# matthewyjiang/safe_bayesian_optimization

Measured on AMD Instinct MI355X. Metric: GP posterior+acq grid-points/sec at N train pts; 1/2/4/8 GPU, higher is better.
Workload: dtype f32 (bf16x3-split MFMA, f32 accumulation)

## Files before the change

### include/sbo.h

```cpp
#ifndef SBO_H_
#define SBO_H_

#include <stdint.h>

#ifdef __cplusplus
extern "C" {
#endif

#define SBO_API __attribute__((visibility("default")))

typedef enum sbo_status {
    SBO_OK = 0,
    SBO_E_INVAL = 1,
    SBO_E_NOT_SPD = 2,
    SBO_E_DEVICE = 3,
    SBO_E_OOM = 4,
    SBO_E_EMPTY = 5,
    SBO_E_STATE = 6
} sbo_status;

#define SBO_DEVICE_PTRS 0x1u
#define SBO_ASYNC 0x2u

typedef struct sbo_hyper {
// ... 89 lines not shown
SBO_API sbo_status sbo_import_state(sbo_ctx *ctx, const void *dev_buf, int64_t bytes);

SBO_API int64_t sbo_find_contours_external(const uint8_t *img, int width, int height,
                                           int32_t *pts, int64_t pts_cap,
                                           int64_t *start, int64_t contours_cap);

SBO_API sbo_status sbo_rbf_fill(sbo_ctx *ctx, const float *x, const float *y, int64_t n,
                                sbo_hyper hyper, float *K, uint32_t flags);
SBO_API sbo_status sbo_get_factor(sbo_ctx *ctx, float *L, float *alpha, uint32_t flags);

SBO_API sbo_status sbo_kd_order(const float *x, const float *y, int64_t n, int64_t first_offset, int64_t *perm);

#define SBO_OPT_INVERSE_BITS 1
#define SBO_OPT_SPATIAL_ORDER 2
#define SBO_OPT_TILE_SKIP 3
#define SBO_OPT_QUERY_ORDER 4
#define SBO_OPT_KERNEL_VARIANT 5
#define SBO_OPT_SWEEP_GROUPS 6
#define SBO_OPT_SKIP_BUDGET 7
#define SBO_OPT_CHOLESKY 8
#define SBO_OPT_INVERSE 9
#define SBO_OPT_JITTER_RETRIES 10
#define SBO_OPT_PRECISION 11
#define SBO_OPT_RESORT 12
#define SBO_OPT_CHOL_RESERVE 13
#define SBO_OPT_INV_OVERLAP 14
#define SBO_OPT_CHOL_OUTER 15
#define SBO_OPT_CHOL_DIAG 16
#define SBO_OPT_CHOL_GEMM 17
#define SBO_OPT_INV_BASE 18
#define SBO_OPT_INV_PANELS 19
#define SBO_OPT_INV_LEAVES 20
#define SBO_OPT_REPROBE 21
#define SBO_OPT_PRECISE_KERNEL 22
#define SBO_OPT_TABLE_MB 23
#define SBO_OPT_INV_OZ 24
#define SBO_OPT_INV_CHECK 25
#define SBO_OPT_PLAN_BLOCK 26
#define SBO_OPT_PROBE_SIZE 27
#define SBO_OPT_INV_OZ_MIN 28
#define SBO_OPT_INV_OZ_ADAPT 29
SBO_API sbo_status sbo_set_option(sbo_ctx *ctx, int option, int64_t value);

typedef struct sbo_inv_check {
    int32_t ran, fired, digits, m;
    double err, err_grid, err_train, err_fallback, tol, var_max, ms;
    double err_mean, mean_max, err_mean_fallback;
    int32_t kept_digits, reserved;
} sbo_inv_check;
SBO_API sbo_status sbo_get_inverse_check(const sbo_ctx *ctx, sbo_inv_check *out);

SBO_API sbo_status sbo_trim(sbo_ctx *ctx);

SBO_API sbo_status sbo_warmup(sbo_ctx *ctx, int64_t n_cap, int64_t m_cap, sbo_hyper hyper);

SBO_API sbo_status sbo_get_precision(const sbo_ctx *ctx, int *precise, double *probe_err, double *probe_var_min,
                                     double *probe_var_max);

typedef struct sbo_probe {
    int32_t precise, m_grid, m_train, precise_kernel;
    int64_t n_at_probe;
    double err, err_grid, err_train;
    double var_min, var_max, var_max_grid, var_max_train;
} sbo_probe;
SBO_API sbo_status sbo_get_probe(const sbo_ctx *ctx, sbo_probe *out);

SBO_API sbo_status sbo_get_skip(const sbo_ctx *ctx, int *cutoff_log2, double *max_row_l1, double *alpha_l1);

SBO_API sbo_status sbo_get_order(const sbo_ctx *ctx, int64_t *order);

SBO_API sbo_status sbo_get_inverse(sbo_ctx *ctx, float *Linv);

SBO_API sbo_status sbo_get_tile_bounds(sbo_ctx *ctx, float *bounds, int64_t cap);

SBO_API sbo_status sbo_profile(sbo_ctx *ctx, int enable);
SBO_API sbo_status sbo_profile_read(sbo_ctx *ctx, double *predict_ms, int64_t *predict_launches,
                                    double *fill_ms, int64_t *fill_launches);
SBO_API sbo_status sbo_profile_work(sbo_ctx *ctx, double *predict_flops);
SBO_API sbo_status sbo_profile_mfma(sbo_ctx *ctx, double *mfma_flops, int64_t *tiles_by_level );
SBO_API sbo_status sbo_debug_x3_stamps(sbo_ctx *ctx, double *cycles, int n);

SBO_API sbo_status sbo_debug_x3_operand(sbo_ctx *ctx, void *host_buf, int64_t cap, int64_t *bytes);

#define SBO_GZ_TRI_A 1u
#define SBO_GZ_TRANS_A 2u
#define SBO_GZ_TRI_B_LOWER 4u
#define SBO_GZ_TRI_B_UPPER 8u
#define SBO_GZ_TRANS_B 16u
#define SBO_GZ_TRANS_C 32u
#define SBO_GZ_BETA1 64u
#define SBO_GZ_LOWER_C 128u
SBO_API sbo_status sbo_debug_gz_gemm(sbo_ctx *ctx, int nd, int is_f32, const void *A, int64_t lda, int64_t a_cols,
                                     const void *B, int64_t ldb, int64_t b_cols, int64_t m, int64_t n, int64_t K,
                                     double alpha, void *C, int64_t ldc, int64_t c_cols, uint32_t flags);
SBO_API sbo_status sbo_debug_gz_gemm_packed(sbo_ctx *ctx, int nd, const float *P, int64_t ld, int64_t mpack,
                                            int64_t K, int64_t a0, int64_t m, int64_t b0, int64_t n, double alpha,
                                            float *C, int64_t ldc, int64_t c_cols, uint32_t flags);

#ifdef __cplusplus
}
#endif

#endif
```

### safe_bayesian_optimization_amd/_native.py

```python
from __future__ import annotations

import ctypes
import os
import subprocess

_PKG = os.path.dirname(os.path.abspath(__file__))
LIB_PATH = os.environ.get("SBO_LIB") or os.path.join(_PKG, "lib", "libsbo.so")

SBO_DEVICE_PTRS = 0x1
SBO_ASYNC = 0x2
SCORE_WIDTH = 0
SCORE_UCB = 1
SBO_E_STATE = 6

STATUS = {0: "SBO_OK", 1: "SBO_E_INVAL", 2: "SBO_E_NOT_SPD", 3: "SBO_E_DEVICE", 4: "SBO_E_OOM",
          5: "SBO_E_EMPTY", 6: "SBO_E_STATE"}

EXPORTS = (
    "sbo_version", "sbo_status_string", "sbo_create", "sbo_destroy", "sbo_set_stream", "sbo_last_error",
    "sbo_fit", "sbo_append", "sbo_num_train", "sbo_predict", "sbo_compute_sets", "sbo_compute_sets_f64", "sbo_argmax", "sbo_tick",
    "sbo_key_combine", "sbo_find_safety_contour_indices", "sbo_next_subgoal", "sbo_find_contours_external",
    "sbo_rbf_fill", "sbo_get_factor", "sbo_profile", "sbo_profile_read", "sbo_set_option", "sbo_get_inverse",
    "sbo_get_order", "sbo_profile_work", "sbo_profile_mfma", "sbo_debug_x3_stamps", "sbo_get_skip", "sbo_frontier", "sbo_subgoal",
    "sbo_get_bounds", "sbo_get_jitter", "sbo_get_tile_bounds", "sbo_state_bytes", "sbo_export_state", "sbo_import_state", "sbo_query_cost",
    "sbo_polygon_correct", "sbo_polydist", "sbo_point_within", "sbo_project_subgoal", "sbo_get_precision",
    "sbo_kd_order", "sbo_get_probe", "sbo_keys_reduce", "sbo_get_inverse_check", "sbo_trim", "sbo_warmup",
    "sbo_debug_gz_gemm", "sbo_debug_gz_gemm_packed", "sbo_debug_x3_operand",
)
SBO_GZ_TRI_A = 1
SBO_GZ_TRANS_A = 2
SBO_GZ_TRI_B_LOWER = 4
SBO_GZ_TRI_B_UPPER = 8
SBO_GZ_TRANS_B = 16
SBO_GZ_TRANS_C = 32
SBO_GZ_BETA1 = 64
SBO_GZ_LOWER_C = 128
SBO_OPT_INVERSE_BITS = 1
SBO_OPT_SPATIAL_ORDER = 2
SBO_OPT_TILE_SKIP = 3
SBO_OPT_QUERY_ORDER = 4
SBO_OPT_KERNEL_VARIANT = 5
SBO_OPT_SWEEP_GROUPS = 6
SBO_OPT_SKIP_BUDGET = 7
SBO_OPT_CHOLESKY = 8
SBO_OPT_INVERSE = 9
SBO_OPT_JITTER_RETRIES = 10
SBO_OPT_PRECISION = 11
SBO_OPT_RESORT = 12
SBO_OPT_CHOL_RESERVE = 13
SBO_OPT_INV_OVERLAP = 14
SBO_OPT_CHOL_OUTER = 15
SBO_OPT_CHOL_DIAG = 16
SBO_OPT_CHOL_GEMM = 17
SBO_OPT_INV_BASE = 18
SBO_OPT_INV_PANELS = 19
SBO_OPT_INV_LEAVES = 20
SBO_OPT_REPROBE = 21
SBO_OPT_PRECISE_KERNEL = 22
SBO_OPT_TABLE_MB = 23
SBO_OPT_INV_OZ = 24
SBO_OPT_INV_CHECK = 25
SBO_OPT_PLAN_BLOCK = 26
SBO_OPT_PROBE_SIZE = 27
SBO_OPT_INV_OZ_MIN = 28
SBO_OPT_INV_OZ_ADAPT = 29


class SboError(RuntimeError):
    def __init__(self, status: int, message: str = ""):
        self.status = status
        super().__init__(f"{STATUS.get(status, status)}: {message}")


class NotSPDError(SboError):
    pass


class sbo_hyper(ctypes.Structure):
    _fields_ = [("length_scale", ctypes.c_double), ("sigma_f", ctypes.c_double),
                ("noise_level", ctypes.c_double), ("prior_mean", ctypes.c_double)]


class sbo_key(ctypes.Structure):
    _fields_ = [("score", ctypes.c_double), ("idx", ctypes.c_int64)]


class sbo_probe(ctypes.Structure):
    _fields_ = [("precise", ctypes.c_int32), ("m_grid", ctypes.c_int32), ("m_train", ctypes.c_int32),
                ("precise_kernel", ctypes.c_int32), ("n_at_probe", ctypes.c_int64), ("err", ctypes.c_double),
                ("err_grid", ctypes.c_double), ("err_train", ctypes.c_double), ("var_min", ctypes.c_double),
                ("var_max", ctypes.c_double), ("var_max_grid", ctypes.c_double), ("var_max_train", ctypes.c_double)]


class sbo_inv_check(ctypes.Structure):
    _fields_ = [("ran", ctypes.c_int32), ("fired", ctypes.c_int32), ("digits", ctypes.c_int32), ("m", ctypes.c_int32),
                ("err", ctypes.c_double), ("err_grid", ctypes.c_double), ("err_train", ctypes.c_double),
                ("err_fallback", ctypes.c_double), ("tol", ctypes.c_double), ("var_max", ctypes.c_double),
                ("ms", ctypes.c_double), ("err_mean", ctypes.c_double), ("mean_max", ctypes.c_double),
                ("err_mean_fallback", ctypes.c_double), ("kept_digits", ctypes.c_int32), ("reserved", ctypes.c_int32)]


_lib = None


def build(jobs: int = 8) -> str:
    subprocess.run(["make", "-s", "-j", str(jobs), "-C", _PKG], check=True)
    return LIB_PATH


def lib():
# ... 22 lines not shown
    L.sbo_last_error.restype = ctypes.c_char_p
    L.sbo_fit.argtypes = [vp, vp, vp, vp, i64, sbo_hyper, u32]
    L.sbo_fit.restype = st
    L.sbo_append.argtypes = [vp, vp, vp, vp, i64, u32]
    L.sbo_append.restype = st
    L.sbo_num_train.argtypes = [vp]
    L.sbo_num_train.restype = i64
    L.sbo_predict.argtypes = [vp, vp, vp, i64, vp, vp, u32]
    L.sbo_predict.restype = st
    L.sbo_compute_sets.argtypes = [vp, vp, vp, i64, dbl, dbl, vp, vp, vp, u32]
    L.sbo_compute_sets.restype = st
    L.sbo_compute_sets_f64.argtypes = [vp, vp, vp, i64, dbl, dbl, vp, vp, vp, u32]
    L.sbo_compute_sets_f64.restype = st
    L.sbo_argmax.argtypes = [vp, vp, vp, i64, i64, ctypes.POINTER(sbo_key), u32]
    L.sbo_argmax.restype = st
    L.sbo_tick.argtypes = [vp, vp, vp, i64, dbl, dbl, i32, i64, vp, vp, vp, vp, vp, vp, u32]
    L.sbo_tick.restype = st
    L.sbo_query_cost.argtypes = [vp, vp, vp, i64, vp, u32]
    L.sbo_query_cost.restype = st
    L.sbo_key_combine.argtypes = [sbo_key, sbo_key]
    L.sbo_key_combine.restype = sbo_key
    L.sbo_keys_reduce.argtypes = [vp, vp, i64, vp, u32]
    L.sbo_keys_reduce.restype = st
    L.sbo_find_safety_contour_indices.argtypes = [vp, vp, vp, i64, i32, i32, vp, i64, ctypes.POINTER(i64)]
    L.sbo_find_safety_contour_indices.restype = st
    L.sbo_next_subgoal.argtypes = [vp, vp, vp, vp, vp, i64, i32, i32, dbl, dbl]
    L.sbo_next_subgoal.restype = i64
    L.sbo_frontier.argtypes = [vp, vp, vp, vp, i64, i32, i32, vp, i64, ctypes.POINTER(i64), u32]
    L.sbo_frontier.restype = st
    L.sbo_subgoal.argtypes = [vp, vp, vp, vp, vp, vp, i64, i32, i32, dbl, dbl, ctypes.POINTER(i64), u32]
    L.sbo_subgoal.restype = st
    L.sbo_get_tile_bounds.argtypes = [vp, vp, i64]
    L.sbo_get_tile_bounds.restype = st
    L.sbo_get_bounds.argtypes = [vp, vp]
    L.sbo_get_bounds.restype = st
    L.sbo_get_jitter.argtypes = [vp, ctypes.POINTER(dbl)]
    L.sbo_get_jitter.restype = st
    L.sbo_state_bytes.argtypes = [vp, ctypes.POINTER(i64)]
    L.sbo_state_bytes.restype = st
    L.sbo_export_state.argtypes = [vp, vp, i64]
    L.sbo_export_state.restype = st
    L.sbo_import_state.argtypes = [vp, vp, i64]
    L.sbo_import_state.restype = st
    L.sbo_find_contours_external.argtypes = [vp, i32, i32, vp, i64, vp, i64]
    L.sbo_find_contours_external.restype = i64
    L.sbo_rbf_fill.argtypes = [vp, vp, vp, i64, sbo_hyper, vp, u32]
    L.sbo_rbf_fill.restype = st
    L.sbo_get_factor.argtypes = [vp, vp, vp, u32]
    L.sbo_get_factor.restype = st
    L.sbo_set_option.argtypes = [vp, i32, i64]
    L.sbo_set_option.restype = st
    L.sbo_get_skip.argtypes = [vp, ctypes.POINTER(i32), ctypes.POINTER(dbl), ctypes.POINTER(dbl)]
    L.sbo_get_skip.restype = st
    L.sbo_get_precision.argtypes = [vp, ctypes.POINTER(i32), ctypes.POINTER(dbl), ctypes.POINTER(dbl),
                                    ctypes.POINTER(dbl)]
    L.sbo_get_precision.restype = st
    L.sbo_get_probe.argtypes = [vp, ctypes.POINTER(sbo_probe)]
    L.sbo_get_probe.restype = st
    L.sbo_get_inverse_check.argtypes = [vp, ctypes.POINTER(sbo_inv_check)]
    L.sbo_get_inverse_check.restype = st
    L.sbo_trim.argtypes = [vp]
    L.sbo_trim.restype = st
    L.sbo_warmup.argtypes = [vp, ctypes.c_int64, ctypes.c_int64, sbo_hyper]
    L.sbo_warmup.restype = st
    L.sbo_get_order.argtypes = [vp, vp]
    L.sbo_get_order.restype = st
    L.sbo_kd_order.argtypes = [vp, vp, i64, i64, vp]
    L.sbo_kd_order.restype = st
    L.sbo_get_inverse.argtypes = [vp, vp]
    L.sbo_get_inverse.restype = st
    L.sbo_profile.argtypes = [vp, i32]
    L.sbo_profile.restype = st
    L.sbo_profile_read.argtypes = [vp, ctypes.POINTER(dbl), ctypes.POINTER(i64), ctypes.POINTER(dbl),
                                   ctypes.POINTER(i64)]
    L.sbo_profile_read.restype = st
    L.sbo_profile_work.argtypes = [vp, ctypes.POINTER(dbl)]
    L.sbo_profile_work.restype = st
    L.sbo_profile_mfma.argtypes = [vp, ctypes.POINTER(dbl), ctypes.POINTER(i64)]
    L.sbo_profile_mfma.restype = st
    L.sbo_debug_x3_stamps.argtypes = [vp, ctypes.POINTER(dbl), ctypes.c_int]
    L.sbo_debug_x3_stamps.restype = st
    L.sbo_debug_x3_operand.argtypes = [vp, vp, i64, ctypes.POINTER(i64)]
    L.sbo_debug_x3_operand.restype = st
    L.sbo_debug_gz_gemm.argtypes = [vp, i32, i32, vp, i64, i64, vp, i64, i64, i64, i64, i64, dbl, vp, i64, i64, u32]
    L.sbo_debug_gz_gemm.restype = st
    L.sbo_debug_gz_gemm_packed.argtypes = [vp, i32, vp, i64, i64, i64, i64, i64, i64, i64, dbl, vp, i64, i64, u32]
    L.sbo_debug_gz_gemm_packed.restype = st
    pd = ctypes.POINTER(dbl)
    L.sbo_polygon_correct.argtypes = [vp, vp, i64, i64, ctypes.POINTER(i64)]
    L.sbo_polygon_correct.restype = st
    L.sbo_polydist.argtypes = [vp, vp, i64, dbl, dbl, pd, pd, pd]
    L.sbo_polydist.restype = st
    L.sbo_point_within.argtypes = [vp, vp, i64, dbl, dbl]
    L.sbo_point_within.restype = ctypes.c_int
    L.sbo_project_subgoal.argtypes = [vp, vp, i64, dbl, dbl, i64, vp, vp, i64, pd, pd, pd]
    L.sbo_project_subgoal.restype = ctypes.c_int
    _lib = L
    return L


def check(status: int, ctx=None) -> None:
    if status == 0:
        return
    msg = ""
    if ctx is not None:
        msg = lib().sbo_last_error(ctx).decode(errors="replace")
    if status == 2:
        raise NotSPDError(status, msg)
    raise SboError(status, msg)
```

### safe_bayesian_optimization_amd/csrc/kernels.hip

```cpp
#include <cstdio>
#include <cstdlib>
#include <algorithm>
#include <cstring>

#include <rocprim/rocprim.hpp>

#include "sbo_internal.hpp"

namespace sbo {
namespace {

typedef float f32x16 __attribute__((ext_vector_type(16)));

__device__ __forceinline__ float fast_exp2(float v) { return __builtin_amdgcn_exp2f(v); }

constexpr int kFillCols = 8;

template <bool VEC>
__global__ __launch_bounds__(256) void rbf_fill_kernel(const float *__restrict__ xa,
                                                       const float *__restrict__ ya, int64_t ma,
                                                       const float *__restrict__ xb,
                                                       const float *__restrict__ yb, int64_t mb,
                                                       int64_t ld, float c, float sf2, float sn2,
                                                       int diag, float *__restrict__ K) {
// ... 1265 lines not shown
            for (int b = 0; b < 3; ++b)
                if (b < nb) {
                    const float xf[4] = {ldexpf(sq[b][0], -ek), ldexpf(sq[b][1], -ek), ldexpf(sq[b][2], -ek),
                                         ldexpf(sq[b][3], -ek)};
                    store_sym_f32(gm, tbi[b], tbj[b], lane, xf);
                }
        }
        __syncthreads();
        double rs = 0.0;
        if (tid < kBK)
            for (int j = 0; j < kBK; ++j) rs += fabs((double)gm[tid * kTnGmLd + j]);
#pragma unroll
        for (int o = 32; o >= 1; o >>= 1) rs = fmax(rs, __shfl_xor(rs, o));
        if (lane == 0) red[1][wave] = rs;
        __syncthreads();
        rs = fmax(fmax(red[1][0], red[1][1]), fmax(red[1][2], red[1][3]));
        if (!live) rs = 0.0;
        const int spl = sp[pi];
        const double lg_g = (double)e0 +
                            ((double)T + log2(rs) - (double)((1 << kGramSquarings) - 1) * log2(1.0 - kSqEta)) /
                                (double)(1 << kGramSquarings) -
                            log2(1.0 - 0x1p-21);
        const double lg_pow = rs > 0.0 ? 0.5 * lg_g + 1e-6 - spl : -1000.0;
        const double spec2 = (rs > 0.0 ? exp2(2.0 * lg_pow) : 0.0) + kTnDelta * fro2 + ldexp(5.0, -110 - 2 * spl);
        const double lg_spec = spec2 > 0.0 ? 0.5 * log2(spec2) : -1000.0;
        const double lg_fro = fro2 > 0.0 ? 0.5 * log2(fro2) : -1000.0;
        const int o = 2 * pi;
        if (tid == 0) {
            out[o] = s > 0.0 ? (float)log2(16.0 * s) + 1e-5f : -1000.0f;
            out[o + 1] = (float)fmin(lg_spec, lg_fro) + 1e-5f;
        }
        if (plane < 0) lg_fro_a = lg_fro;
        __syncthreads();
    }
    if (tid == 0) {
        lgn[2 * tile] = make_float4(out[0], out[1], (float)lg_fro_a + 1e-5f, 0.0f);
        lgn[2 * tile + 1] = make_float4(out[2], out[3], out[4], out[5]);
    }
}

__global__ void widen_sub_kernel(const float *__restrict__ in, double v, int64_t n, double *__restrict__ d) {
    const int64_t i = (int64_t)blockIdx.x * blockDim.x + threadIdx.x;
    if (i < n) d[i] = (double)in[i] - v;
}

__global__ void narrow_kernel(const double *__restrict__ d, int64_t n, float *__restrict__ out) {
    const int64_t i = (int64_t)blockIdx.x * blockDim.x + threadIdx.x;
    if (i < n) out[i] = (float)d[i];
}

__global__ void tile_box_kernel(const float *__restrict__ x, const float *__restrict__ y, int64_t n,
                                int64_t ntiles, float4 *__restrict__ kbox) {
    const int64_t t = (int64_t)blockIdx.x * blockDim.x + threadIdx.x;
    if (t >= ntiles) return;
    float x0 = INFINITY, x1 = -INFINITY, y0 = INFINITY, y1 = -INFINITY;
    for (int64_t k = t * kBK; k < (t + 1) * kBK && k < n; ++k) {
        x0 = fminf(x0, x[k]); x1 = fmaxf(x1, x[k]);
        y0 = fminf(y0, y[k]); y1 = fmaxf(y1, y[k]);
    }
    kbox[t] = make_float4(x0, x1, y0, y1);
}

constexpr int kStageFloats = kTileFloats + 3 * kBK;
constexpr int kPredictWaves = kBN / 16;
constexpr int kPredictThreads = 64 * kPredictWaves;
constexpr int kDescWindow = 64;
constexpr int kListWindow = 512;
constexpr int kRecWindow = 64;
constexpr int kSmemFloats = 2 * kStageFloats + 2 * 256 + 2 * 256;
constexpr int kBudgetFloor = 40;
constexpr int kBinsPerBit = 4;
constexpr int kBudgetBins = kBudgetFloor * kBinsPerBit + 2;
constexpr int kPlanThreads = 256;
constexpr int kPlanWaves = kPlanThreads / 64;
constexpr int kPlanD2 = 2048;
constexpr int kPlanBinCache = 256;
constexpr int kPlanWriteBlocks = 4096;
constexpr int kPlanKeyShift = 40;
constexpr unsigned long long kPlanCountMask = (1ull << kPlanKeyShift) - 1ull;
constexpr unsigned kLevelWeight0 = 64, kLevelWeight1 = 42, kLevelWeight2 = 33;
constexpr unsigned kMeanWeight0 = 80, kMeanWeight1 = 45, kMeanWeight2 = 33;
__device__ unsigned g_mean_w[3] = {kMeanWeight0, kMeanWeight1, kMeanWeight2};
__device__ unsigned g_rb_slope = 0;
constexpr int kSteps = kBK / 4;
constexpr int kRowBlocks = kBM / 16;

typedef float f32x4 __attribute__((ext_vector_type(4)));

typedef float f32x2 __attribute__((ext_vector_type(2)));

__device__ __forceinline__ f32x2 kstar_pair(f32x2 x, f32x2 y, float xq, float yq, float cexp) {
    const f32x2 dx = x - xq, dy = y - yq;
    const f32x2 d2 = __builtin_elementwise_fma(dy, dy, dx * dx);
    const f32x2 a = d2 * cexp;
    f32x2 b;
    b.x = fast_exp2(a.x);
    b.y = fast_exp2(a.y);
    return b;
}

template <bool MEAN>
__device__ __forceinline__ void tile_steps(const float4 *__restrict__ pa, const float *__restrict__ pc, float xq,
                                           float yq, float cexp, f32x4 (&acc)[kRowBlocks], double &mu) {
    const f32x4 zero = {0.f, 0.f, 0.f, 0.f};
    const f32x2 *pc2 = reinterpret_cast<const f32x2 *>(pc);
    float4 a_cur[4];
#pragma unroll
    for (int jj = 0; jj < 4; ++jj) a_cur[jj] = pa[jj * 1024];
    f32x2 b_cur = kstar_pair(pc2[0], pc2[kBK / 2], xq, yq, cexp);
    f32x2 x1 = pc2[1], y1 = pc2[kBK / 2 + 1];
    f32x2 b_nxt = b_cur;
#pragma unroll
    for (int p = 0; p < kSteps; ++p) {
        float4 a_nxt[4];
        f32x2 x2 = x1, y2 = y1;
        if (p + 1 < kSteps) {
#pragma unroll
            for (int jj = 0; jj < 4; ++jj) a_nxt[jj] = pa[jj * 1024 + (p + 1) * 64];
        }
        if ((p & 1) == 0 && p + 4 < kSteps) {
            x2 = pc2[(p + 4) / 2];
            y2 = pc2[kBK / 2 + (p + 4) / 2];
        }
        const float alpha = MEAN ? pc[2 * kBK + p] : 0.0f;
        __builtin_amdgcn_sched_barrier(0);
        if ((p & 1) == 0 && p + 2 < kSteps) b_nxt = kstar_pair(x1, y1, xq, yq, cexp);
        const float b = (p & 1) ? b_cur.y : b_cur.x;
        if (MEAN) mu = fma((double)alpha, (double)b, mu);
#pragma unroll
        for (int jj = 0; jj < 4; ++jj) {
            acc[4 * jj + 0] = __builtin_amdgcn_mfma_f32_16x16x4f32(a_cur[jj].x, b, p == 0 ? zero : acc[4 * jj + 0], 0, 0, 0);
            acc[4 * jj + 1] = __builtin_amdgcn_mfma_f32_16x16x4f32(a_cur[jj].y, b, p == 0 ? zero : acc[4 * jj + 1], 0, 0, 0);
            acc[4 * jj + 2] = __builtin_amdgcn_mfma_f32_16x16x4f32(a_cur[jj].z, b, p == 0 ? zero : acc[4 * jj + 2], 0, 0, 0);
            acc[4 * jj + 3] = __builtin_amdgcn_mfma_f32_16x16x4f32(a_cur[jj].w, b, p == 0 ? zero : acc[4 * jj + 3], 0, 0, 0);
        }
        __builtin_amdgcn_sched_barrier(0);
        if (p + 1 < kSteps) {
#pragma unroll
            for (int jj = 0; jj < 4; ++jj) a_cur[jj] = a_nxt[jj];
        }
        if ((p & 1) == 0) {
            x1 = x2;
            y1 = y2;
        } else {
            b_cur = b_nxt;
        }
    }
}

__device__ __forceinline__ float wave_min(float v) {
#pragma unroll
    for (int o = 32; o >= 1; o >>= 1) v = fminf(v, __shfl_xor(v, o));
    return v;
}
__device__ __forceinline__ float wave_max(float v) {
#pragma unroll
    for (int o = 32; o >= 1; o >>= 1) v = fmaxf(v, __shfl_xor(v, o));
    return v;
}

struct QBox {
    float x0, x1, y0, y1;
};

__device__ __forceinline__ float tile_box_d2(const float4 b, const QBox &q) {
    const float dx = fmaxf(0.0f, fmaxf(b.x - q.x1, q.x0 - b.y));
    const float dy = fmaxf(0.0f, fmaxf(b.z - q.y1, q.y0 - b.w));
    return fmaf(dy, dy, dx * dx);
}

constexpr float kLg3 = -14.36f;
constexpr float kLg1 = -6.96f;
constexpr float kRho0 = 0.0029f;
constexpr float kRho1 = -9.0f + 0.0029f;
constexpr float kRho2 = -18.0f + 0.0058f;

__device__ __forceinline__ int inc_bin(float l, unsigned long long &w, float key = 0.0f) {
    const float f = (l + key + (float)kBudgetFloor) * (float)kBinsPerBit + 1.0f;
    const int bi = f < 0.0f ? 0 : (f >= (float)(kBudgetBins - 1) ? kBudgetBins - 1 : (int)f);
    w = bi < kBudgetBins - 1 ? (unsigned long long)ceilf(exp2f(l + 32.0f) * 1.0001f) + 1ull : 0ull;
    return bi;
}

__device__ __forceinline__ float lg_add(float a, float b) {
    const float hi = fmaxf(a, b), lo = fminf(a, b);
    return hi + __log2f(1.0f + exp2f(lo - hi)) + 1e-4f;
}

__device__ __forceinline__ void tile_increments(float d2, float kn, float4 lgn_t, float4 lgp_t, float cexp,
                                                float lg_tau, float2 key, int (&bi)[3],
                                                unsigned long long (&w)[3]) {
    const float kmax = cexp * d2 * 0.999f;
    const float b = fminf(lgn_t.x + kmax, lgn_t.y + kn) - lg_tau + 0.01f;
    const float n0 = fminf(lgn_t.x + kRho0 + kmax, lg_add(lgn_t.y, lgn_t.z - 9.0f) + kn) - lg_tau + 0.01f;
    const float n1 = fminf(lgp_t.x + kmax, lgp_t.y + kn) - lg_tau + 0.01f;
    const float n2 = fminf(lgp_t.z + kmax, lgp_t.w + kn) - lg_tau + 0.01f;
    const float r3 = lg_add(lg_add(n2 + kRho0, n1 + kRho1), n0 + kRho2);
    const float r1 = lg_add(n1 + kRho0, n0 + kRho1);
    const float r31 = lg_add(r3, r1);
    bi[0] = inc_bin(r3, w[0], key.x);
    bi[1] = inc_bin(r1, w[1], key.y);
    const float dl = r31 - b;
    bi[2] = dl < -0.01f ? inc_bin(b + __log2f(1.0f - exp2f(dl)), w[2]) : inc_bin(b, w[2]);
    bi[1] = max(bi[1], bi[0]);
    bi[2] = max(bi[2], bi[1]);
}

struct PlanRule {
    const float4 *kbox;
    const float4 *lgn;
    float cexp, skip_d2, skip_d2_mean, lg_tau;
    int nI;
    QBox box;
    const float *d2s;
    const float *kns;
    int levels;
    float2 key;

    __device__ __forceinline__ float d2(int t) const { return t < kPlanD2 ? d2s[t] : tile_box_d2(kbox[t], box); }
    __device__ __forceinline__ float kn(int t) const { return t < kPlanD2 ? kns[t] : 3.0f + cexp * d2(t) * 0.999f; }

    __device__ __forceinline__ bool far_tile(int I, int t, float dd) const {
        const float kf = fmaxf(0.0f, fmaxf(key.x + kLg3, key.y + kLg1));
        return lgn[2 * (tile_start(I) + t)].x + cexp * dd * 0.999f - lg_tau + 0.01f + kf < -(float)kBudgetFloor;
    }

    __device__ __forceinline__ void incs(int I, int t, int (&bi)[3], unsigned long long (&w)[3]) const {
        const int64_t T = tile_start(I) + t;
        tile_increments(d2(t), kn(t), lgn[2 * T], lgn[2 * T + 1], cexp, lg_tau, key, bi, w);
        if (levels != 1) {
            bi[0] = bi[1] = 0;
            w[0] = w[1] = 0ull;
            const float kmax = cexp * d2(t) * 0.999f;
            const float4 l = lgn[2 * T];
            bi[2] = inc_bin(fminf(l.x + kmax, l.y + kn(t)) - lg_tau + 0.01f, w[2]);
        }
    }

    __device__ unsigned long long total_weight(int I, int lane, bool &over) const {
        const int T = kTilesPerRowBlockStep * (I + 1);
        unsigned long long wsum = 0;
        int ov = 0;
        for (int t0 = 0; t0 < T; t0 += 64) {
            const int t = t0 + lane;
            if (t < T) {
                if (far_tile(I, t, d2(t))) {
                    wsum += 6ull;
                } else {
                    int bi[3];
                    unsigned long long w[3];
                    incs(I, t, bi, w);
#pragma unroll
                    for (int j = 0; j < 3; ++j) {
                        if (bi[j] < kBudgetBins - 1) wsum += w[j];
                        else ov = 1;
                    }
                }
            }
            if (__ballot(ov)) break;
        }
#pragma unroll
        for (int o = 32; o >= 1; o >>= 1) {
            wsum += __shfl_xor(wsum, o);
            ov |= __shfl_xor(ov, o);
        }
        over = ov != 0;
        return wsum;
    }

    __device__ int threshold(int I, unsigned long long *bins, int lane, unsigned long long budget,
                             unsigned *bc = nullptr) const {
        if (!lgn) return -1;
        const int T = kTilesPerRowBlockStep * (I + 1);
        for (int i = lane; i < kBudgetBins; i += 64) bins[i] = 0ull;
        __builtin_amdgcn_wave_barrier();
        unsigned long long nfar = 0;
        for (int t = lane; t < T; t += 64) {
            if (far_tile(I, t, d2(t))) {
                ++nfar;
                if (bc && t < kPlanBinCache) bc[t] = 0u;
                continue;
            }
            int bi[3];
            unsigned long long w[3];
            incs(I, t, bi, w);
            if (bc && t < kPlanBinCache) bc[t] = (unsigned)bi[0] | ((unsigned)bi[1] << 8) | ((unsigned)bi[2] << 16);
#pragma unroll
            for (int j = 0; j < 3; ++j)
                if (bi[j] < kBudgetBins - 1) atomicAdd(bins + bi[j], w[j]);
        }
        if (nfar) atomicAdd(bins, 6ull * nfar);
        __builtin_amdgcn_wave_barrier();
        constexpr int per = (kBudgetBins + 63) / 64;
        unsigned long long v[per], run = 0;
#pragma unroll
        for (int j = 0; j < per; ++j) {
            const int i = lane * per + j;
            v[j] = i < kBudgetBins - 1 ? bins[i] : (1ull << 40);
            run += v[j];
        }
        unsigned long long incl = run;
#pragma unroll
        for (int o = 1; o < 64; o <<= 1) {
            const unsigned long long u = __shfl_up(incl, o);
            if (lane >= o) incl += u;
        }
        unsigned long long pre = incl - run;
        int ok = 0;
#pragma unroll
        for (int j = 0; j < per; ++j) {
            pre += v[j];
            ok += pre <= budget ? 1 : 0;
        }
#pragma unroll
        for (int o = 32; o >= 1; o >>= 1) ok += __shfl_xor(ok, o);
        __builtin_amdgcn_wave_barrier();
        return ok - 1;
    }

    __device__ __forceinline__ int level(int I, int t, int drop_max, const unsigned *bc = nullptr) const {
        const float dd = d2(t);
        int code;
        if (lgn) {
            int spent;
            if (bc && t < kPlanBinCache) {
                const unsigned c = bc[t];
                spent = ((int)(c & 0xffu) <= drop_max) + ((int)((c >> 8) & 0xffu) <= drop_max) +
                        ((int)(c >> 16) <= drop_max);
            } else if (far_tile(I, t, dd)) {
                spent = drop_max >= 0 ? 3 : 0;
            } else {
                int bi[3];
                unsigned long long w[3];
                incs(I, t, bi, w);
                spent = (bi[0] <= drop_max) + (bi[1] <= drop_max) + (bi[2] <= drop_max);
            }
            code = spent == 3 ? -1 : (levels == 1 ? spent : (levels > 1 ? levels - 2 : 0));
        } else {
            code = (skip_d2 <= 0.0f || dd <= skip_d2) ? 0 : -1;
        }
        if (code < 0 && I == nI - 1 && dd <= skip_d2_mean) code = lgn && levels ? 2 : 0;
        return code;
    }
};

__device__ __forceinline__ float plan_ref(float lg_tau, int nI) { return lg_tau + 0.5f * __log2f((float)nI) - 1e-4f; }
constexpr int kPlanMaxI = 512;

__device__ __forceinline__ float tile_knorm(const float *__restrict__ kc, const QBox &b, float cexp, float d2box) {
    float sum = 0.0f;
    for (int i = 0; i < kBK; ++i) {
        const float px = kc[i], py = kc[kBK + i];
        const float dx = fmaxf(0.0f, fmaxf(b.x0 - px, px - b.x1));
        const float dy = fmaxf(0.0f, fmaxf(b.y0 - py, py - b.y1));
        sum += __builtin_amdgcn_exp2f(fmaf(2.0f * cexp, fmaf(dy, dy, dx * dx) * 0.999f, 120.0f));
    }
    return sum > 0.0f ? 0.5f * (__log2f(sum * 1.002f) - 120.0f) + 0.001f : 3.0f + cexp * d2box * 0.999f;
}

__device__ QBox plan_setup(const float *__restrict__ qx, const float *__restrict__ qy, int64_t m, int64_t qb,
                           const float4 *__restrict__ kbox, const float *__restrict__ kcoord, float cexp, int nkt,
                           float *d2s, float *kns, float *red) {
    const int tid = threadIdx.x, lane = tid & 63, wave = tid >> 6;
    const int64_t q = qb * kBN + (tid & (kBN - 1));
    const int64_t qc = q < m ? q : m - 1;
    const float xq = qx[qc], yq = qy[qc];
    const float bx0 = wave_min(xq), bx1 = wave_max(xq), by0 = wave_min(yq), by1 = wave_max(yq);
    if (lane == 0) {
        red[wave * 4 + 0] = bx0; red[wave * 4 + 1] = bx1;
        red[wave * 4 + 2] = by0; red[wave * 4 + 3] = by1;
    }
    __syncthreads();
    QBox b = {red[0], red[1], red[2], red[3]};
#pragma unroll
    for (int w = 1; w < kPlanWaves; ++w) {
        b.x0 = fminf(b.x0, red[w * 4 + 0]); b.x1 = fmaxf(b.x1, red[w * 4 + 1]);
        b.y0 = fminf(b.y0, red[w * 4 + 2]); b.y1 = fmaxf(b.y1, red[w * 4 + 3]);
    }
    for (int t = tid; t < nkt && t < kPlanD2; t += kPlanThreads) {
        const float d = tile_box_d2(kbox[t], b);
        d2s[t] = d;
        kns[t] = (kcoord && cexp * d > -400.0f) ? tile_knorm(kcoord + (int64_t)t * (3 * kBK), b, cexp, d)
                                                : 3.0f + cexp * d * 0.999f;
    }
    __syncthreads();
    return b;
}

__device__ __forceinline__ int64_t plan_item(int I, int nI, int64_t nQ, int64_t qb, int blk = 0) {
    const int64_t r = nI - 1 - I;
    if (blk == 0) return r * nQ + qb;
    const int64_t bi = blk >> 8, bq = blk & 255;
    const int64_t IB = r / bi, ii = r % bi, QB = qb / bq, qq = qb % bq;
    const int64_t bie = min(bi, (int64_t)nI - IB * bi), bqe = min(bq, nQ - QB * bq);
    return IB * bi * nQ + QB * bie * bq + ii * bqe + qq;
}
__device__ __forceinline__ void plan_item_inv(int64_t item, int nI, int64_t nQ, int blk, int &I, int64_t &qb) {
    if (blk == 0) {
        I = nI - 1 - (int)(item / nQ);
        qb = item % nQ;
        return;
    }
    const int64_t bi = blk >> 8, bq = blk & 255;
    const int64_t IB = item / (bi * nQ), r0 = item - IB * bi * nQ;
    const int64_t bie = min(bi, (int64_t)nI - IB * bi);
    const int64_t QB = r0 / (bie * bq), r1 = r0 - QB * bie * bq;
    const int64_t bqe = min(bq, nQ - QB * bq);
    I = nI - 1 - (int)(IB * bi + r1 / bqe);
    qb = QB * bq + r1 % bqe;
}
__host__ __device__ __forceinline__ int plan_chunks(int nI) { return (kTilesPerRowBlockStep * nI + 63) / 64; }

__global__ __launch_bounds__(kPlanThreads) void plan_count_kernel(
    const float4 *__restrict__ kbox, const float *__restrict__ kcoord, const float4 *__restrict__ lgn, int levels,
    float2 lvl_key, int nI,
    int64_t nQ,
    const float *__restrict__ qx, const float *__restrict__ qy, int64_t m, float cexp, float skip_d2,
    float skip_d2_mean, float lg_tau, float m0, int64_t ldp, float *__restrict__ part, float *__restrict__ mean,
    unsigned long long *__restrict__ key, unsigned char *__restrict__ thr, unsigned long long *__restrict__ wkey,
    unsigned long long *__restrict__ bits, int wide, int blk) {
    extern __shared__ unsigned plan_dyn[];
    __shared__ float red[4 * kPlanWaves];
    __shared__ unsigned long long bins[kPlanWaves][kBudgetBins];
    __shared__ unsigned long long wtot[kPlanMaxI];
    __shared__ unsigned long long budget_exp;
    const int64_t qb = blockIdx.x;
    const int lane = threadIdx.x & 63, wave = threadIdx.x >> 6;
    const int nkt = kTilesPerRowBlockStep * nI;
    unsigned *bc = plan_dyn + wave * kPlanBinCache;
    float *d2s = reinterpret_cast<float *>(plan_dyn + kPlanWaves * kPlanBinCache);
    float *kns = d2s + min(nkt, kPlanD2);
    PlanRule R{kbox, lgn, cexp, skip_d2, skip_d2_mean, plan_ref(lg_tau, nI), nI, {}, d2s, kns, levels, lvl_key};
    R.box = plan_setup(qx, qy, m, qb, kbox, lgn ? kcoord : nullptr, cexp, nkt, d2s, kns, red);
    const bool fill = lgn && nI <= kPlanMaxI;
    if (fill) {
        for (int I = wave; I < nI; I += kPlanWaves) {
            bool over;
            const unsigned long long w = R.total_weight(I, lane, over);
            if (lane == 0) wtot[I] = over ? ~0ull : w;
        }
        __syncthreads();
        if (threadIdx.x == 0) {
            const double one = 4294967296.0;
            double share = 1.0 / sqrt((double)nI);
            for (int it = 0; it < 4; ++it) {
                double cheap2 = 0.0;
                int nexp = 0;
                for (int I = 0; I < nI; ++I) {
                    const double w = wtot[I] == ~0ull ? 2.0 : (double)wtot[I] / one;
                    if (w <= share) cheap2 += w * w;
                    else ++nexp;
                }
                if (nexp == 0) break;
                const double s2 = fmax(0.0, (1.0 - cheap2) * (1.0 - 1e-9)) / (double)nexp;
                const double sn = sqrt(s2) * (1.0 - 1e-9);
                if (!(sn > share)) break;
                share = sn;
            }
            budget_exp = (unsigned long long)floor(share * one);
        }
        __syncthreads();
    }
    for (int I = wave; I < nI; I += kPlanWaves) {
        const int T = kTilesPerRowBlockStep * (I + 1);
        const unsigned long long bud = !fill ? (unsigned long long)floor(4294967296.0 / sqrt((double)nI))
                                       : (wtot[I] <= budget_exp ? ~0ull : budget_exp);
        const int drop_max = R.threshold(I, bins[wave], lane, bud, bc);
        const int64_t item = plan_item(I, nI, nQ, qb, blk);
        unsigned long long *ib = bits + item * (int64_t)plan_chunks(nI) * 3;
        int cnt = 0;
        unsigned wsum = 0;
#pragma unroll 1
        for (int t0 = 0; t0 < T; t0 += 64) {
            const int t = t0 + lane;
            const int code = t < T ? R.level(I, t, drop_max, bc) : -1;
            const unsigned long long b0 = __ballot(code == 0), b1 = __ballot(code == 1), b2 = __ballot(code == 2);
            if (lane < 3) ib[(t0 >> 6) * 3 + lane] = lane == 0 ? (b0 | b1 | b2) : (lane == 1 ? b1 : b2);
            const int n0 = __popcll(b0), n1 = __popcll(b1), n2 = __popcll(b2);
            cnt += n0 + n1 + n2;
            wsum += I == nI - 1 ? g_mean_w[0] * n0 + g_mean_w[1] * n1 + g_mean_w[2] * n2
                                : kLevelWeight0 * n0 + kLevelWeight1 * n1 + kLevelWeight2 * n2;
        }
        if (g_rb_slope)
            wsum = (unsigned)((unsigned long long)wsum * (100u * (unsigned)nI + g_rb_slope * (unsigned)I) /
                              (100u * (unsigned)nI));
        if (lane == 0) {
            key[item] = (unsigned long long)cnt | ((cnt > 0 ? 1ull : 0ull) << kPlanKeyShift);
            thr[item] = (unsigned char)(drop_max + 1);
            wkey[item] = wsum;
        }
        if (cnt == 0)
            for (int j = lane; j < kBN; j += 64) {
                const int64_t q = qb * kBN + j;
                if (q < m) {
                    if (wide) {
                        reinterpret_cast<double *>(part)[(int64_t)I * ldp + q] = 0.0;
                        if (I == nI - 1) reinterpret_cast<double *>(mean)[q] = (double)m0;
                    } else {
                        part[(int64_t)I * ldp + q] = 0.0f;
                        if (I == nI - 1) mean[q] = m0;
                    }
                }
            }
    }
}

__global__ __launch_bounds__(256) void plan_write_kernel(
    int nI, int64_t nQ, const unsigned long long *__restrict__ key, const unsigned long long *__restrict__ scan,
    const unsigned long long *__restrict__ bits, int4 *__restrict__ desc, unsigned short *__restrict__ tl,
    int prod_full, unsigned long long *__restrict__ partial, int blk) {
    const int lane = threadIdx.x & 63;
    const int64_t gw = (int64_t)blockIdx.x * 4 + (threadIdx.x >> 6), nw = (int64_t)gridDim.x * 4;
    const int64_t items = (int64_t)nI * nQ;
    unsigned long long prod = 0, nl1 = 0, nl2 = 0;
    for (int64_t item = gw; item < items; item += nw) {
        const unsigned long long k = key[item];
        const int cnt = (int)(k & kPlanCountMask);
        if (cnt > 0) {
            int I;
            int64_t qb;
            plan_item_inv(item, nI, nQ, blk, I, qb);
            const unsigned long long ex = scan[item] - k;
            const uint64_t off = ex & kPlanCountMask;
            const int64_t ne = (int64_t)(ex >> kPlanKeyShift);
            const int T = kTilesPerRowBlockStep * (I + 1);
            const unsigned long long *ib = bits + item * (int64_t)plan_chunks(nI) * 3;
            uint64_t base = off;
            for (int t0 = 0; t0 < T; t0 += 64) {
                const unsigned long long kept = ib[(t0 >> 6) * 3], l1 = ib[(t0 >> 6) * 3 + 1],
                                         l2 = ib[(t0 >> 6) * 3 + 2];
                if ((kept >> lane) & 1ull) {
                    const int code = ((l1 >> lane) & 1ull) ? 1 : (((l2 >> lane) & 1ull) ? 2 : 0);
                    tl[base + __popcll(kept & ((1ull << lane) - 1ull))] =
                        (unsigned short)((t0 + lane) | (code << kLevelShift));
                    prod += code == 0 ? prod_full : (code == 1 ? 3 : 1);
                    nl1 += code == 1 ? 1 : 0;
                    nl2 += code == 2 ? 1 : 0;
                }
                base += __popcll(kept);
            }
            if (lane == 0) desc[ne] = make_int4(I, (int)qb, (int)(uint32_t)off, cnt | (int)((off >> 32) << 16));
        }
    }
    if (partial) {
#pragma unroll
        for (int o = 32; o >= 1; o >>= 1) {
            prod += __shfl_xor(prod, o);
            nl1 += __shfl_xor(nl1, o);
            nl2 += __shfl_xor(nl2, o);
        }
        if (lane == 0) {
            unsigned long long *p = partial + 3 * gw;
            p[0] = prod;
            p[1] = nl1;
            p[2] = nl2;
        }
    }
}

__global__ __launch_bounds__(256) void plan_counts_reduce_kernel(const unsigned long long *__restrict__ partial,
                                                                 int64_t n, unsigned long long *__restrict__ out) {
    __shared__ unsigned long long red[3][256];
    unsigned long long v[3] = {0, 0, 0};
    for (int64_t i = threadIdx.x; i < n; i += 256)
#pragma unroll
        for (int j = 0; j < 3; ++j) v[j] += partial[3 * i + j];
#pragma unroll
    for (int j = 0; j < 3; ++j) red[j][threadIdx.x] = v[j];
    __syncthreads();
    for (int o = 128; o >= 1; o >>= 1) {
        if ((int)threadIdx.x < o)
#pragma unroll
            for (int j = 0; j < 3; ++j) red[j][threadIdx.x] += red[j][threadIdx.x + o];
        __syncthreads();
    }
    if (threadIdx.x == 0)
#pragma unroll
        for (int j = 0; j < 3; ++j) out[j] += red[j][0];
}

__global__ void plan_seg_kernel(const unsigned long long *__restrict__ scan, int64_t n_items,
                                const int4 *__restrict__ desc, int P, int *__restrict__ seg,
                                unsigned long long *__restrict__ tiles_done, const unsigned long long *__restrict__ wkey,
                                const unsigned long long *__restrict__ wscan, int nI, int64_t nQ, int blk) {
    const unsigned long long last = scan[n_items - 1];
    const uint64_t total = last & kPlanCountMask;
    const uint64_t wtotal = wscan[n_items - 1];
    const int64_t nne = (int64_t)(last >> kPlanKeyShift);
    for (int w = threadIdx.x; w <= P; w += blockDim.x) {
        if (w == P) {
            seg[P] = (int)nne;
            continue;
        }
        const uint64_t target = wtotal * (uint64_t)w / (uint64_t)P;
        int64_t lo = 0, hi = nne;
        while (lo < hi) {
            const int64_t mid = (lo + hi) >> 1;
            const int4 d = desc[mid];
            const int64_t it = plan_item(d.x, nI, nQ, d.y, blk);
            const uint64_t off = wscan[it] - wkey[it];
            if (off < target) lo = mid + 1; else hi = mid;
        }
        seg[w] = (int)lo;
    }
    if (threadIdx.x == 0 && tiles_done) atomicAdd(tiles_done, (unsigned long long)total);
}

__device__ __forceinline__ int64_t xcd_position(int64_t k, const int *__restrict__ xseg, int G) {
    int x = 0;
#pragma unroll
    for (int i = 1; i < 8; ++i) x += k >= xseg[i] ? 1 : 0;
    const int64_t a = xseg[x], n = xseg[x + 1] - a, q = n / G, rm = n % G, c = (k - a) % G, j = (k - a) / G;
    return a + c * q + (c < rm ? c : rm) + j;
}

__global__ void plan_perm_kernel(const unsigned long long *__restrict__ scan, int64_t n_items,
                                 const int4 *__restrict__ desc, const int *__restrict__ xseg, int G,
                                 int *__restrict__ pos_of, unsigned long long *__restrict__ cnt2) {
    const int64_t nne = (int64_t)(scan[n_items - 1] >> kPlanKeyShift);
    const int64_t k = (int64_t)blockIdx.x * blockDim.x + threadIdx.x;
    if (k >= nne) return;
    const int64_t p = xcd_position(k, xseg, G);
    pos_of[k] = (int)p;
    cnt2[p] = (unsigned long long)(desc[k].w & 0xffff);
}

__device__ __forceinline__ int4 step_record(int64_t ts, int I, int qb, int te, int i, int cnt);

__global__ __launch_bounds__(256) void plan_move_kernel(const unsigned long long *__restrict__ scan, int64_t n_items,
                                                        const int4 *__restrict__ desc,
                                                        const unsigned short *__restrict__ tl,
                                                        const int *__restrict__ pos_of,
                                                        const unsigned long long *__restrict__ off2,
                                                        int4 *__restrict__ desc2, unsigned short *__restrict__ tl2,
                                                        int4 *__restrict__ rec) {
    const int64_t nne = (int64_t)(scan[n_items - 1] >> kPlanKeyShift);
    const int64_t k = (int64_t)blockIdx.x * 4 + (threadIdx.x >> 6);
    const int lane = threadIdx.x & 63;
    if (k >= nne) return;
    const int4 d = desc[k];
    const int cnt = d.w & 0xffff;
    const uint64_t off = (uint64_t)(uint32_t)d.z | ((uint64_t)((uint32_t)d.w >> 16) << 32);
    const int p = pos_of[k];
    const uint64_t o2 = off2[p];
    const int64_t ts = tile_start(d.x);
    for (int i = lane; i < cnt; i += 64) {
        const unsigned short te = tl[off + i];
        tl2[o2 + i] = te;
        if (rec) rec[o2 + i] = step_record(ts, d.x, d.y, te, i, cnt);
    }
    if (lane == 0) desc2[p] = make_int4(d.x, d.y, (int)(uint32_t)o2, cnt | (int)((o2 >> 32) << 16));
}

__device__ __forceinline__ int4 step_record(int64_t ts, int I, int qb, int te, int i, int cnt) {
    const int t = te & ((1 << kLevelShift) - 1);
    const int w = I | ((te >> kLevelShift) << 16) | (i == 0 ? kRecFirst : 0) | (i == cnt - 1 ? kRecLast : 0);
    return make_int4((int)(uint32_t)((ts + t) * 96), t * 256, qb, w);
}

__global__ __launch_bounds__(256) void plan_rec_kernel(const unsigned long long *__restrict__ scan, int64_t n_items,
                                                       const int4 *__restrict__ desc,
                                                       const unsigned short *__restrict__ tl, int4 *__restrict__ rec) {
    const int64_t nne = (int64_t)(scan[n_items - 1] >> kPlanKeyShift);
    const int64_t k = (int64_t)blockIdx.x * 4 + (threadIdx.x >> 6);
    const int lane = threadIdx.x & 63;
    if (k >= nne) return;
    const int4 d = desc[k];
    const int cnt = d.w & 0xffff;
    const uint64_t off = (uint64_t)(uint32_t)d.z | ((uint64_t)((uint32_t)d.w >> 16) << 32);
    const int64_t ts = tile_start(d.x);
    for (int i = lane; i < cnt; i += 64) rec[off + i] = step_record(ts, d.x, d.y, tl[off + i], i, cnt);
}

__global__ void plan_seg2_kernel(const int *__restrict__ xseg, int G, int P, int *__restrict__ seg2) {
    for (int r = threadIdx.x; r <= P; r += blockDim.x) {
        if (r == P) {
            seg2[P] = xseg[8];
            continue;
        }
        const int x = r / G, c = r % G;
        const int a = xseg[x], n = xseg[x + 1] - a, q = n / G, rm = n % G;
        seg2[r] = a + c * q + (c < rm ? c : rm);
    }
}

__global__ void plan_block_cost_kernel(const unsigned long long *__restrict__ wkey, int nI, int64_t nQ,
                                       float *__restrict__ bcost) {
    const int64_t qb = (int64_t)blockIdx.x * blockDim.x + threadIdx.x;
    if (qb >= nQ) return;
    unsigned long long c = 0;
    for (int I = 0; I < nI; ++I) c += wkey[plan_item(I, nI, nQ, qb)];
    bcost[qb] = (float)((double)c / (double)kLevelWeight0);
}

__global__ __launch_bounds__(kBN) void plan_query_cost_kernel(const float *__restrict__ bcost, int64_t m,
                                                              const int32_t *__restrict__ perm,
                                                              float *__restrict__ cost) {
    __shared__ int nv;
    const int64_t qb = blockIdx.x, i = qb * kBN + threadIdx.x;
    const int64_t o = i < m ? (perm ? (int64_t)perm[i] : i) : -1;
    if (threadIdx.x == 0) nv = 0;
    __syncthreads();
    if (o >= 0) atomicAdd(&nv, 1);
    __syncthreads();
// ... 136 lines not shown
        if (j == cnt - 1) {
            double s = 0.0;
#pragma unroll
            for (int rb = 0; rb < kRowBlocks; ++rb)
#pragma unroll
                for (int c = 0; c < 4; ++c) {
                    s = fma((double)outer[rb][c], (double)outer[rb][c], s);
                    outer[rb][c] = (OT)0;
                }
            s += __shfl_xor(s, 16);
            s += __shfl_xor(s, 32);
            const bool writer = lane < 16 && q < m;
            if (writer) part[(int64_t)I * ldp + q] = (float)s;
            if (I == nI - 1) {
                mu += __shfl_xor(mu, 16);
                mu += __shfl_xor(mu, 32);
                if (writer) mean[q] = (float)((double)m0 + mu);
                mu = 0.0;
            }
        }
        asm volatile("s_waitcnt vmcnt(0)" ::: "memory");
        __syncthreads();
        if (!more) break;
        if (kn != k) {
            k = kn;
            dc = dn;
            xq = xqn;
            yq = yqn;
            q = (int64_t)dc.y * kBN + wave * 16 + r;
        }
        j = jn;
        ++e;
        cur ^= 1;
    }
#undef SBO_STAGE
#undef SBO_DESC_WINDOW
#undef SBO_LIST_WINDOW
#undef SBO_DMA16
}

__device__ __forceinline__ bool key_better(double as, int64_t ai, double bs, int64_t bi) {
    if (ai < 0) return false;
    if (bi < 0) return true;
    if (as > bs) return true;
    if (as < bs) return false;
    return ai < bi;
}

__device__ __forceinline__ void block_reduce_key(double &s, int64_t &i, sbo_key *out) {
    __shared__ double ss[kAcqThreads / 64];
    __shared__ int64_t si[kAcqThreads / 64];
#pragma unroll
    for (int off = 32; off >= 1; off >>= 1) {
        const double os = __shfl_xor(s, off);
        const int64_t oi = __shfl_xor(i, off);
        if (key_better(os, oi, s, i)) { s = os; i = oi; }
    }
    const int w = threadIdx.x >> 6;
    if ((threadIdx.x & 63) == 0) { ss[w] = s; si[w] = i; }
    __syncthreads();
    if (threadIdx.x == 0) {
        for (int k = 1; k < (int)(blockDim.x >> 6); ++k)
            if (key_better(ss[k], si[k], s, i)) { s = ss[k]; i = si[k]; }
        out->score = s;
        out->idx = i;
    }
}

template <typename T>
__device__ __forceinline__ void compute_sets_one(T mu, T sd, double beta, double f_min,
                                                 double &lo, double &hi, bool &safe) {
    const double c = __dmul_rn(beta, (double)sd);
    lo = __dsub_rn((double)mu, c);
    hi = __dadd_rn((double)mu, c);
    safe = lo > f_min;
}

template <class PT>
__global__ __launch_bounds__(kAcqThreads) void acquire_kernel(
    const PT *__restrict__ part, const PT *__restrict__ mean, int nI, int64_t ldp, int64_t m,
    double sf2, double beta, double f_min, int score_kind, int64_t index_offset,
    const int32_t *__restrict__ perm, float *__restrict__ mu_out, float *__restrict__ sd_out,
    double *__restrict__ lo_out, double *__restrict__ hi_out, uint8_t *__restrict__ safe_out,
    sbo_key *__restrict__ keys) {
    const int64_t i = (int64_t)blockIdx.x * kAcqThreads + threadIdx.x;
    double bs = 0.0;
    int64_t bi = -1;
    if (i < m && (!perm || perm[i] >= 0)) {
        double s = 0.0;
        int I = 0;
        for (; I + 8 <= nI; I += 8) {
            PT v[8];
#pragma unroll
            for (int u = 0; u < 8; ++u) v[u] = part[(int64_t)(I + u) * ldp + i];
#pragma unroll
            for (int u = 0; u < 8; ++u) s += (double)v[u];
        }
        for (; I < nI; ++I) s += (double)part[(int64_t)I * ldp + i];
        double vd = sf2 - s;
        float var = vd > 0.0 ? (float)vd : 0.0f;
        const float sd = __fsqrt_rn(var);
        const float mu = (float)mean[i];
        const int64_t o = perm ? (int64_t)perm[i] : i;
        if (mu_out) mu_out[o] = mu;
        if (sd_out) sd_out[o] = sd;
        double lo, hi;
        bool safe;
        compute_sets_one(mu, sd, beta, f_min, lo, hi, safe);
        if (lo_out) lo_out[o] = lo;
        if (hi_out) hi_out[o] = hi;
        if (safe_out) safe_out[o] = safe ? 1 : 0;
        const double score = score_kind == SBO_SCORE_UCB ? hi : __dsub_rn(hi, lo);
        if (safe && score == score) { bs = score; bi = index_offset + o; }
    }
    block_reduce_key(bs, bi, keys + blockIdx.x);
}

template <typename T>
__global__ __launch_bounds__(kAcqThreads) void sets_kernel(const T *__restrict__ mu,
                                                           const T *__restrict__ sd, int64_t m,
                                                           double beta, double f_min,
                                                           double *__restrict__ lo,
                                                           double *__restrict__ hi,
                                                           uint8_t *__restrict__ safe) {
    const int64_t i = (int64_t)blockIdx.x * kAcqThreads + threadIdx.x;
    if (i >= m) return;
    double l, h;
    bool s;
    compute_sets_one(mu[i], sd[i], beta, f_min, l, h, s);
    if (lo) lo[i] = l;
    if (hi) hi[i] = h;
    if (safe) safe[i] = s ? 1 : 0;
}

__global__ __launch_bounds__(kAcqThreads) void argmax_kernel(const double *__restrict__ score,
                                                             const uint8_t *__restrict__ mask,
                                                             int64_t m, int64_t index_offset,
                                                             sbo_key *__restrict__ keys) {
    const int64_t i = (int64_t)blockIdx.x * kAcqThreads + threadIdx.x;
    double bs = 0.0;
    int64_t bi = -1;
    if (i < m && (!mask || mask[i])) {
        const double v = score[i];
        if (v == v) { bs = v; bi = index_offset + i; }
    }
    block_reduce_key(bs, bi, keys + blockIdx.x);
}

__global__ __launch_bounds__(kAcqThreads) void reduce_keys_kernel(const sbo_key *__restrict__ keys,
                                                                  int64_t nb,
                                                                  sbo_key *__restrict__ out) {
    double bs = 0.0;
    int64_t bi = -1;
    for (int64_t k = threadIdx.x; k < nb; k += kAcqThreads) {
        const sbo_key v = keys[k];
        if (key_better(v.score, v.idx, bs, bi)) { bs = v.score; bi = v.idx; }
    }
    block_reduce_key(bs, bi, out);
}

}

hipError_t launch_rbf_fill(hipStream_t s, const float *xa, const float *ya, int64_t ma, const float *xb,
                           const float *yb, int64_t mb, int64_t ld, float ell, float sf2, float sn2, bool diag,
                           float *K) {
    const float c = -1.0f / (2.0f * ell * ell);
    const dim3 grid((unsigned)((ma + 1023) / 1024), (unsigned)((mb + kFillCols - 1) / kFillCols));
    const bool vec = (ld % 4 == 0) && ((reinterpret_cast<uintptr_t>(K) & 15) == 0) &&
                     ((reinterpret_cast<uintptr_t>(xa) & 15) == 0) &&
                     ((reinterpret_cast<uintptr_t>(ya) & 15) == 0);
    if (vec)
        hipLaunchKernelGGL(rbf_fill_kernel<true>, grid, dim3(256), 0, s, xa, ya, ma, xb, yb, mb, ld, c, sf2, sn2,
                           (int)diag, K);
    else
        hipLaunchKernelGGL(rbf_fill_kernel<false>, grid, dim3(256), 0, s, xa, ya, ma, xb, yb, mb, ld, c, sf2, sn2,
                           (int)diag, K);
    return hipGetLastError();
}

hipError_t launch_sub_scalar(hipStream_t s, const float *in, float v, int64_t n, float *out) {
    hipLaunchKernelGGL(sub_scalar_kernel, dim3((unsigned)((n + 255) / 256)), dim3(256), 0, s, in, v, n, out);
// ... 103 lines not shown
                           s, L11, ld, kb, A21, m2);
    else if (version == 2)
        hipLaunchKernelGGL(chol_trsm_mfma_kernel, dim3((unsigned)((m2 + kCholNB - 1) / kCholNB)), dim3(2 * kCholNB), 0,
                           s, L11, ld, kb, A21, m2);
    else
        hipLaunchKernelGGL(chol_trsm_kernel, dim3((unsigned)((m2 + kCholNB - 1) / kCholNB)), dim3(2 * kCholNB), 0, s,
                           L11, ld, kb, A21, m2);
    return hipGetLastError();
}

hipError_t launch_pack_tile_norms(hipStream_t s, const double *Linv, int64_t ld, int64_t n, int64_t npad, int64_t I0,
                                  double sf2, float *aug, float4 *lgn) {
    const int64_t nI = npad / kBM;
    const int64_t t0 = tile_start(I0), t1 = tile_start(nI);
    if (t1 <= t0) return hipSuccess;
    hipLaunchKernelGGL(tile_norm_kernel<true>, dim3((unsigned)(t1 - t0)), dim3(kBM), 0, s, aug, t0, lgn, Linv, ld, n,
                       sf2, aug);
    return hipGetLastError();
}

hipError_t launch_tile_norms(hipStream_t s, const float *aug, int64_t npad, int64_t I0, float4 *lgn) {
    const int64_t nI = npad / kBM;
    const int64_t t0 = tile_start(I0), t1 = tile_start(nI);
    if (t1 <= t0) return hipSuccess;
    hipLaunchKernelGGL(tile_norm_kernel<false>, dim3((unsigned)(t1 - t0)), dim3(kBM), 0, s, aug, t0, lgn, nullptr,
                       (int64_t)0, (int64_t)0, 0.0, nullptr);
    return hipGetLastError();
}

hipError_t launch_widen_sub(hipStream_t s, const float *in, double v, int64_t n, double *d) {
    hipLaunchKernelGGL(widen_sub_kernel, dim3((unsigned)((n + 255) / 256)), dim3(256), 0, s, in, v, n, d);
    return hipGetLastError();
}

hipError_t launch_narrow(hipStream_t s, const double *d, int64_t n, float *out) {
    hipLaunchKernelGGL(narrow_kernel, dim3((unsigned)((n + 255) / 256)), dim3(256), 0, s, d, n, out);
    return hipGetLastError();
}

size_t alpha_work_bytes(int64_t n) { return sizeof(double) * (size_t)((n + kAlK - 1) / kAlK) * (size_t)n; }

hipError_t launch_alpha_f64(hipStream_t s, const double *X, int64_t ld, int64_t n, const float *obs, double m0,
                            double *z, double *alpha, double *work) {
    if (n <= 0) return hipSuccess;
    const dim3 g1((unsigned)((n + kAlRows - 1) / kAlRows), (unsigned)((n + kAlK - 1) / kAlK));
    hipLaunchKernelGGL(alpha_z_kernel, g1, dim3(256), 0, s, X, ld, n, obs, m0, work);
    hipError_t e = hipGetLastError();
    if (e != hipSuccess) return e;
    hipLaunchKernelGGL(alpha_z_reduce_kernel, dim3((unsigned)((n + 255) / 256)), dim3(256), 0, s, work, n, z);
    if ((e = hipGetLastError()) != hipSuccess) return e;
    hipLaunchKernelGGL(alpha_xtz_kernel, dim3((unsigned)((n + 3) / 4)), dim3(256), 0, s, X, ld, n, z, alpha);
    return hipGetLastError();
}

hipError_t launch_row_dot(hipStream_t s, const double *A, int64_t ld, int64_t rows, int64_t n, const double *x,
                          double *out) {
    if (rows <= 0) return hipSuccess;
    hipLaunchKernelGGL(row_dot_kernel, dim3((unsigned)rows), dim3(256), 0, s, A, ld, n, x, out);
    return hipGetLastError();
}

hipError_t launch_narrow_2d(hipStream_t s, const double *d, int64_t ldd, int64_t m, int64_t n, float *out,
                            int64_t ldo) {
    if (m <= 0 || n <= 0) return hipSuccess;
    hipLaunchKernelGGL(narrow_2d_kernel, dim3((unsigned)((m + 255) / 256), (unsigned)std::min<int64_t>(n, kMaxGridY)),
                       dim3(256), 0, s, d, ldd, m, n, out, ldo);
    return hipGetLastError();
}

hipError_t launch_narrow_strided(hipStream_t s, const double *d, int64_t n, float *out, int64_t stride) {
    if (n <= 0) return hipSuccess;
    hipLaunchKernelGGL(narrow_strided_kernel, dim3((unsigned)((n + 255) / 256)), dim3(256), 0, s, d, n, out, stride);
    return hipGetLastError();
}

hipError_t launch_tile_boxes(hipStream_t s, const float *x, const float *y, int64_t n, int64_t npad, float4 *kbox) {
    const int64_t nt = npad / kBK;
    hipLaunchKernelGGL(tile_box_kernel, dim3((unsigned)((nt + 255) / 256)), dim3(256), 0, s, x, y, n, nt, kbox);
    return hipGetLastError();
}

namespace {
struct PlanLayout {
    size_t key, scan, thr, desc, tl, seg, temp, temp_bytes, wkey, wscan, lvcnt, rec, bits;
    bool xcd;
    size_t xseg, pos_of, cnt2, off2, desc2, tl2, seg2, temp2, temp2_bytes;
    size_t total;
};

bool xcd_interleave(int P) { return P >= 8 && P % 8 == 0; }

PlanLayout plan_layout(int64_t nI, int64_t nQ, int P) {
    const int64_t items = nI * nQ;
    const int64_t cap = 2 * nI * (nI + 1) * nQ;
    PlanLayout L{};
    size_t o = 0;
    auto take = [&](size_t b) {
        const size_t at = o;
        o = (o + b + 255) / 256 * 256;
        return at;
    };
    L.key = take(8 * (size_t)items);
    L.scan = take(8 * (size_t)items);
    L.thr = take((size_t)items);
    L.wkey = take(8 * (size_t)items);
    L.wscan = take(8 * (size_t)items);
    L.lvcnt = take(8 * 3 * 4 * (size_t)kPlanWriteBlocks);
    L.bits = take(8 * 3 * (size_t)items * (size_t)plan_chunks((int)nI));
    L.desc = take(16 * (size_t)(items + 2 * kDescWindow));
    L.tl = take(2 * (size_t)(cap + 2 * kListWindow));
    L.seg = take(4 * (size_t)(P + 1));
    L.rec = take(16 * (size_t)(cap + 2 * kRecWindow));
    size_t tb = 0;
    (void)rocprim::inclusive_scan(nullptr, tb, (const unsigned long long *)nullptr, (unsigned long long *)nullptr,
                                  (size_t)items, rocprim::plus<unsigned long long>());
    L.temp = take(tb);
    L.temp_bytes = tb;
    L.xcd = xcd_interleave(P);
    if (L.xcd) {
        L.xseg = take(4 * 9);
        L.pos_of = take(4 * (size_t)items);
        L.cnt2 = take(8 * (size_t)items);
        L.off2 = take(8 * (size_t)items);
        L.desc2 = take(16 * (size_t)(items + 2 * kDescWindow));
        L.tl2 = take(2 * (size_t)(cap + 2 * kListWindow));
        L.seg2 = take(4 * (size_t)(P + 1));
        size_t t2 = 0;
        (void)rocprim::exclusive_scan(nullptr, t2, (const unsigned long long *)nullptr, (unsigned long long *)nullptr,
                                      0ull, (size_t)items, rocprim::plus<unsigned long long>());
        L.temp2 = take(t2);
        L.temp2_bytes = t2;
    }
    L.total = o;
    return L;
}

float cutoff_d2(int L, double ce) { return L > 0 ? (float)((double)L / -ce * 1.001) : -1.0f; }
double exp2_coef(float ell) { return -1.0 / (2.0 * (double)ell * (double)ell * 0.69314718055994530942); }
}

size_t predict_work_bytes(int64_t npad, int64_t m, int P) {
    return plan_layout(npad / kBM, (m + kBN - 1) / kBN, P).total;
}

hipError_t launch_plan(hipStream_t s, const float4 *kbox, int64_t npad, const float *qx, const float *qy, int64_t m,
                       int64_t ldp, float ell, float m0, const SkipPlan &skip, float *part, float *mean,
                       unsigned long long *tiles_done, int P, void *work, size_t work_bytes) {
    const int nI = (int)(npad / kBM);
    const int64_t nQ = (m + kBN - 1) / kBN;
    const int64_t items = (int64_t)nI * nQ;
    if (m <= 0 || nI <= 0) return hipSuccess;
    if (nQ > 0x7fffffff || items >= (1ll << (64 - kPlanKeyShift)) ||
        2 * (int64_t)nI * (nI + 1) * nQ >= (1ll << kPlanKeyShift) || kTilesPerRowBlockStep * (int64_t)nI > (1 << kLevelShift) - 1)
        return hipErrorInvalidValue;
    const PlanLayout L = plan_layout(nI, nQ, P);
    if (work_bytes < L.total) return hipErrorInvalidValue;
    if (skip.order_blk != 0 && ((skip.order_blk >> 8) < 1 || (skip.order_blk & 255) < 1 || (skip.order_blk >> 16) != 0))
        return hipErrorInvalidValue;
    char *w = static_cast<char *>(work);
    auto *key = reinterpret_cast<unsigned long long *>(w + L.key);
    auto *scan = reinterpret_cast<unsigned long long *>(w + L.scan);
    auto *thr = reinterpret_cast<unsigned char *>(w + L.thr);
    auto *desc = reinterpret_cast<int4 *>(w + L.desc);
    auto *tl = reinterpret_cast<unsigned short *>(w + L.tl);
    auto *seg = reinterpret_cast<int *>(w + L.seg);
    auto *wkey = reinterpret_cast<unsigned long long *>(w + L.wkey);
    auto *wscan = reinterpret_cast<unsigned long long *>(w + L.wscan);
#ifdef SBO_DIAG
    if (const char *ev = getenv("SBO_MEAN_W")) {
        unsigned v[3] = {kMeanWeight0, kMeanWeight1, kMeanWeight2};
        if (sscanf(ev, "%u,%u,%u", &v[0], &v[1], &v[2]) == 3)
            (void)hipMemcpyToSymbolAsync(HIP_SYMBOL(g_mean_w), v, sizeof(v), 0, hipMemcpyHostToDevice, s);
    }
    if (const char *ev = getenv("SBO_RB_SLOPE")) {
        const unsigned v = (unsigned)std::max(0, atoi(ev));
        (void)hipMemcpyToSymbolAsync(HIP_SYMBOL(g_rb_slope), &v, sizeof(v), 0, hipMemcpyHostToDevice, s);
    }
#endif
    const double ce = exp2_coef(ell);
    const float cexp = (float)ce;
    const float skip_d2 = cutoff_d2(skip.L, ce);
    const float skip_d2_mean = skip.L > 0 && skip.L_mean > skip.L ? cutoff_d2(skip.L_mean, ce) : skip_d2;
    const float4 *lgn = skip.L > 0 ? skip.lgn : nullptr;
    const int levels = lgn ? skip.levels : 0;
    auto *bits = reinterpret_cast<unsigned long long *>(w + L.bits);
    const int nc = std::min(kTilesPerRowBlockStep * nI, kPlanD2);
    const size_t plan_lds = 4 * (size_t)kPlanWaves * kPlanBinCache + 8 * (size_t)nc;
    hipLaunchKernelGGL(plan_count_kernel, dim3((unsigned)nQ), dim3(kPlanThreads), plan_lds, s, kbox, skip.kcoord, lgn,
                       levels, make_float2(skip.lvl_key[0], skip.lvl_key[1]), nI,
                       nQ, qx, qy,
                       m, cexp, skip_d2, skip_d2_mean, skip.lg_tau_v, m0, ldp, part, mean, key, thr, wkey, bits,
                       skip.wide ? 1 : 0, skip.order_blk);
    hipError_t e = hipGetLastError();
    if (e != hipSuccess) return e;
    size_t tb = L.temp_bytes;
    e = rocprim::inclusive_scan(w + L.temp, tb, key, scan, (size_t)items, rocprim::plus<unsigned long long>(), s);
    if (e != hipSuccess) return e;
    tb = L.temp_bytes;
    e = rocprim::inclusive_scan(w + L.temp, tb, wkey, wscan, (size_t)items, rocprim::plus<unsigned long long>(), s);
    if (e != hipSuccess) return e;
    const int64_t wblocks = std::min<int64_t>((items + 3) / 4, kPlanWriteBlocks);
    hipLaunchKernelGGL(plan_write_kernel, dim3((unsigned)wblocks), dim3(256), 0, s, nI, nQ, key, scan, bits,
                       desc, tl, skip.prod_full, tiles_done ? reinterpret_cast<unsigned long long *>(w + L.lvcnt) : nullptr,
                       skip.order_blk);
    if (tiles_done)
        hipLaunchKernelGGL(plan_counts_reduce_kernel, dim3(1), dim3(256), 0, s,
                           reinterpret_cast<const unsigned long long *>(w + L.lvcnt), wblocks * 4, tiles_done + 1);
    auto *rec = reinterpret_cast<int4 *>(w + L.rec);
    if (!L.xcd) {
        hipLaunchKernelGGL(plan_seg_kernel, dim3(1), dim3(256), 0, s, scan, items, desc, P, seg, tiles_done, wkey,
                           wscan, nI, nQ, skip.order_blk);
        if (skip.records)
            hipLaunchKernelGGL(plan_rec_kernel, dim3((unsigned)((items + 3) / 4)), dim3(256), 0, s, scan, items, desc,
                               tl, rec);
        return hipGetLastError();
    }
    auto *xseg = reinterpret_cast<int *>(w + L.xseg);
    auto *pos_of = reinterpret_cast<int *>(w + L.pos_of);
    auto *cnt2 = reinterpret_cast<unsigned long long *>(w + L.cnt2);
    auto *off2 = reinterpret_cast<unsigned long long *>(w + L.off2);
    auto *desc2 = reinterpret_cast<int4 *>(w + L.desc2);
    auto *tl2 = reinterpret_cast<unsigned short *>(w + L.tl2);
    auto *seg2 = reinterpret_cast<int *>(w + L.seg2);
    const int G = P / 8;
    e = hipMemsetAsync(cnt2, 0, 8 * (size_t)items, s);
    if (e != hipSuccess) return e;
    hipLaunchKernelGGL(plan_seg_kernel, dim3(1), dim3(256), 0, s, scan, items, desc, 8, xseg, tiles_done, wkey, wscan,
                       nI, nQ, skip.order_blk);
    hipLaunchKernelGGL(plan_perm_kernel, dim3((unsigned)((items + 255) / 256)), dim3(256), 0, s, scan, items, desc,
                       xseg, G, pos_of, cnt2);
    e = hipGetLastError();
    if (e != hipSuccess) return e;
    size_t t2 = L.temp2_bytes;
    e = rocprim::exclusive_scan(w + L.temp2, t2, cnt2, off2, 0ull, (size_t)items,
                                rocprim::plus<unsigned long long>(), s);
    if (e != hipSuccess) return e;
    hipLaunchKernelGGL(plan_move_kernel, dim3((unsigned)((items + 3) / 4)), dim3(256), 0, s, scan, items, desc, tl,
                       pos_of, off2, desc2, tl2, skip.records ? rec : nullptr);
    hipLaunchKernelGGL(plan_seg2_kernel, dim3(1), dim3(256), 0, s, xseg, G, P, seg2);
    return hipGetLastError();
}

void plan_views(int64_t npad, int64_t m, int P, const void *work, const int4 **desc, const unsigned short **tl,
                const int **seg, const int4 **rec) {
    const PlanLayout L = plan_layout(npad / kBM, (m + kBN - 1) / kBN, P);
    const char *w = static_cast<const char *>(work);
    *desc = reinterpret_cast<const int4 *>(w + (L.xcd ? L.desc2 : L.desc));
    *tl = reinterpret_cast<const unsigned short *>(w + (L.xcd ? L.tl2 : L.tl));
    *seg = reinterpret_cast<const int *>(w + (L.xcd ? L.seg2 : L.seg));
    if (rec) *rec = reinterpret_cast<const int4 *>(w + L.rec);
}

float exp2_coef_f(float ell) { return (float)exp2_coef(ell); }

hipError_t launch_plan_cost(hipStream_t s, int64_t npad, int64_t m, int P, const void *work, const int32_t *perm,
                            float *bcost, float *cost) {
    const int nI = (int)(npad / kBM);
    const int64_t nQ = (m + kBN - 1) / kBN;
    if (m <= 0 || nI <= 0) return hipSuccess;
    const PlanLayout L = plan_layout(nI, nQ, P);
    const auto *wkey = reinterpret_cast<const unsigned long long *>(static_cast<const char *>(work) + L.wkey);
    hipLaunchKernelGGL(plan_block_cost_kernel, dim3((unsigned)((nQ + 255) / 256)), dim3(256), 0, s, wkey, nI, nQ,
                       bcost);
    hipLaunchKernelGGL(plan_query_cost_kernel, dim3((unsigned)nQ), dim3(kBN), 0, s, bcost, m, perm, cost);
    return hipGetLastError();
}

hipError_t launch_predict(hipStream_t s, const float *aug, const float *kcoord, int64_t npad, const float *qx,
                          const float *qy, int64_t m, int64_t ldp, float ell, float m0, float *part, float *mean,
                          int variant, int P, const void *work) {
    const int nI = (int)(npad / kBM);
    const int64_t nQ = (m + kBN - 1) / kBN;
    if (m <= 0 || nI <= 0) return hipSuccess;
    const int4 *desc = nullptr;
    const unsigned short *tl = nullptr;
    const int *seg = nullptr;
    plan_views(npad, m, P, work, &desc, &tl, &seg);
    const float cexp = (float)exp2_coef(ell);
#define SBO_PREDICT_ARGS aug, kcoord, desc, tl, seg, P, (int)(nI * nQ), nI, qx, qy, m, ldp, cexp, m0, part, mean
    switch (variant) {
        case 1: hipLaunchKernelGGL((predict_kernel<double>), dim3((unsigned)P), dim3(kPredictThreads), 0, s, SBO_PREDICT_ARGS); break;
        default: hipLaunchKernelGGL((predict_kernel<float>), dim3((unsigned)P), dim3(kPredictThreads), 0, s, SBO_PREDICT_ARGS); break;
    }
#undef SBO_PREDICT_ARGS
    return hipGetLastError();
}

hipError_t launch_acquire(hipStream_t s, const float *part, const float *mean, int nI, int64_t ldp,
                          int64_t m, float sf2, double beta, double f_min, int score_kind,
                          int64_t index_offset, const int32_t *perm, float *mu, float *sd, double *lo,
                          double *hi, uint8_t *safe, sbo_key *block_keys) {
    hipLaunchKernelGGL(acquire_kernel<float>, dim3((unsigned)acq_blocks(m)), dim3(kAcqThreads), 0, s, part, mean,
                       nI, ldp, m, (double)sf2, beta, f_min, score_kind, index_offset, perm, mu, sd, lo, hi, safe,
                       block_keys);
    return hipGetLastError();
}

hipError_t launch_acquire(hipStream_t s, const double *part, const double *mean, int nI, int64_t ldp,
                          int64_t m, double sf2, double beta, double f_min, int score_kind,
                          int64_t index_offset, const int32_t *perm, float *mu, float *sd, double *lo,
                          double *hi, uint8_t *safe, sbo_key *block_keys) {
    hipLaunchKernelGGL(acquire_kernel<double>, dim3((unsigned)acq_blocks(m)), dim3(kAcqThreads), 0, s, part, mean,
                       nI, ldp, m, sf2, beta, f_min, score_kind, index_offset, perm, mu, sd, lo, hi, safe,
                       block_keys);
    return hipGetLastError();
}

hipError_t launch_sets(hipStream_t s, const float *mu, const float *sd, int64_t m, double beta,
                       double f_min, double *lo, double *hi, uint8_t *safe) {
    hipLaunchKernelGGL(sets_kernel<float>, dim3((unsigned)acq_blocks(m)), dim3(kAcqThreads), 0, s, mu, sd, m, beta,
                       f_min, lo, hi, safe);
    return hipGetLastError();
}

hipError_t launch_sets(hipStream_t s, const double *mu, const double *sd, int64_t m, double beta,
                       double f_min, double *lo, double *hi, uint8_t *safe) {
    hipLaunchKernelGGL(sets_kernel<double>, dim3((unsigned)acq_blocks(m)), dim3(kAcqThreads), 0, s, mu, sd, m,
                       beta, f_min, lo, hi, safe);
    return hipGetLastError();
}

hipError_t launch_argmax_blocks(hipStream_t s, const double *score, const uint8_t *mask, int64_t m,
                                int64_t index_offset, sbo_key *block_keys) {
    hipLaunchKernelGGL(argmax_kernel, dim3((unsigned)acq_blocks(m)), dim3(kAcqThreads), 0, s, score, mask,
                       m, index_offset, block_keys);
    return hipGetLastError();
}

hipError_t launch_reduce_keys(hipStream_t s, const sbo_key *keys, int64_t nblocks, sbo_key *out) {
    hipLaunchKernelGGL(reduce_keys_kernel, dim3(1), dim3(kAcqThreads), 0, s, keys, nblocks, out);
    return hipGetLastError();
}

}
```

### safe_bayesian_optimization_amd/csrc/sbo_api.cpp

```cpp
#include <rocsolver/rocsolver.h>

#include <algorithm>
#include <limits>
#include <cstddef>
#include <cmath>
#include <cstring>
#include <new>
#include <string>
#include <thread>
#include <vector>

#include "sbo_internal.hpp"

using sbo::DevBuf;

namespace {

constexpr const char *kVersion = "sbo-mi355x 0.1.0";

#define SBO_HIP(expr)                                                                   \
    do {                                                                                \
        hipError_t e_ = (expr);                                                         \
        if (e_ != hipSuccess) {                                                         \
            ctx->err = std::string(#expr) + ": " + hipGetErrorString(e_);               \
// ... 847 lines not shown
    if (p.aux) {
        SBO_HIP(hipEventRecord(ctx->ev_panel, ctx->stream));
        SBO_HIP(hipStreamWaitEvent(ctx->aux_stream, ctx->ev_panel, 0));
    }
    if (p.inc_alpha) {
        const int64_t b = n - n_old;
        const double one = 1.0;
        SBO_HIP(ctx->rvec.reserve(sizeof(double) * (size_t)n));
        double *rv = ctx->rvec.as<double>();
        SBO_HIP(sbo::launch_widen_sub(sa, ctx->obs.as<float>(), ctx->hyper.prior_mean, n, rv));
        SBO_BLAS(rocblas_set_pointer_mode(ha, rocblas_pointer_mode_host));
        SBO_HIP(sbo::launch_row_dot(sa, Li + n_old, ld, b, n, rv, zv + n_old));
        SBO_HIP(hipMemsetAsync(d + n_old, 0, sizeof(double) * (size_t)b, sa));
        SBO_BLAS(rocblas_dgemv(ha, rocblas_operation_transpose, (rocblas_int)b, (rocblas_int)n, &one, Li + n_old,
                               (rocblas_int)ld, zv + n_old, 1, &one, d, 1));
    } else {
        SBO_HIP(ctx->awork.reserve(sbo::alpha_work_bytes(n)));
        SBO_HIP(sbo::launch_alpha_f64(sa, Li, ld, n, ctx->obs.as<float>(), ctx->hyper.prior_mean, zv, d,
                                      ctx->awork.as<double>()));
    }
    ctx->z_n = n;
    SBO_HIP(sbo::launch_narrow(sa, d, n, ctx->alpha.as<float>()));
    if (p.aux) SBO_HIP(hipEventRecord(ctx->ev_trail, ctx->aux_stream));
    return SBO_OK;
}

sbo_status refresh_packs(sbo_ctx *ctx, const RefreshPlan &p) {
    const int64_t n = p.n, ld = p.ld, npad = p.npad, I0 = p.I0;
    double *Li = ctx->Linv.as<double>();
    ctx->a64_I0 = std::min(ctx->a64_I0, I0);
    if (!p.incr) ctx->a64_I0 = 0;
    if (p.eager_x3) {
        if (p.x3_layout != ctx->x3_layout) ctx->x3_I0 = 0;
        const int64_t xI0 = std::max<int64_t>(std::min(ctx->x3_I0, I0), 0);
        SBO_HIP(grow_keep(ctx, ctx->ax3, sbo::x3_operand_bytes(npad), sbo::x3_operand_bytes(xI0 * sbo::kBM)));
        SBO_HIP(ctx->kc3.reserve(sbo::x3_coord_bytes(npad)));
        ctx->x3_I0 = xI0;
    }
    if (p.eager_f64)
        if (sbo_status st = reserve_precise(ctx, npad, std::max<int64_t>(ctx->a64_I0, 0))) return st;
#if SBO_FUSED_TN
    SBO_HIP(grow_keep(ctx, ctx->tile_lgn, 2 * sizeof(float4) * (size_t)sbo::total_tiles(p.nI),
                      2 * sizeof(float4) * p.old_tiles));
    SBO_HIP(sbo::launch_pack_tile_norms(ctx->stream, Li, ld, n, npad, I0, p.sf2, ctx->aug.as<float>(),
                                        ctx->tile_lgn.as<float4>()));
#else
    SBO_HIP(sbo::launch_pack_tiles(ctx->stream, Li, ld, n, npad, I0, p.sf2, ctx->aug.as<float>()));
#endif
    if (!p.eager_x3 && !p.eager_f64) return SBO_OK;
    SBO_HIP(hipEventRecord(ctx->ev_panel, ctx->stream));
    SBO_HIP(hipStreamWaitEvent(ctx->aux_stream, ctx->ev_panel, 0));
    if (p.eager_x3)
        SBO_HIP(sbo::launch_pack_x3(ctx->aux_stream, ctx->aug.as<float>(), nullptr, npad, ctx->x3_I0, p.x3_layout,
                                    ctx->ax3.as<char>(), nullptr));
    SBO_HIP(ctx->scratch.reserve(sizeof(double) * (size_t)npad));
    SBO_HIP(sbo::launch_row_l1(ctx->aux_stream, ctx->aug.as<float>(), npad, I0, ctx->scratch.as<double>()));
    SBO_HIP(hipEventRecord(ctx->ev_pack, ctx->aux_stream));
    if (p.eager_f64) {
        if (sbo_status st = pack_precise(ctx, ctx->aux_stream, npad, std::max<int64_t>(ctx->a64_I0, 0))) return st;
        ctx->a64_I0 = INT64_MAX;
        SBO_HIP(hipEventRecord(ctx->ev_poz, ctx->aux_stream));
        ctx->poz_pending = true;
    }
    return SBO_OK;
}

sbo_status refresh_f32(sbo_ctx *ctx, const RefreshPlan &p) {
    const int64_t n = p.n, ld = p.ld;
    float *L = ctx->L.as<float>(), *alpha = ctx->alpha.as<float>();
    ctx->linv_n = 0;
    SBO_HIP(sbo::launch_sub_scalar(ctx->stream, ctx->obs.as<float>(), (float)ctx->hyper.prior_mean, n, alpha));
    SBO_BLAS(rocsolver_spotrs(ctx->blas, rocblas_fill_lower, (rocblas_int)n, 1, L, (rocblas_int)ld, alpha,
                              (rocblas_int)n));
    SBO_HIP(ctx->Linv.reserve(sizeof(float) * (size_t)ld * (size_t)n));
    float *Li = ctx->Linv.as<float>();
    SBO_HIP(hipMemcpyAsync(Li, L, sizeof(float) * (size_t)ld * (size_t)n, hipMemcpyDeviceToDevice, ctx->stream));
    SBO_BLAS(rocsolver_strtri(ctx->blas, rocblas_fill_lower, rocblas_diagonal_non_unit, (rocblas_int)n, Li,
                              (rocblas_int)ld, ctx->info.as<rocblas_int>()));
    SBO_HIP(sbo::launch_pack_operand(ctx->stream, Li, ld, n, p.npad, 0, p.sf2, ctx->x.as<float>(), ctx->y.as<float>(),
                                     alpha, ctx->aug.as<float>(), ctx->kcoord.as<float>()));
    return SBO_OK;
}

sbo_status refresh_join(sbo_ctx *ctx, const RefreshPlan &p) {
    const int64_t npad = p.npad;
    const bool packs_aux = p.eager_x3 || p.eager_f64;
    if (!packs_aux) {
        SBO_HIP(ctx->scratch.reserve(sizeof(double) * (size_t)npad));
        SBO_HIP(sbo::launch_row_l1(ctx->stream, ctx->aug.as<float>(), npad, p.I0, ctx->scratch.as<double>()));
    }
    if (!p.fused_norms) {
        SBO_HIP(grow_keep(ctx, ctx->tile_lgn, 2 * sizeof(float4) * (size_t)sbo::total_tiles(p.nI),
                          2 * sizeof(float4) * p.old_tiles));
        SBO_HIP(sbo::launch_tile_norms(ctx->stream, ctx->aug.as<float>(), npad, p.I0, ctx->tile_lgn.as<float4>()));
    }
    if (p.f64) {
        if (p.aux) SBO_HIP(hipStreamWaitEvent(ctx->stream, ctx->ev_trail, 0));
        SBO_HIP(sbo::launch_pack_kcoord(ctx->stream, ctx->x.as<float>(), ctx->y.as<float>(), ctx->alpha.as<float>(),
                                        p.n, npad, p.sf2, ctx->kcoord.as<float>()));
        if (p.eager_x3)
            SBO_HIP(sbo::launch_pack_x3(ctx->stream, nullptr, ctx->kcoord.as<float>(), npad, 0, 0, nullptr,
                                        ctx->kc3.as<float>()));
    }
    if (packs_aux) SBO_HIP(hipStreamWaitEvent(ctx->stream, ctx->ev_pack, 0));
    return SBO_OK;
}

int skip_cut(double need) {
    const double l2 = std::log2(std::max(need, 1.0));
    return std::isfinite(l2) ? std::min(160, std::max(16, (int)std::ceil(l2))) : 160;
}
void skip_cutoffs(double max_row_l1, int64_t n, int64_t nI, double tau2, int &L, float &lg_tau) {
    L = skip_cut(max_row_l1 * std::sqrt((double)n) / tau2);
    lg_tau = (float)std::log2(tau2 / std::sqrt((double)nI));
}

sbo_status refresh_skip_budget(sbo_ctx *ctx, const RefreshPlan &p) {
    const int64_t n = p.n, r0 = p.I0 * sbo::kBM;
    std::vector<double> rl1((size_t)(p.npad - r0));
    std::vector<float> ha((size_t)n);
    SBO_HIP(hipMemcpyAsync(rl1.data(), ctx->scratch.as<double>() + r0, sizeof(double) * (p.npad - r0),
                           hipMemcpyDeviceToHost, ctx->stream));
    SBO_HIP(hipMemcpyAsync(ha.data(), ctx->alpha.as<float>(), sizeof(float) * n, hipMemcpyDeviceToHost, ctx->stream));
    SBO_HIP(hipStreamSynchronize(ctx->stream));
    double mx = *std::max_element(rl1.begin(), rl1.end());
    if (p.incr) mx = std::max(mx, ctx->max_row_l1);
    ctx->max_row_l1 = mx;
    double al1 = 0.0;
    for (float v : ha) al1 += std::fabs((double)v);
    ctx->alpha_l1 = al1 * p.sf2;
    const double tol = std::ldexp(1.0, -ctx->skip_budget), sf = std::sqrt(p.sf2);
    const double tau2 = tol * sf / 2.0 * 0.99;
    skip_cutoffs(ctx->max_row_l1, n, p.nI, tau2, ctx->auto_skip_log2, ctx->lg_tau_v);
    ctx->auto_skip_mean_log2 = skip_cut(ctx->alpha_l1 / (tol * sf));
    return SBO_OK;
}

sbo_status refresh_read_info(sbo_ctx *ctx, const RefreshPlan &p) {
    SBO_HIP(ctx->kbox.reserve(sizeof(float4) * (size_t)(p.npad / sbo::kBK)));
    SBO_HIP(sbo::launch_tile_boxes(ctx->stream, ctx->x.as<float>(), ctx->y.as<float>(), p.n, p.npad,
                                   ctx->kbox.as<float4>()));
    const int64_t nslots = info_slots(p.n);
    std::vector<rocblas_int> hinfos((size_t)nslots);
    SBO_HIP(hipMemcpyAsync(hinfos.data(), ctx->info.as<rocblas_int>(), sizeof(rocblas_int) * (size_t)nslots,
                           hipMemcpyDeviceToHost, ctx->stream));
    SBO_HIP(hipStreamSynchronize(ctx->stream));
    rocblas_int hinfo = 0;
    for (rocblas_int v : hinfos)
        if (hinfo == 0) hinfo = v;
    if (hinfo != 0) ctx->linv_n = 0;
    SBO_CHECK(hinfo == 0, SBO_E_NOT_SPD, "trtri: singular factor (info=" + std::to_string(hinfo) + ")");
    ctx->npad = p.npad;
    if (p.eager_x3) {
        ctx->x3_I0 = INT64_MAX;
        ctx->x3_layout = p.x3_layout;
    } else {
        ctx->x3_I0 = std::min(ctx->x3_I0, p.I0);
        if (!p.incr && ctx->a64_I0 != INT64_MAX) ctx->a64_I0 = 0;
    }
    return SBO_OK;
}

sbo_status refresh_guard_verdict(sbo_ctx *ctx, InvAttempt attempt, bool &redo) {
    sbo_inv_check r = ctx->chk_res;
    if (sbo_status st = inverse_check_read(ctx, r)) return st;
    r.err_fallback = r.err_mean_fallback = -1.0;
    r.kept_digits = r.digits;
    ctx->chk_res = r;
    if (attempt != kInvDgemm) record_inv_digits(ctx, r);
    redo = !inv_check_passed(ctx, r) && r.digits != 0 && attempt != kInvDgemm;
    return SBO_OK;
}

sbo_status refresh_operand(sbo_ctx *ctx, int64_t n_old = 0, FactorHandover ho = {}) {
    sbo_inv_check first{};
    bool fired = false;
    float ms_rejected = 0.0f;
    for (InvAttempt attempt = kInvChosen;;) {
// ... 319 lines not shown
                          : rocblas_ssyrk(ctx->blas_aux, rocblas_fill_lower, rocblas_operation_none, (rocblas_int)m4,
                                          (rocblas_int)W, &minus_one, P + W2, (rocblas_int)ld, &one,
                                          C1 + W2 + W2 * ld, (rocblas_int)ld)) == rocblas_status_success;
            if (!ok) { st = SBO_E_DEVICE; break; }
            trail_pending = true;
            if (hipEventRecord(ctx->ev_trail, ctx->aux_stream) != hipSuccess) { st = SBO_E_DEVICE; break; }
        }
        if (wid) {
            if ((m4 <= 0 && hipStreamWaitEvent(ctx->aux_stream, ctx->ev_panel, 0) != hipSuccess) ||
                sbo::launch_widen(ctx->aux_stream, L + K + K * ld, ld, n - K, W, true, Lw + K + K * ld, ld) !=
                    hipSuccess ||
                (K > 0 && hipMemset2DAsync(Lw + K * ld, sizeof(double) * (size_t)ld, 0, sizeof(double) * (size_t)K,
                                           (size_t)W, ctx->aux_stream) != hipSuccess)) {
                st = SBO_E_DEVICE;
                break;
            }
            Kw = K + W;
        }
    }
    if (st != SBO_OK) {
        (void)hipStreamSynchronize(ctx->aux_stream);
        if (early_pending) (void)hipStreamSynchronize(ctx->inv_stream);
        ctx->err = "blocked Cholesky: a rocBLAS or HIP call failed";
        return st;
    }
    if (trail_pending) SBO_HIP(hipStreamWaitEvent(ctx->stream, ctx->ev_trail, 0));
    if (wid) {
        SBO_HIP(sbo::launch_widen(ctx->stream, L + Kw + Kw * ld, ld, n - Kw, n - Kw, true, Lw + Kw + Kw * ld, ld));
        if (Kw > 0)
            SBO_HIP(hipMemset2DAsync(Lw + Kw * ld, sizeof(double) * (size_t)ld, 0, sizeof(double) * (size_t)Kw,
                                     (size_t)(n - Kw), ctx->stream));
        SBO_HIP(hipEventRecord(ctx->ev_trail, ctx->aux_stream));
        SBO_HIP(hipStreamWaitEvent(ctx->stream, ctx->ev_trail, 0));
        ho.widened_n = n;
    }
    if (early_pending) {
        SBO_HIP(hipStreamWaitEvent(ctx->stream, ctx->ev_inv, 0));
        ho.half_n = n;
    }
    if (out) *out = ho;
    return SBO_OK;
}

sbo_status factor_and_refresh(sbo_ctx *ctx) {
    rocblas_int *info = ctx->info.as<rocblas_int>();
    ctx->inv_oz_cur = choose_inv_digits(ctx);
    FactorHandover ho;
    if (ctx->chol_blocked) {
        const bool early_inv = ctx->inverse_bits == 64 && ctx->inverse_rec;
        if (sbo_status st = blocked_potrf(ctx, ctx->L.as<float>(), ctx->n, ctx->cap, info, early_inv, &ho);
            st != SBO_OK)
            return st;
        info = ctx->info.as<rocblas_int>();
    } else {
        SBO_BLAS(rocsolver_spotrf(ctx->blas, rocblas_fill_lower, (rocblas_int)ctx->n, ctx->L.as<float>(),
                                  (rocblas_int)ctx->cap, info));
    }
    rocblas_int hinfo = 0;
    SBO_HIP(hipMemcpyAsync(&hinfo, info, sizeof(hinfo), hipMemcpyDeviceToHost, ctx->stream));
    SBO_HIP(hipStreamSynchronize(ctx->stream));
    if (hinfo != 0) {
        ctx->err = "spotrf: leading minor " + std::to_string(hinfo) + " not positive definite";
        return SBO_E_NOT_SPD;
    }
    ctx->has_factor = true;
    return refresh_operand(ctx, 0, ho);
}

sbo_status run_tick(sbo_ctx *ctx, const float *qx, const float *qy, int64_t m, double beta, double f_min,
                    int score_kind, int64_t index_offset, float *mu, float *sd, double *lo, double *hi,
                    uint8_t *safe, sbo_key *key_dev, float *cost, int sweep, QueryOrder *order) {
    const int64_t nI = ctx->npad / sbo::kBM;
    if (sweep == kSweepCtx) sweep = ctx->precise ? kSweepPrecise : kSweepFast;
    SBO_CHECK(sweep == kSweepFast || (ctx->has_factor && ctx->linv_n == ctx->n && ctx->inverse_bits == 64),
              SBO_E_STATE, "precise sweep: needs the fit's f64 inverse (not an imported state, INVERSE_BITS 64)");
    const bool precise = sweep != kSweepFast;
    const int32_t *perm = nullptr;
    int64_t ms = m;
    sbo::SkipPlan plan;
    if (sweep == kSweepPreciseDense) {
        skip_budget_for(ctx, ctx->probe_ref_tol, plan.L, plan.lg_tau_v);
        plan.L_mean = ctx->auto_skip_mean_log2;
        plan.lgn = ctx->tile_lgn.as<float4>();
        plan.kcoord = ctx->kcoord.as<float>();
    } else if (ctx->skip_log2 < 0) {
        plan.L = precise ? ctx->p_skip_log2 : ctx->auto_skip_log2;
        plan.L_mean = precise ? std::min(160, ctx->auto_skip_mean_log2 + 8) : ctx->auto_skip_mean_log2;
        plan.lgn = ctx->tile_lgn.as<float4>();
        plan.levels = !precise && sbo::x3_levels(ctx->kernel_variant) ? 1 : 0;
        plan.kcoord = ctx->kcoord.as<float>();
        plan.lg_tau_v = precise ? ctx->p_lg_tau_v : ctx->lg_tau_v;
    } else {
        plan.L = ctx->skip_log2;
    }
    plan.prod_full = !precise && ctx->kernel_variant >= 2 ? 6 : 1;
    plan.records = !precise && ctx->kernel_variant >= 2;
    plan.wide = precise;
    plan.order_blk = precise && !cost ? ctx->plan_block : 0;
#ifdef SBO_DIAG
    if (const char *e = getenv("SBO_LVL_FORCE"); e && plan.levels) plan.levels = 2 + std::clamp(atoi(e), 0, 2);
    if (const char *e = getenv("SBO_LVL_KEY")) (void)sscanf(e, "%f,%f", &plan.lvl_key[0], &plan.lvl_key[1]);
#endif
    if (ctx->query_order && plan.L > 0 && m > sbo::kBN) {
        int32_t *p = nullptr;
        float *sx = nullptr, *sy = nullptr;
        if (ctx->query_order == 1) {
            SBO_HIP(ctx->qgwork.reserve(sbo::query_grid_bytes(m)));
            if (qx != ctx->qgrid_x || qy != ctx->qgrid_y || m != ctx->qgrid_m) {
                unsigned long long g[6];
                SBO_HIP(sbo::launch_grid_detect(ctx->stream, qx, qy, m, ctx->qgwork.as<void>(), g));
                sbo::grid_layout(g, m, ctx->qgrid);
                ctx->qgrid_x = qx;
                ctx->qgrid_y = qy;
                ctx->qgrid_m = m;
            }
        }
        if (ctx->query_order == 1 && ctx->qgrid.ok) {
            SBO_HIP(sbo::launch_query_grid(ctx->stream, qx, qy, m, ctx->qgrid, ctx->qgwork.as<void>(), &p, &sx, &sy));
            ms = ctx->qgrid.ms;
        } else if (order && order->perm) {
            p = order->perm;
            sx = order->sx;
            sy = order->sy;
        } else {
            const size_t wb = sbo::query_order_bytes(m);
            SBO_HIP(ctx->qwork.reserve(wb));
            SBO_HIP(sbo::launch_query_order(ctx->stream, qx, qy, m, ctx->bbox, ctx->qwork.as<void>(), wb, &p, &sx, &sy));
            if (order) *order = QueryOrder{p, sx, sy};
        }
        perm = p;
        qx = sx;
        qy = sy;
    }
    const int64_t ldp = sbo::round_up(ms, 64);
    const size_t pw = precise ? sizeof(double) : sizeof(float);
    SBO_HIP(ctx->part.reserve(pw * (size_t)nI * (size_t)ldp));
    SBO_HIP(ctx->mean.reserve(pw * (size_t)ldp));
    const int64_t nb = sbo::acq_blocks(ms);
    SBO_HIP(ctx->keys.reserve(sizeof(sbo_key) * (size_t)(nb + 1)));
    sbo_key *bkeys = ctx->keys.as<sbo_key>();
    const int P = ctx->sweep_groups > 0 ? ctx->sweep_groups : std::max(1, ctx->num_cu);
    {
        const int64_t nQ = (ms + sbo::kBN - 1) / sbo::kBN;
        SBO_CHECK((double)2 * nI * (nI + 1) * (double)nQ < 4294967296.0, SBO_E_INVAL,
                  "sbo_tick: N x M too large for one tick plan (2 nI (nI + 1) nQ >= 2^32 tile entries); "
                  "split the queries into shards");
    }
    SBO_HIP(ctx->plan_work.reserve(sbo::predict_work_bytes(ctx->npad, ms, P)));
    const bool chunked = precise && ctx->precise_kernel >= 3 && ctx->precise_kernel != 9 && !cost;
    const bool pairs = ctx->precise_kernel == 4 || ctx->precise_kernel == 10;
    if (!chunked)
        SBO_HIP(sbo::launch_plan(ctx->stream, ctx->kbox.as<float4>(), ctx->npad, qx, qy, ms, ldp,
                                 (float)ctx->hyper.length_scale, (float)ctx->hyper.prior_mean, plan,
                                 ctx->part.as<float>(), ctx->mean.as<float>(),
                                 ctx->prof && !cost ? ctx->counters.as<unsigned long long>() : nullptr, P,
                                 ctx->plan_work.as<void>(), ctx->plan_work.capacity()));
    if (cost) {
        SBO_HIP(ctx->qcost.reserve(sizeof(float) * (size_t)((ms + sbo::kBN - 1) / sbo::kBN)));
        SBO_HIP(sbo::launch_plan_cost(ctx->stream, ctx->npad, ms, P, ctx->plan_work.as<void>(), perm,
                                      ctx->qcost.as<float>(), cost));
        return SBO_OK;
    }
    if (precise) {
        if (ctx->poz_pending) SBO_HIP(hipStreamWaitEvent(ctx->stream, ctx->ev_poz, 0));
        const int64_t nIc = ctx->npad / sbo::kBM;
        if (ctx->a64_I0 < nIc) {
            if (sbo_status st = pack_precise(ctx, ctx->stream, ctx->npad, std::max<int64_t>(ctx->a64_I0, 0))) return st;
            ctx->a64_I0 = INT64_MAX;
        }
        const int4 *desc = nullptr;
        const unsigned short *tl = nullptr;
        const int *seg = nullptr;
        if (chunked) {
            const int64_t nQ = (ms + sbo::kBN - 1) / sbo::kBN;
            const size_t per_qb = sbo::oz_table_bytes(ctx->npad, pairs);
            size_t budget = (size_t)ctx->table_mb << 20;
            if (budget == 0) {
                size_t fr = 0, tot = 0;
                if (hipMemGetInfo(&fr, &tot) != hipSuccess) fr = size_t(64) << 30;
                budget = std::clamp(fr / 32 + ctx->kzt.capacity() / 32, size_t(256) << 20, size_t(8) << 30);
            }
            const int64_t Qc = std::clamp<int64_t>((int64_t)(budget / per_qb), 1, nQ);
            SBO_HIP(ctx->kzt.reserve(per_qb * (size_t)Qc));
            double *pd = ctx->part.as<double>(), *md = ctx->mean.as<double>();
            Bracket br(ctx, ctx->ev_predict);
            for (int64_t qb0 = 0; qb0 < nQ; qb0 += Qc) {
                const int64_t c0 = qb0 * sbo::kBN, mc = std::min<int64_t>(Qc * sbo::kBN, ms - c0);
                const int64_t nq = (mc + sbo::kBN - 1) / sbo::kBN;
                SBO_HIP(sbo::launch_plan(ctx->stream, ctx->kbox.as<float4>(), ctx->npad, qx + c0, qy + c0, mc, ldp,
                                         (float)ctx->hyper.length_scale, (float)ctx->hyper.prior_mean, plan,
                                         reinterpret_cast<float *>(pd + c0), reinterpret_cast<float *>(md + c0),
                                         ctx->prof ? ctx->counters.as<unsigned long long>() : nullptr, P,
                                         ctx->plan_work.as<void>(), ctx->plan_work.capacity()));
                SBO_HIP(sbo::launch_kstar_table(ctx->stream, ctx->koz.as<char>(), qx + c0, qy + c0, mc, ctx->npad,
                                                ctx->hyper.length_scale, nq, ctx->kzt.as<char>(), pairs));
                sbo::plan_views(ctx->npad, mc, P, ctx->plan_work.as<void>(), &desc, &tl, &seg);
                SBO_HIP(sbo::launch_predict_oz(ctx->stream, ctx->aoz.as<char>(), ctx->eoz.as<int>(),
                                               ctx->koz.as<char>(), desc, tl, seg, P, (int)(nIc * nq), (int)nIc,
                                               qx + c0, qy + c0, mc, ldp, ctx->hyper.length_scale,
                                               ctx->hyper.prior_mean, pd + c0, md + c0, ctx->precise_kernel,
                                               ctx->kzt.as<char>()));
            }
        } else {
        sbo::plan_views(ctx->npad, ms, P, ctx->plan_work.as<void>(), &desc, &tl, &seg);
        Bracket br(ctx, ctx->ev_predict);
        if (ctx->precise_kernel >= 1)
            SBO_HIP(sbo::launch_predict_oz(ctx->stream, ctx->aoz.as<char>(), ctx->eoz.as<int>(), ctx->koz.as<char>(),
                                           desc, tl, seg, P, (int)(nIc * ((ms + sbo::kBN - 1) / sbo::kBN)), (int)nIc,
                                           qx, qy, ms, ldp, ctx->hyper.length_scale, ctx->hyper.prior_mean,
                                           ctx->part.as<double>(), ctx->mean.as<double>(), ctx->precise_kernel));
        else
            SBO_HIP(sbo::launch_predict_f64(ctx->stream, ctx->a64.as<double>(), ctx->kc64.as<double>(), desc, tl, seg,
                                            P, (int)(nIc * ((ms + sbo::kBN - 1) / sbo::kBN)), (int)nIc, qx, qy, ms,
                                            ldp, ctx->hyper.length_scale, ctx->hyper.prior_mean,
                                            ctx->part.as<double>(), ctx->mean.as<double>()));
        }
    } else if (ctx->kernel_variant >= 2) {
        const int64_t nIc = ctx->npad / sbo::kBM;
        if (sbo_status st = derive_x3(ctx)) return st;
        if (!perm) {
            const int64_t mp = sbo::round_up(m, sbo::kBN);
            SBO_HIP(ctx->qpad.reserve(sizeof(float) * 2 * (size_t)mp));
            float *px = ctx->qpad.as<float>(), *py = px + mp;
            SBO_HIP(hipMemcpyAsync(px, qx, sizeof(float) * (size_t)m, hipMemcpyDeviceToDevice, ctx->stream));
            SBO_HIP(hipMemcpyAsync(py, qy, sizeof(float) * (size_t)m, hipMemcpyDeviceToDevice, ctx->stream));
            qx = px;
            qy = py;
        }
        const int4 *desc = nullptr;
        const unsigned short *tl = nullptr;
        const int *seg = nullptr;
        const int4 *rec = nullptr;
        sbo::plan_views(ctx->npad, ms, P, ctx->plan_work.as<void>(), &desc, &tl, &seg, &rec);
        Bracket br(ctx, ctx->ev_predict);
        SBO_HIP(sbo::launch_predict_x3(ctx->stream, ctx->ax3.as<char>(), ctx->kc3.as<float>(), desc, rec, seg, P,
                                       (int)(nIc * ((ms + sbo::kBN - 1) / sbo::kBN)), (int)nIc, qx, qy, ms, ldp,
                                       sbo::exp2_coef_f((float)ctx->hyper.length_scale),
                                       (float)ctx->hyper.prior_mean, ctx->part.as<float>(), ctx->mean.as<float>(),
                                       ctx->kernel_variant));
    } else {
        Bracket br(ctx, ctx->ev_predict);
        SBO_HIP(sbo::launch_predict(ctx->stream, ctx->aug.as<float>(), ctx->kcoord.as<float>(), ctx->npad, qx, qy,
                                    ms, ldp, (float)ctx->hyper.length_scale, (float)ctx->hyper.prior_mean,
                                    ctx->part.as<float>(), ctx->mean.as<float>(), ctx->kernel_variant, P,
                                    ctx->plan_work.as<void>()));
    }
    if (precise) {
        SBO_HIP(sbo::launch_acquire(ctx->stream, ctx->part.as<double>(), ctx->mean.as<double>(), (int)nI, ldp, ms,
                                    ctx->hyper.sigma_f * ctx->hyper.sigma_f, beta, f_min, score_kind, index_offset,
                                    perm, mu, sd, lo, hi, safe, bkeys));
    } else {
        const float sf2 = (float)(ctx->hyper.sigma_f * ctx->hyper.sigma_f);
        SBO_HIP(sbo::launch_acquire(ctx->stream, ctx->part.as<float>(), ctx->mean.as<float>(), (int)nI, ldp, ms, sf2,
                                    beta, f_min, score_kind, index_offset, perm, mu, sd, lo, hi, safe, bkeys));
    }
    SBO_HIP(sbo::launch_reduce_keys(ctx->stream, bkeys, nb, key_dev ? key_dev : bkeys + nb));
    return SBO_OK;
}

}

namespace {
template <typename T>
sbo_status compute_sets_impl(sbo_ctx *ctx, const T *mu, const T *sd, int64_t m, double beta, double f_min,
                             double *lo, double *hi, uint8_t *safe, uint32_t flags) {
    if (!ctx) return SBO_E_INVAL;
    SBO_CHECK(mu && sd, SBO_E_INVAL, "sbo_compute_sets: null mu/sd");
    SBO_CHECK(m >= 0, SBO_E_INVAL, "sbo_compute_sets: m must be >= 0");
    if (m == 0) return SBO_OK;
    SBO_HIP(hipSetDevice(ctx->device));
    if (dev(flags)) {
        SBO_HIP(sbo::launch_sets(ctx->stream, mu, sd, m, beta, f_min, lo, hi, safe));
        return finish(ctx, flags);
    }
    const size_t need = Carve::need(m, sizeof(T)) * 2 + Carve::need(m, 8) * 2 + Carve::need(m, 1);
    SBO_HIP(ctx->hq.reserve(need));
    Carve c(ctx->hq.as<void>());
    T *dmu = c.take<T>(m), *dsd = c.take<T>(m);
    double *dlo = c.take<double>(m), *dhi = c.take<double>(m);
    uint8_t *ds = c.take<uint8_t>(m);
    SBO_HIP(hipMemcpyAsync(dmu, mu, sizeof(T) * m, hipMemcpyHostToDevice, ctx->stream));
    SBO_HIP(hipMemcpyAsync(dsd, sd, sizeof(T) * m, hipMemcpyHostToDevice, ctx->stream));
    SBO_HIP(sbo::launch_sets(ctx->stream, (const T *)dmu, (const T *)dsd, m, beta, f_min, lo ? dlo : nullptr,
                             hi ? dhi : nullptr, safe ? ds : nullptr));
    if (lo) SBO_HIP(hipMemcpyAsync(lo, dlo, sizeof(double) * m, hipMemcpyDeviceToHost, ctx->stream));
    if (hi) SBO_HIP(hipMemcpyAsync(hi, dhi, sizeof(double) * m, hipMemcpyDeviceToHost, ctx->stream));
    if (safe) SBO_HIP(hipMemcpyAsync(safe, ds, m, hipMemcpyDeviceToHost, ctx->stream));
    SBO_HIP(hipStreamSynchronize(ctx->stream));
    return SBO_OK;
}
}

extern "C" {

SBO_API const char *sbo_version(void) { return kVersion; }

SBO_API const char *sbo_status_string(sbo_status s) {
    switch (s) {
        case SBO_OK: return "SBO_OK";
        case SBO_E_INVAL: return "SBO_E_INVAL";
        case SBO_E_NOT_SPD: return "SBO_E_NOT_SPD";
        case SBO_E_DEVICE: return "SBO_E_DEVICE";
        case SBO_E_OOM: return "SBO_E_OOM";
        case SBO_E_EMPTY: return "SBO_E_EMPTY";
        case SBO_E_STATE: return "SBO_E_STATE";
    }
    return "SBO_E_UNKNOWN";
}

SBO_API sbo_status sbo_create(int device, sbo_ctx **out) {
    if (!out) return SBO_E_INVAL;
    *out = nullptr;
    int count = 0;
    if (hipGetDeviceCount(&count) != hipSuccess || device < 0 || device >= count) return SBO_E_DEVICE;
    sbo_ctx *ctx = new (std::nothrow) sbo_ctx();
    if (!ctx) return SBO_E_OOM;
    ctx->device = device;
    if (hipSetDevice(device) != hipSuccess || hipStreamCreateWithFlags(&ctx->own_stream, hipStreamNonBlocking) != hipSuccess ||
        rocblas_create_handle(&ctx->blas) != rocblas_status_success ||
        hipHostMalloc(reinterpret_cast<void **>(&ctx->host_key), sizeof(sbo_key)) != hipSuccess ||
        ctx->info.reserve(256) != hipSuccess ||
        hipDeviceGetAttribute(&ctx->num_cu, hipDeviceAttributeMultiprocessorCount, device) != hipSuccess) {
        sbo_destroy(ctx);
        return SBO_E_DEVICE;
    }
    ctx->stream = ctx->own_stream;
    rocblas_set_stream(ctx->blas, ctx->stream);
    *out = ctx;
    return SBO_OK;
}

SBO_API void sbo_destroy(sbo_ctx *ctx) {
    if (!ctx) return;
    (void)hipSetDevice(ctx->device);
    if (ctx->stream) (void)hipStreamSynchronize(ctx->stream);
    recycle_events(ctx);
    for (hipEvent_t e : ctx->ev_pool) (void)hipEventDestroy(e);
// ... 387 lines not shown
        Bracket br(ctx, ctx->ev_fill);
        SBO_HIP(sbo::launch_rbf_fill(ctx->stream, x, y, n, x, y, n, n, (float)hyper.length_scale, sf2,
                                     (float)hyper.noise_level, true, K));
        return finish(ctx, flags);
    }
    const size_t need = Carve::need(n, 4) * 2 + Carve::need((size_t)n * n, 4);
    SBO_HIP(ctx->hq.reserve(need));
    Carve c(ctx->hq.as<void>());
    float *dx = c.take<float>(n), *dy = c.take<float>(n), *dK = c.take<float>((size_t)n * n);
    SBO_HIP(hipMemcpyAsync(dx, x, sizeof(float) * n, hipMemcpyHostToDevice, ctx->stream));
    SBO_HIP(hipMemcpyAsync(dy, y, sizeof(float) * n, hipMemcpyHostToDevice, ctx->stream));
    SBO_HIP(sbo::launch_rbf_fill(ctx->stream, dx, dy, n, dx, dy, n, n, (float)hyper.length_scale, sf2,
                                 (float)hyper.noise_level, true, dK));
    SBO_HIP(hipMemcpyAsync(K, dK, sizeof(float) * (size_t)n * n, hipMemcpyDeviceToHost, ctx->stream));
    SBO_HIP(hipStreamSynchronize(ctx->stream));
    return SBO_OK;
}

SBO_API sbo_status sbo_get_factor(sbo_ctx *ctx, float *L, float *alpha, uint32_t flags) {
    if (!ctx) return SBO_E_INVAL;
    SBO_CHECK(ctx->fitted && ctx->has_factor, SBO_E_STATE, "sbo_get_factor: call sbo_fit first");
    SBO_HIP(hipSetDevice(ctx->device));
    const int64_t n = ctx->n;
    const hipMemcpyKind k = dev(flags) ? hipMemcpyDeviceToDevice : hipMemcpyDeviceToHost;
    if (L) {
        if (dev(flags)) {
            SBO_HIP(sbo::launch_copy_lower(ctx->stream, ctx->L.as<float>(), ctx->cap, n, L, n));
        } else {
            SBO_HIP(ctx->hq.reserve(sizeof(float) * (size_t)n * n));
            SBO_HIP(sbo::launch_copy_lower(ctx->stream, ctx->L.as<float>(), ctx->cap, n, ctx->hq.as<float>(), n));
            SBO_HIP(hipMemcpyAsync(L, ctx->hq.as<float>(), sizeof(float) * (size_t)n * n, k, ctx->stream));
        }
    }
    if (alpha) SBO_HIP(hipMemcpyAsync(alpha, ctx->alpha.as<float>(), sizeof(float) * n, k, ctx->stream));
    if (!dev(flags)) {
        SBO_HIP(hipStreamSynchronize(ctx->stream));
        return SBO_OK;
    }
    return finish(ctx, flags);
}

SBO_API sbo_status sbo_profile(sbo_ctx *ctx, int enable) {
    if (!ctx) return SBO_E_INVAL;
    SBO_HIP(hipStreamSynchronize(ctx->stream));
    recycle_events(ctx);
    ctx->prof = enable != 0;
    SBO_HIP(ctx->counters.reserve(64));
    SBO_HIP(hipMemsetAsync(ctx->counters.as<void>(), 0, 64, ctx->stream));
    SBO_HIP(hipStreamSynchronize(ctx->stream));
    return SBO_OK;
}

SBO_API sbo_status sbo_profile_work(sbo_ctx *ctx, double *predict_flops) {
    if (!ctx || !predict_flops) return SBO_E_INVAL;
    unsigned long long t = 0;
    if (ctx->counters.capacity()) {
        SBO_HIP(hipMemcpyAsync(&t, ctx->counters.as<void>(), sizeof(t), hipMemcpyDeviceToHost, ctx->stream));
        SBO_HIP(hipStreamSynchronize(ctx->stream));
    }
    *predict_flops = 2.0 * sbo::kBM * sbo::kBN * sbo::kBK * (double)t;
    return SBO_OK;
}

SBO_API sbo_status sbo_debug_x3_stamps(sbo_ctx *ctx, double *cycles, int n) {
    if (!ctx || !cycles || n <= 0) return SBO_E_INVAL;
    SBO_HIP(hipSetDevice(ctx->device));
    SBO_HIP(hipStreamSynchronize(ctx->stream));
    SBO_HIP(sbo::read_x3_stamps(cycles, n));
    return SBO_OK;
}

SBO_API sbo_status sbo_debug_x3_operand(sbo_ctx *ctx, void *host_buf, int64_t cap, int64_t *bytes) {
    if (!ctx || !bytes || cap < 0) return SBO_E_INVAL;
    if (!ctx->fitted || ctx->kernel_variant < 2) return SBO_E_INVAL;
    SBO_HIP(hipSetDevice(ctx->device));
    SBO_HIP(hipStreamSynchronize(ctx->aux_stream));
    if (sbo_status st = derive_x3(ctx)) return st;
    const int64_t need = (int64_t)sbo::x3_operand_bytes(ctx->npad);
    *bytes = need;
    if (!host_buf) return SBO_OK;
    if (cap < need) return SBO_E_INVAL;
    SBO_HIP(hipMemcpyAsync(host_buf, ctx->ax3.as<char>(), (size_t)need, hipMemcpyDeviceToHost, ctx->stream));
    SBO_HIP(hipStreamSynchronize(ctx->stream));
    return SBO_OK;
}

namespace {
static_assert(SBO_GZ_TRI_A == sbo::kGzTriA && SBO_GZ_TRANS_A == sbo::kGzTransA &&
                  SBO_GZ_TRI_B_LOWER == sbo::kGzTriBLower && SBO_GZ_TRI_B_UPPER == sbo::kGzTriBUpper &&
                  SBO_GZ_TRANS_B == sbo::kGzTransB && SBO_GZ_TRANS_C == sbo::kGzTransC &&
                  SBO_GZ_BETA1 == sbo::kGzBeta1 && SBO_GZ_LOWER_C == sbo::kGzLowerC,
              "include/sbo.h documents the sliced GEMM's flags");
sbo_status gz_status(sbo_ctx *ctx, hipError_t e, const char *what) {
    if (e == hipSuccess) return SBO_OK;
    ctx->err = std::string(what) + ": " + hipGetErrorString(e);
    return e == hipErrorInvalidValue ? SBO_E_INVAL : e == hipErrorOutOfMemory ? SBO_E_OOM : SBO_E_DEVICE;
}
}

SBO_API sbo_status sbo_debug_gz_gemm(sbo_ctx *ctx, int nd, int is_f32, const void *A, int64_t lda, int64_t a_cols,
                                     const void *B, int64_t ldb, int64_t b_cols, int64_t m, int64_t n, int64_t K,
                                     double alpha, void *C, int64_t ldc, int64_t c_cols, uint32_t flags) {
    if (!ctx) return SBO_E_INVAL;
    SBO_CHECK(A && B && C, SBO_E_INVAL, "sbo_debug_gz_gemm: null operand");
    SBO_CHECK(m >= 0 && n >= 0 && K >= 0 && lda >= 1 && ldb >= 1 && ldc >= 1 && a_cols >= 1 && b_cols >= 1 &&
                  c_cols >= 1,
              SBO_E_INVAL, "sbo_debug_gz_gemm: negative size or empty buffer");
    SBO_CHECK((flags & ~255u) == 0, SBO_E_INVAL, "sbo_debug_gz_gemm: unknown flag");
    const bool tA = flags & sbo::kGzTransA, tB = flags & sbo::kGzTransB, tC = flags & sbo::kGzTransC;
    SBO_CHECK((tA ? K : m) <= lda && (tA ? m : K) <= a_cols && (tB ? n : K) <= ldb && (tB ? K : n) <= b_cols &&
                  (tC ? n : m) <= ldc && (tC ? m : n) <= c_cols,
              SBO_E_INVAL, "sbo_debug_gz_gemm: operand larger than its buffer");
    SBO_HIP(hipSetDevice(ctx->device));
    const size_t es = is_f32 ? sizeof(float) : sizeof(double);
    const size_t ab = es * (size_t)lda * (size_t)a_cols, bb = es * (size_t)ldb * (size_t)b_cols,
                 cb = es * (size_t)ldc * (size_t)c_cols;
    DevBuf dA, dB, dC, ws;
    SBO_HIP(dA.reserve(ab));
    SBO_HIP(dB.reserve(bb));
    SBO_HIP(dC.reserve(cb));
    SBO_HIP(ws.reserve(sbo::gz_workspace_bytes(std::max<int64_t>(m, 1), std::max<int64_t>(n, 1),
                                               std::max<int64_t>(K, 1), std::min(std::max(nd, 4), 6))));
    SBO_HIP(hipMemcpyAsync(dA.as<void>(), A, ab, hipMemcpyHostToDevice, ctx->stream));
    SBO_HIP(hipMemcpyAsync(dB.as<void>(), B, bb, hipMemcpyHostToDevice, ctx->stream));
    SBO_HIP(hipMemcpyAsync(dC.as<void>(), C, cb, hipMemcpyHostToDevice, ctx->stream));
    const hipError_t e =
        is_f32 ? sbo::launch_gz_gemm_f32(ctx->stream, nd, dA.as<float>(), lda, dB.as<float>(), ldb, m, n, K, alpha,
                                         dC.as<float>(), ldc, flags, ws.as<char>())
               : sbo::launch_gz_gemm(ctx->stream, nd, dA.as<double>(), lda, dB.as<double>(), ldb, m, n, K, alpha,
                                     dC.as<double>(), ldc, flags, ws.as<char>());
    if (e == hipSuccess) SBO_HIP(hipMemcpyAsync(C, dC.as<void>(), cb, hipMemcpyDeviceToHost, ctx->stream));
    SBO_HIP(hipStreamSynchronize(ctx->stream));
    return gz_status(ctx, e, "sbo_debug_gz_gemm");
}

SBO_API sbo_status sbo_debug_gz_gemm_packed(sbo_ctx *ctx, int nd, const float *P, int64_t ld, int64_t mpack,
                                            int64_t K, int64_t a0, int64_t m, int64_t b0, int64_t n, double alpha,
                                            float *C, int64_t ldc, int64_t c_cols, uint32_t flags) {
    if (!ctx) return SBO_E_INVAL;
    SBO_CHECK(P && C, SBO_E_INVAL, "sbo_debug_gz_gemm_packed: null operand");
    SBO_CHECK(mpack >= 1 && K >= 1 && ld >= mpack && a0 >= 0 && b0 >= 0 && m >= 0 && n >= 0 && ldc >= 1 &&
                  c_cols >= 1 && m <= ldc && n <= c_cols,
              SBO_E_INVAL, "sbo_debug_gz_gemm_packed: size out of range or C larger than its buffer");
    SBO_CHECK((flags & ~255u) == 0, SBO_E_INVAL, "sbo_debug_gz_gemm_packed: unknown flag");
    SBO_HIP(hipSetDevice(ctx->device));
    const size_t pb = sizeof(float) * (size_t)ld * (size_t)K, cb = sizeof(float) * (size_t)ldc * (size_t)c_cols;
    DevBuf dP, dC, pack;
    SBO_HIP(dP.reserve(pb));
    SBO_HIP(dC.reserve(cb));
    SBO_HIP(pack.reserve(sbo::gz_pack_bytes(mpack, K, std::min(std::max(nd, 4), 5))));
    SBO_HIP(hipMemcpyAsync(dP.as<void>(), P, pb, hipMemcpyHostToDevice, ctx->stream));
    SBO_HIP(hipMemcpyAsync(dC.as<void>(), C, cb, hipMemcpyHostToDevice, ctx->stream));
    hipError_t e = sbo::launch_gz_pack_f32(ctx->stream, nd, dP.as<float>(), ld, mpack, K, pack.as<char>());
    if (e == hipSuccess)
        e = sbo::launch_gz_gemm_packed_f32(ctx->stream, nd, pack.as<char>(), mpack, K, a0, m, b0, n, alpha,
                                           dC.as<float>(), ldc, flags);
    if (e == hipSuccess) SBO_HIP(hipMemcpyAsync(C, dC.as<void>(), cb, hipMemcpyDeviceToHost, ctx->stream));
    SBO_HIP(hipStreamSynchronize(ctx->stream));
    return gz_status(ctx, e, "sbo_debug_gz_gemm_packed");
}

SBO_API sbo_status sbo_profile_mfma(sbo_ctx *ctx, double *mfma_flops, int64_t *tiles_by_level) {
    if (!ctx || !mfma_flops) return SBO_E_INVAL;
    unsigned long long t[4] = {0, 0, 0, 0};
    if (ctx->counters.capacity()) {
        SBO_HIP(hipMemcpyAsync(t, ctx->counters.as<void>(), sizeof(t), hipMemcpyDeviceToHost, ctx->stream));
// ... 530 lines not shown
    if (!ctx || !bounds) return SBO_E_INVAL;
    if (!ctx->fitted) return SBO_E_STATE;
    for (int i = 0; i < 4; ++i) bounds[i] = (double)ctx->bbox[i];
    return SBO_OK;
}

SBO_API sbo_status sbo_state_bytes(sbo_ctx *ctx, int64_t *bytes) {
    if (!ctx || !bytes) return SBO_E_INVAL;
    SBO_CHECK(ctx->fitted, SBO_E_STATE, "sbo_state_bytes: call sbo_fit first");
    *bytes = state_layout(ctx).total;
    return SBO_OK;
}

SBO_API sbo_status sbo_export_state(sbo_ctx *ctx, void *dev_buf, int64_t cap) {
    if (!ctx) return SBO_E_INVAL;
    SBO_CHECK(ctx->fitted, SBO_E_STATE, "sbo_export_state: call sbo_fit first");
    const StateHeader h = state_layout(ctx);
    SBO_CHECK(dev_buf && cap >= h.total, SBO_E_INVAL, "sbo_export_state: buffer smaller than sbo_state_bytes");
    SBO_HIP(hipSetDevice(ctx->device));
    char *b = static_cast<char *>(dev_buf);
    const int64_t nt = ctx->npad / sbo::kBK;
    SBO_HIP(hipMemcpyAsync(b, &h, sizeof(h), hipMemcpyHostToDevice, ctx->stream));
    SBO_HIP(hipMemcpyAsync(b + h.off_order, ctx->order.data(), 8 * (size_t)h.n, hipMemcpyHostToDevice, ctx->stream));
    SBO_HIP(hipMemcpyAsync(b + h.off_aug, ctx->aug.as<void>(),
                           4 * (size_t)sbo::total_tiles(ctx->npad / sbo::kBM) * sbo::kTileFloats,
                           hipMemcpyDeviceToDevice, ctx->stream));
    SBO_HIP(hipMemcpyAsync(b + h.off_kcoord, ctx->kcoord.as<void>(), 4 * (size_t)nt * 3 * sbo::kBK,
                           hipMemcpyDeviceToDevice, ctx->stream));
    SBO_HIP(hipMemcpyAsync(b + h.off_kbox, ctx->kbox.as<void>(), 16 * (size_t)nt, hipMemcpyDeviceToDevice,
                           ctx->stream));
    SBO_HIP(hipMemcpyAsync(b + h.off_lgn, ctx->tile_lgn.as<void>(),
                           32 * (size_t)sbo::total_tiles(ctx->npad / sbo::kBM), hipMemcpyDeviceToDevice, ctx->stream));
    SBO_HIP(hipStreamSynchronize(ctx->stream));
    return SBO_OK;
}

SBO_API sbo_status sbo_import_state(sbo_ctx *ctx, const void *dev_buf, int64_t bytes) {
    if (!ctx) return SBO_E_INVAL;
    SBO_CHECK(dev_buf && bytes >= (int64_t)sizeof(StateHeader), SBO_E_INVAL, "sbo_import_state: bad buffer");
    SBO_HIP(hipSetDevice(ctx->device));
    if (sbo_status st = drain_poz(ctx)) return st;
    const char *b = static_cast<const char *>(dev_buf);
    StateHeader h;
    SBO_HIP(hipMemcpyAsync(&h, b, sizeof(h), hipMemcpyDeviceToHost, ctx->stream));
    SBO_HIP(hipStreamSynchronize(ctx->stream));
    SBO_CHECK(h.magic == kStateMagic && h.n > 0 && h.n <= (int64_t)1 << 32 && h.npad == sbo::round_up(h.n, sbo::kBM),
              SBO_E_INVAL, "sbo_import_state: not an sbo state blob");
    {
        StateHeader e = h;
        state_offsets(e);
        SBO_CHECK(e.off_order == h.off_order && e.off_aug == h.off_aug && e.off_kcoord == h.off_kcoord &&
                      e.off_kbox == h.off_kbox && e.off_lgn == h.off_lgn && e.total == h.total,
                  SBO_E_INVAL, "sbo_import_state: section offsets do not match the blob's (n, npad)");
        SBO_CHECK(h.total <= bytes, SBO_E_INVAL, "sbo_import_state: truncated blob");
        SBO_CHECK(h.spatial_order >= 0 && h.spatial_order <= 3 && std::isfinite(h.lg_tau_v) &&
                      h.bbox[0] <= h.bbox[1] && h.bbox[2] <= h.bbox[3],
                  SBO_E_INVAL, "sbo_import_state: header fields out of range");
        const sbo_hyper hh{h.hyper[0], h.hyper[1], h.hyper[2], h.hyper[3]};
        if (sbo_status st = check_hyper(ctx, hh)) {
            ctx->err = "sbo_import_state: " + ctx->err;
            return st;
        }
    }
    FitCommit fc(ctx);
    ctx->has_factor = false;
    ctx->precise = false;
    ctx->probe_n = 0;
    ctx->linv_n = 0;
    const int64_t nt = h.npad / sbo::kBK;
    const size_t aug_bytes = 4 * (size_t)sbo::total_tiles(h.npad / sbo::kBM) * sbo::kTileFloats;
    SBO_HIP(ctx->aug.reserve(aug_bytes));
    SBO_HIP(ctx->kcoord.reserve(4 * (size_t)nt * 3 * sbo::kBK));
    SBO_HIP(ctx->kbox.reserve(16 * (size_t)nt));
    SBO_HIP(ctx->tile_lgn.reserve(32 * (size_t)sbo::total_tiles(h.npad / sbo::kBM)));
    ctx->order.resize((size_t)h.n);
    SBO_HIP(hipMemcpyAsync(ctx->order.data(), b + h.off_order, 8 * (size_t)h.n, hipMemcpyDeviceToHost, ctx->stream));
    SBO_HIP(hipMemcpyAsync(ctx->aug.as<void>(), b + h.off_aug, aug_bytes, hipMemcpyDeviceToDevice, ctx->stream));
    SBO_HIP(hipMemcpyAsync(ctx->kcoord.as<void>(), b + h.off_kcoord, 4 * (size_t)nt * 3 * sbo::kBK,
                           hipMemcpyDeviceToDevice, ctx->stream));
    SBO_HIP(hipMemcpyAsync(ctx->kbox.as<void>(), b + h.off_kbox, 16 * (size_t)nt, hipMemcpyDeviceToDevice,
                           ctx->stream));
    SBO_HIP(hipMemcpyAsync(ctx->tile_lgn.as<void>(), b + h.off_lgn, 32 * (size_t)sbo::total_tiles(h.npad / sbo::kBM),
                           hipMemcpyDeviceToDevice, ctx->stream));
    SBO_HIP(hipStreamSynchronize(ctx->stream));
    {
        std::vector<uint8_t> seen((size_t)h.n, 0);
        for (int64_t v : ctx->order) {
            if (v < 0 || v >= h.n || seen[(size_t)v]) {
                ctx->order.clear();
                ctx->n = 0;
                ctx->err = "sbo_import_state: training order is not a permutation";
                return SBO_E_INVAL;
            }
            seen[(size_t)v] = 1;
        }
    }
    ctx->n = h.n;
    ctx->npad = h.npad;
    ctx->hyper = sbo_hyper{h.hyper[0], h.hyper[1], h.hyper[2], h.hyper[3]};
    ctx->jitter = 0.0;
    ctx->max_row_l1 = h.max_row_l1;
    ctx->alpha_l1 = h.alpha_l1;
    for (int i = 0; i < 4; ++i) ctx->bbox[i] = h.bbox[i];
    ctx->auto_skip_log2 = h.auto_skip_log2;
    ctx->auto_skip_mean_log2 = h.auto_skip_mean_log2;
    ctx->lg_tau_v = h.lg_tau_v;
    ctx->spatial_order = h.spatial_order;
    ctx->x3_I0 = 0;
    return fc.commit(SBO_OK);
}

}
```

### safe_bayesian_optimization_amd/csrc/sbo_internal.hpp

```cpp
#pragma once

#include <hip/hip_runtime.h>
#include <rocblas/rocblas.h>

#include <cstddef>
#include <cstdint>
#include <string>
#include <utility>
#include <vector>

#include "../../include/sbo.h"

namespace sbo {

constexpr int kBM = 256;
constexpr int kBN = 128;
constexpr int kBK = 64;
constexpr int kTileFloats = kBM * kBK;
constexpr int kTilesPerRowBlockStep = kBM / kBK;
constexpr int kAcqThreads = 256;
constexpr int64_t kMaxGridY = 65535;

__host__ __device__ inline int64_t round_up(int64_t v, int64_t m) { return (v + m - 1) / m * m; }

// ... 23 lines not shown
        hipError_t e = hipMalloc(&ptr_, bytes);
        if (e != hipSuccess) { ptr_ = nullptr; return e; }
        cap_ = bytes;
        return hipSuccess;
    }
    void release() {
        if (ptr_) (void)hipFree(ptr_);
        ptr_ = nullptr;
        cap_ = 0;
    }
    template <class T> T *as() const { return static_cast<T *>(ptr_); }
    void swap(DevBuf &o) {
        std::swap(ptr_, o.ptr_);
        std::swap(cap_, o.cap_);
    }
    size_t capacity() const { return cap_; }

private:
    void *ptr_ = nullptr;
    size_t cap_ = 0;
};

}

struct sbo_ctx {
    int device = 0;
    hipStream_t own_stream = nullptr;
    hipStream_t stream = nullptr;
    rocblas_handle blas = nullptr;
    hipStream_t aux_stream = nullptr;
    rocblas_handle blas_aux = nullptr;
    int chol_reserve = 0;
    int aux_reserved = 0;
    hipEvent_t ev_panel = nullptr, ev_trail = nullptr;
    hipEvent_t ev_pack = nullptr;
    hipEvent_t ev_poz = nullptr;
    bool poz_pending = false;
    int chol_gemm_own = 4;
    int chol_diag = 1;
    int chol_outer = 1024;
    hipStream_t inv_stream = nullptr;
    rocblas_handle blas_inv = nullptr;
    int inv_overlap = 0, inv_reserved = 0;
    hipEvent_t ev_half = nullptr, ev_inv = nullptr;
    int64_t inv_base = 2048;
    int64_t inv_panels = 16;
    int inv_oz = 6;
    int64_t inv_oz_min = 0;
    int inv_oz_adapt = 1;
    int inv_oz_cur = 0, inv_oz_next = 0;
    int64_t inv_oz_hist_n = 0;
    double inv_oz_hist_area = 0.0;
    sbo_hyper inv_oz_hist_hyper{};
    bool inv_oz_pinned = false;
    int inv_check = 1;
    hipStream_t chk_stream = nullptr;
    hipEvent_t ev_chk0 = nullptr, ev_chk1 = nullptr;
    sbo::DevBuf chk;
    sbo_inv_check chk_res{};
    std::string err;

    int64_t n = 0;
    int64_t cap = 0;
    sbo_hyper hyper{0.4, 1.0, 0.1, 0.0};
    bool fitted = false;
    bool has_factor = false;

    sbo::DevBuf x, y, obs;
    sbo::DevBuf L;
    sbo::DevBuf Linv;
    int64_t linv_n = 0;
    int inverse_bits = 64;
    int jitter_retries = 0;
    double jitter = 0.0;
    bool inverse_rec = true;
    bool chol_blocked = true;
    bool chol_trsm_own = true;
    int spatial_order = 3;
    int skip_log2 = -1;
    int auto_skip_log2 = 160;
    int auto_skip_mean_log2 = 160;
    float lg_tau_v = -1000.0f;
    sbo::DevBuf tile_lgn;
    int skip_budget = 20;
    double max_row_l1 = 0.0;
    double alpha_l1 = 0.0;
    std::vector<int64_t> order;
    float bbox[4] = {0.f, 0.f, 0.f, 0.f};
    int query_order = 1;
    const float *qgrid_x = nullptr, *qgrid_y = nullptr;
    int64_t qgrid_m = -1;
    sbo::QueryGrid qgrid;
    sbo::DevBuf qgwork;
    int kernel_variant = 3;
    int sweep_groups = 0;
    int num_cu = 0;
    sbo::DevBuf plan_work;
    sbo::DevBuf fwork, fowner, fimg, fpix, fout;
    sbo::DevBuf qwork;
    sbo::DevBuf kbox;
    sbo::DevBuf alpha;
    sbo::DevBuf aug;
    sbo::DevBuf kcoord;
    sbo::DevBuf ax3, kc3;
    int64_t x3_I0 = 0;
    int x3_layout = -1;
    sbo::DevBuf qpad;
    sbo::DevBuf qcost;
    sbo::DevBuf info;
    sbo::DevBuf scratch;
    int64_t npad = 0;
    int precision_opt = -1;
    int resort_pct = 25;
    int64_t n_sorted = 0;
    sbo::DevBuf restage;
    bool precise = false;
    sbo::DevBuf alpha64;
    sbo::DevBuf zvec, rvec;
    sbo::DevBuf awork;
    int64_t z_n = 0;
    sbo::DevBuf a64, kc64;
    sbo::DevBuf aoz, eoz, koz;
    sbo::DevBuf gzws;
    sbo::DevBuf gzws_aux;
    sbo::DevBuf cholx3[2];
    sbo::DevBuf kzt;
    int precise_kernel = 3;
    int64_t a64_I0 = 0;
    int64_t probe_n = 0;
    double probe_err = -1.0, probe_vmin = 0.0, probe_vmax = 0.0;
    double probe_err_grid = -1.0, probe_err_train = -1.0, probe_vmax_grid = 0.0, probe_vmax_train = 0.0;
    int probe_m_grid = 0, probe_m_train = 0;
    int64_t table_mb = 0;
    int probe_grid = 32, probe_train = 512;
    int plan_block = 0;
    int reprobe_pct = 25;
    bool inv_batched = true;
    bool inv_leaves_own = true;
    double probe_ref_tol = 0.0;
    int p_skip_log2 = 160;
    float p_lg_tau_v = -1000.0f;
    sbo::DevBuf qprobe, oprobe;

    sbo::DevBuf part, mean;
    sbo::DevBuf hq;
    sbo::DevBuf hout;
    sbo::DevBuf keys;
    sbo_key *host_key = nullptr;

    bool prof = false;
    std::vector<hipEvent_t> ev_pool;
    std::vector<std::pair<hipEvent_t, hipEvent_t>> ev_predict, ev_fill;
    sbo::DevBuf counters;

    bool fail(const std::string &m) { err = m; return false; }
};

namespace sbo {

hipError_t launch_rbf_fill(hipStream_t s, const float *xa, const float *ya, int64_t ma, const float *xb,
                           const float *yb, int64_t mb, int64_t ld, float ell, float sf2, float sn2, bool diag,
                           float *K);
hipError_t launch_sub_scalar(hipStream_t s, const float *in, float v, int64_t n, float *out);
hipError_t launch_copy_lower(hipStream_t s, const float *src, int64_t ld_src, int64_t n,
                             float *dst, int64_t ld_dst);
hipError_t launch_pack_tiles(hipStream_t s, const double *Linv, int64_t ld, int64_t n, int64_t npad, int64_t I0,
                             double sf2, float *aug);
hipError_t launch_pack_kcoord(hipStream_t s, const float *x, const float *y, const float *alpha, int64_t n,
                              int64_t npad, double sf2, float *kcoord);
hipError_t launch_pack_operand(hipStream_t s, const float *Linv, int64_t ld, int64_t n, int64_t npad, int64_t I0,
                               double sf2, const float *x, const float *y, const float *alpha, float *aug,
                               float *kcoord);
hipError_t launch_pack_operand(hipStream_t s, const double *Linv, int64_t ld, int64_t n, int64_t npad, int64_t I0,
                               double sf2, const float *x, const float *y, const float *alpha, float *aug,
                               float *kcoord);
hipError_t launch_widen(hipStream_t s, const float *src, int64_t ld_src, int64_t m, int64_t n, bool lower,
                        double *dst, int64_t ld_dst);
struct SkipPlan {
    int L = 0;
    int L_mean = 0;
    const float4 *lgn = nullptr;
    const float *kcoord = nullptr;
    float lg_tau_v = 0.0f;
    int levels = 0;
    int prod_full = 1;
    bool records = false;
    bool wide = false;
    int order_blk = 0;
    float lvl_key[2] = {0.80f, 1.72f};
};
size_t predict_work_bytes(int64_t npad, int64_t m, int P);
hipError_t launch_plan(hipStream_t s, const float4 *kbox, int64_t npad, const float *qx, const float *qy, int64_t m,
                       int64_t ldp, float ell, float m0, const SkipPlan &skip, float *part, float *mean,
                       unsigned long long *tiles_done, int P, void *work, size_t work_bytes);
hipError_t launch_predict(hipStream_t s, const float *aug, const float *kcoord, int64_t npad, const float *qx,
                          const float *qy, int64_t m, int64_t ldp, float ell, float m0, float *part, float *mean,
                          int variant, int P, const void *work);
float exp2_coef_f(float ell);
hipError_t launch_plan_cost(hipStream_t s, int64_t npad, int64_t m, int P, const void *work, const int32_t *perm,
                            float *bcost, float *cost);
void plan_views(int64_t npad, int64_t m, int P, const void *work, const int4 **desc, const unsigned short **tl,
                const int **seg, const int4 **rec = nullptr);
size_t x3_operand_bytes(int64_t npad);
size_t x3_coord_bytes(int64_t npad);
hipError_t launch_pack_x3(hipStream_t s, const float *aug, const float *kcoord, int64_t npad, int64_t I0, int layout,
                          char *ax3, float *kc3);
constexpr int kLevelShift = 14;
constexpr int kRecFirst = 1 << 20, kRecLast = 1 << 21;
inline bool x3_levels(int variant) { return variant == 3 || variant == 23 || variant == 24 || variant == 30 || variant == 32 || variant == 33 || variant == 39 || variant == 41 || variant == 42 || variant == 43 || variant == 46 || variant == 47 || variant == 48 || variant == 49 || variant == 51 || variant == 52 || variant == 53 || variant == 54 || variant == 55 || variant == 56 || variant == 57 || (variant >= 58 && variant <= 62); }
inline bool variant_allowed(int v) {
#ifdef SBO_DIAG
    return v >= 0 && v <= 62;
#else
    return v == 0 || v == 1 || v == 3 || v == 22;
#endif
}
inline int x3_layout(int variant) { return (variant == 13 || variant == 14) ? 1 : (variant == 3 || variant == 22) ? 2 : 0; }
hipError_t read_x3_stamps(double *out, int n);
hipError_t launch_predict_x3(hipStream_t s, const char *ax3, const float *kc3, const int4 *desc, const int4 *rec,
                             const int *seg, int P, int n_items, int nI, const float *qx, const float *qy, int64_t m,
                             int64_t ldp, float cexp, float m0, float *part, float *mean, int variant);
hipError_t launch_tile_norms(hipStream_t s, const float *aug, int64_t npad, int64_t I0, float4 *lgn);
hipError_t launch_pack_tile_norms(hipStream_t s, const double *Linv, int64_t ld, int64_t n, int64_t npad, int64_t I0,
                                  double sf2, float *aug, float4 *lgn);
constexpr int kCholNB = 128;
hipError_t launch_chol_diag(hipStream_t s, float *A, int64_t ld, int kb, int64_t k0, int *info, int version = 1);
hipError_t launch_chol_update(hipStream_t s, const float *P, const float *Q, int64_t ld, int64_t m, int64_t nc,
                              int64_t K, bool lower, float *C);
size_t chol_x3_bytes(int64_t m, int64_t K);
hipError_t launch_chol_split(hipStream_t s, const float *P, int64_t ld, int64_t m, int64_t K, char *planes);
hipError_t launch_chol_update_x3(hipStream_t s, const char *planes, int64_t m, int64_t K, int64_t r0, int64_t rows,
                                 int64_t c0, int64_t cols, bool lower, float *C, int64_t ld);
hipError_t launch_chol_trsm(hipStream_t s, const float *L11, int64_t ld, int kb, float *A21, int64_t m2, int version = 1);
hipError_t launch_widen_sub(hipStream_t s, const float *in, double v, int64_t n, double *d);
size_t alpha_work_bytes(int64_t n);
hipError_t launch_alpha_f64(hipStream_t s, const double *X, int64_t ld, int64_t n, const float *obs, double m0,
                            double *z, double *alpha, double *work);
hipError_t launch_narrow(hipStream_t s, const double *d, int64_t n, float *out);
hipError_t launch_row_dot(hipStream_t s, const double *A, int64_t ld, int64_t rows, int64_t n, const double *x,
                          double *out);
hipError_t launch_narrow_2d(hipStream_t s, const double *d, int64_t ldd, int64_t m, int64_t n, float *out,
                            int64_t ldo);
hipError_t launch_narrow_strided(hipStream_t s, const double *d, int64_t n, float *out, int64_t stride);
hipError_t launch_row_l1(hipStream_t s, const float *aug, int64_t npad, int64_t I0, double *row_l1);
hipError_t launch_tile_boxes(hipStream_t s, const float *x, const float *y, int64_t n, int64_t npad,
                             float4 *kbox);
hipError_t launch_acquire(hipStream_t s, const float *part, const float *mean, int nI, int64_t ldp,
                          int64_t m, float sf2, double beta, double f_min, int score_kind,
                          int64_t index_offset, const int32_t *perm, float *mu, float *sd, double *lo,
                          double *hi, uint8_t *safe, sbo_key *block_keys);
hipError_t launch_acquire(hipStream_t s, const double *part, const double *mean, int nI, int64_t ldp,
                          int64_t m, double sf2, double beta, double f_min, int score_kind,
                          int64_t index_offset, const int32_t *perm, float *mu, float *sd, double *lo,
                          double *hi, uint8_t *safe, sbo_key *block_keys);
size_t f64_operand_bytes(int64_t npad);
size_t f64_coord_bytes(int64_t npad);
hipError_t launch_pack_f64(hipStream_t s, const double *Linv, int64_t ld, int64_t n, int64_t npad, int64_t I0,
                           double sf2, const float *x, const float *y, const double *alpha, double *a64,
                           double *kc64);
hipError_t launch_predict_f64(hipStream_t s, const double *a64, const double *kc64, const int4 *desc,
                              const unsigned short *tl, const int *seg, int P, int n_items, int nI, const float *qx,
                              const float *qy, int64_t m, int64_t ldp, double ell, double m0, double *part,
                              double *mean);
size_t oz_operand_bytes(int64_t npad);
size_t oz_exp_bytes(int64_t npad);
size_t oz_coord_bytes(int64_t npad);
hipError_t launch_pack_oz(hipStream_t s, const double *Linv, int64_t ld, int64_t n, int64_t npad, int64_t I0,
                          double sf2, const float *x, const float *y, const double *alpha, char *aoz, int *eoz,
                          char *koz, bool pairs = false);
hipError_t launch_predict_oz(hipStream_t s, const char *aoz, const int *eoz, const char *koz, const int4 *desc,
                             const unsigned short *tl, const int *seg, int P, int n_items, int nI, const float *qx,
                             const float *qy, int64_t m, int64_t ldp, double ell, double m0, double *part,
                             double *mean, int variant = 1, const char *kzt = nullptr);
size_t oz_table_bytes(int64_t npad, bool pairs = false);
hipError_t launch_kstar_table(hipStream_t s, const char *koz, const float *qx, const float *qy, int64_t m,
                              int64_t npad, double ell, int64_t nq, char *kzt, bool pairs = false);
constexpr unsigned kGzTriA = 1;
constexpr unsigned kGzTransA = 2;
constexpr unsigned kGzTriBLower = 4;
constexpr unsigned kGzTriBUpper = 8;
constexpr unsigned kGzTransB = 16;
constexpr unsigned kGzTransC = 32;
constexpr unsigned kGzBeta1 = 64;
constexpr unsigned kGzLowerC = 128;
size_t gz_workspace_bytes(int64_t m, int64_t n, int64_t K, int nd);
hipError_t launch_gz_gemm(hipStream_t s, int nd, const double *A, int64_t lda, const double *B, int64_t ldb,
                          int64_t m, int64_t n, int64_t K, double alpha, double *C, int64_t ldc, unsigned flags,
                          char *ws);
hipError_t launch_gz_gemm_f32(hipStream_t s, int nd, const float *A, int64_t lda, const float *B, int64_t ldb,
                              int64_t m, int64_t n, int64_t K, double alpha, float *C, int64_t ldc, unsigned flags,
                              char *ws);
size_t gz_pack_bytes(int64_t m, int64_t K, int nd);
hipError_t launch_gz_pack_f32(hipStream_t s, int nd, const float *P, int64_t ld, int64_t m, int64_t K, char *pack);
hipError_t launch_gz_gemm_packed_f32(hipStream_t s, int nd, const char *pack, int64_t mpack, int64_t K, int64_t a0,
                                     int64_t m, int64_t b0, int64_t n, double alpha, float *C, int64_t ldc,
                                     unsigned flags);
constexpr int kChkQ = 32;
int64_t inv_check_rows(int64_t n);
size_t inv_check_bytes(int64_t n);
hipError_t launch_inv_check(hipStream_t s, const double *Linv, const float *L, int64_t ld, int64_t n,
                            const float *x, const float *y, const float *obs, double m0, double sf2, double ell,
                            void *work, float **qxy, double **colsums);
size_t query_order_bytes(int64_t m);
hipError_t launch_query_order(hipStream_t s, const float *qx, const float *qy, int64_t m, const float bbox[4],
                              void *work, size_t work_bytes, int32_t **perm, float **sqx, float **sqy);
size_t query_grid_bytes(int64_t m);
hipError_t launch_grid_detect(hipStream_t s, const float *qx, const float *qy, int64_t m, void *work,
                              unsigned long long host_g[6]);
bool grid_layout(const unsigned long long g[6], int64_t m, QueryGrid &q);
hipError_t launch_query_grid(hipStream_t s, const float *qx, const float *qy, int64_t m, const QueryGrid &q,
                             void *work, int32_t **perm, float **sqx, float **sqy);
hipError_t launch_sets(hipStream_t s, const float *mu, const float *sd, int64_t m, double beta,
                       double f_min, double *lo, double *hi, uint8_t *safe);
hipError_t launch_sets(hipStream_t s, const double *mu, const double *sd, int64_t m, double beta,
                       double f_min, double *lo, double *hi, uint8_t *safe);
hipError_t launch_argmax_blocks(hipStream_t s, const double *score, const uint8_t *mask, int64_t m,
                                int64_t index_offset, sbo_key *block_keys);
hipError_t launch_reduce_keys(hipStream_t s, const sbo_key *keys, int64_t nblocks, sbo_key *out);

inline int64_t acq_blocks(int64_t m) { return (m + kAcqThreads - 1) / kAcqThreads; }

size_t frontier_work_bytes(int64_t m);
hipError_t launch_frontier_raster(hipStream_t s, const double *Dx, const double *Dy, const uint8_t *safe, int64_t m,
                                  int width, int height, void *work, int32_t *owner, uint8_t *img);
hipError_t launch_frontier_gather(hipStream_t s, const int32_t *pix, int64_t nf, const int32_t *owner,
                                  const double *Dx, const double *Dy, const double *lo, const double *hi, int32_t *F,
                                  double *out);
void trace_external_pixels(const uint8_t *img, int w, int h, std::vector<int32_t> &pix);
int64_t select_subgoal(size_t nf, const double *fx, const double *fy, const double *flo, const double *fhi,
                       double goal_x, double goal_y);

}
```

Baseline: 44.93 million.

## Precompute per-column tile bounds to prune far tiles in the skip planner

Adds a per-tile column maximum of the log-norm bounds, used at plan time to build a compact near-tile list for each query block. Budget totals are computed over near tiles only, in a block-wide flattened pass. Row blocks under budget are written out in bulk instead of running the threshold search per wave. The change also vectorises the tile_knorm loop, threads a nonempty mask into the acquire kernel, and adds a debug plan export. It lowers planner overhead at the cost of more shared memory and extra planner branches that must stay consistent with the original skip rules.

```diff
diff --git a/include/sbo.h b/include/sbo.h
--- a/include/sbo.h
+++ b/include/sbo.h
@@ -195,6 +195,9 @@
 
 SBO_API sbo_status sbo_debug_x3_operand(sbo_ctx *ctx, void *host_buf, int64_t cap, int64_t *bytes);
 
+SBO_API sbo_status sbo_debug_plan(sbo_ctx *ctx, const float *qx, const float *qy, int64_t m, int32_t *host_buf,
+                                  int64_t cap, int64_t *n_out);
+
 #define SBO_GZ_TRI_A 1u
 #define SBO_GZ_TRANS_A 2u
 #define SBO_GZ_TRI_B_LOWER 4u
diff --git a/safe_bayesian_optimization_amd/_native.py b/safe_bayesian_optimization_amd/_native.py
--- a/safe_bayesian_optimization_amd/_native.py
+++ b/safe_bayesian_optimization_amd/_native.py
@@ -25,7 +25,7 @@
     "sbo_get_bounds", "sbo_get_jitter", "sbo_get_tile_bounds", "sbo_state_bytes", "sbo_export_state", "sbo_import_state", "sbo_query_cost",
     "sbo_polygon_correct", "sbo_polydist", "sbo_point_within", "sbo_project_subgoal", "sbo_get_precision",
     "sbo_kd_order", "sbo_get_probe", "sbo_keys_reduce", "sbo_get_inverse_check", "sbo_trim", "sbo_warmup",
-    "sbo_debug_gz_gemm", "sbo_debug_gz_gemm_packed", "sbo_debug_x3_operand",
+    "sbo_debug_gz_gemm", "sbo_debug_gz_gemm_packed", "sbo_debug_x3_operand", "sbo_debug_plan",
 )
 SBO_GZ_TRI_A = 1
 SBO_GZ_TRANS_A = 2
@@ -214,6 +214,8 @@
     L.sbo_debug_x3_stamps.restype = st
     L.sbo_debug_x3_operand.argtypes = [vp, vp, i64, ctypes.POINTER(i64)]
     L.sbo_debug_x3_operand.restype = st
+    L.sbo_debug_plan.argtypes = [vp, vp, vp, i64, vp, i64, ctypes.POINTER(i64)]
+    L.sbo_debug_plan.restype = st
     L.sbo_debug_gz_gemm.argtypes = [vp, i32, i32, vp, i64, i64, vp, i64, i64, i64, i64, i64, dbl, vp, i64, i64, u32]
     L.sbo_debug_gz_gemm.restype = st
     L.sbo_debug_gz_gemm_packed.argtypes = [vp, i32, vp, i64, i64, i64, i64, i64, i64, i64, dbl, vp, i64, i64, u32]
diff --git a/safe_bayesian_optimization_amd/csrc/kernels.hip b/safe_bayesian_optimization_amd/csrc/kernels.hip
--- a/safe_bayesian_optimization_amd/csrc/kernels.hip
+++ b/safe_bayesian_optimization_amd/csrc/kernels.hip
@@ -1371,6 +1371,17 @@
 constexpr unsigned kMeanWeight0 = 80, kMeanWeight1 = 45, kMeanWeight2 = 33;
 __device__ unsigned g_mean_w[3] = {kMeanWeight0, kMeanWeight1, kMeanWeight2};
 __device__ unsigned g_rb_slope = 0;
+#ifdef SBO_DIAG
+__device__ unsigned long long g_plan_near[9] = {0ull, 0ull, 0ull, 0ull, 0ull, 0ull, 0ull, 0ull, 0ull};
+#define SBO_PLAN_LAP(acc)                                \
+    if (threadIdx.x == 0) {                              \
+        const unsigned long long now_ = wall_clock64(); \
+        (acc) += now_ - tprev_;                          \
+        tprev_ = now_;                                   \
+    }
+#else
+#define SBO_PLAN_LAP(acc)
+#endif
 constexpr int kSteps = kBK / 4;
 constexpr int kRowBlocks = kBM / 16;
 
@@ -1509,9 +1520,20 @@
     __device__ __forceinline__ float d2(int t) const { return t < kPlanD2 ? d2s[t] : tile_box_d2(kbox[t], box); }
     __device__ __forceinline__ float kn(int t) const { return t < kPlanD2 ? kns[t] : 3.0f + cexp * d2(t) * 0.999f; }
 
+    __device__ __forceinline__ bool far_lg(float l, float dd) const {
+        const float kf = fmaxf(0.0f, fmaxf(key.x + kLg3, key.y + kLg1));
+        return l + cexp * dd * 0.999f - lg_tau + 0.01f + kf < -(float)kBudgetFloor;
+    }
     __device__ __forceinline__ bool far_tile(int I, int t, float dd) const {
-        const float kf = fmaxf(0.0f, fmaxf(key.x + kLg3, key.y + kLg1));
-        return lgn[2 * (tile_start(I) + t)].x + cexp * dd * 0.999f - lg_tau + 0.01f + kf < -(float)kBudgetFloor;
+        return far_lg(lgn[2 * (tile_start(I) + t)].x, dd);
+    }
+
+    const unsigned long long *nearm = nullptr;
+    const int *nearp = nullptr;
+    const unsigned short *nearl = nullptr;
+    __device__ __forceinline__ int near_count(int T) const {
+        const int c = T >> 6, r = T & 63;
+        return nearp[c] + (r ? __popcll(nearm[c] & ((1ull << r) - 1ull)) : 0);
     }
 
     __device__ __forceinline__ void incs(int I, int t, int (&bi)[3], unsigned long long (&w)[3]) const {
@@ -1528,11 +1550,12 @@
 
     __device__ unsigned long long total_weight(int I, int lane, bool &over) const {
         const int T = kTilesPerRowBlockStep * (I + 1);
-        unsigned long long wsum = 0;
+        const int n = nearl ? near_count(T) : T;
+        unsigned long long wsum = lane == 0 ? 6ull * (unsigned long long)(T - n) : 0ull;
         int ov = 0;
-        for (int t0 = 0; t0 < T; t0 += 64) {
-            const int t = t0 + lane;
-            if (t < T) {
+        for (int t0 = 0; t0 < n; t0 += 64) {
+            if (t0 + lane < n) {
+                const int t = nearl ? (int)nearl[t0 + lane] : t0 + lane;
                 if (far_tile(I, t, d2(t))) {
                     wsum += 6ull;
                 } else {
@@ -1563,8 +1586,10 @@
         const int T = kTilesPerRowBlockStep * (I + 1);
         for (int i = lane; i < kBudgetBins; i += 64) bins[i] = 0ull;
         __builtin_amdgcn_wave_barrier();
-        unsigned long long nfar = 0;
-        for (int t = lane; t < T; t += 64) {
+        const int n = nearl ? near_count(T) : T;
+        unsigned long long nfar = lane == 0 ? (unsigned long long)(T - n) : 0ull;
+        for (int i = lane; i < n; i += 64) {
+            const int t = nearl ? (int)nearl[i] : i;
             if (far_tile(I, t, d2(t))) {
                 ++nfar;
                 if (bc && t < kPlanBinCache) bc[t] = 0u;
@@ -1624,25 +1649,42 @@
                 incs(I, t, bi, w);
                 spent = (bi[0] <= drop_max) + (bi[1] <= drop_max) + (bi[2] <= drop_max);
             }
-            code = spent == 3 ? -1 : (levels == 1 ? spent : (levels > 1 ? levels - 2 : 0));
+            code = spent_code(spent);
         } else {
             code = (skip_d2 <= 0.0f || dd <= skip_d2) ? 0 : -1;
         }
+        return mean_keep(I, dd, code);
+    }
+    __device__ __forceinline__ int spent_code(int spent) const {
+        return spent == 3 ? -1 : (levels == 1 ? spent : (levels > 1 ? levels - 2 : 0));
+    }
+    __device__ __forceinline__ int mean_keep(int I, float dd, int code) const {
         if (code < 0 && I == nI - 1 && dd <= skip_d2_mean) code = lgn && levels ? 2 : 0;
         return code;
     }
+    __device__ __forceinline__ int level_far(int I, int t, int drop_max) const {
+        return mean_keep(I, d2(t), spent_code(drop_max >= 0 ? 3 : 0));
+    }
 };
 
 __device__ __forceinline__ float plan_ref(float lg_tau, int nI) { return lg_tau + 0.5f * __log2f((float)nI) - 1e-4f; }
+constexpr int kDropAll = 64 * ((kBudgetBins + 63) / 64) - 1;
 constexpr int kPlanMaxI = 512;
 
 __device__ __forceinline__ float tile_knorm(const float *__restrict__ kc, const QBox &b, float cexp, float d2box) {
     float sum = 0.0f;
-    for (int i = 0; i < kBK; ++i) {
-        const float px = kc[i], py = kc[kBK + i];
-        const float dx = fmaxf(0.0f, fmaxf(b.x0 - px, px - b.x1));
-        const float dy = fmaxf(0.0f, fmaxf(b.y0 - py, py - b.y1));
-        sum += __builtin_amdgcn_exp2f(fmaf(2.0f * cexp, fmaf(dy, dy, dx * dx) * 0.999f, 120.0f));
+    const float4 *kx = reinterpret_cast<const float4 *>(kc), *ky = reinterpret_cast<const float4 *>(kc + kBK);
+#pragma unroll 4
+    for (int i = 0; i < kBK / 4; ++i) {
+        const float4 vx = kx[i], vy = ky[i];
+        const float pxs[4] = {vx.x, vx.y, vx.z, vx.w}, pys[4] = {vy.x, vy.y, vy.z, vy.w};
+#pragma unroll
+        for (int j = 0; j < 4; ++j) {
+            const float px = pxs[j], py = pys[j];
+            const float dx = fmaxf(0.0f, fmaxf(b.x0 - px, px - b.x1));
+            const float dy = fmaxf(0.0f, fmaxf(b.y0 - py, py - b.y1));
+            sum += __builtin_amdgcn_exp2f(fmaf(2.0f * cexp, fmaf(dy, dy, dx * dx) * 0.999f, 120.0f));
+        }
     }
     return sum > 0.0f ? 0.5f * (__log2f(sum * 1.002f) - 120.0f) + 0.001f : 3.0f + cexp * d2box * 0.999f;
 }
@@ -1707,28 +1749,140 @@
     const float *__restrict__ qx, const float *__restrict__ qy, int64_t m, float cexp, float skip_d2,
     float skip_d2_mean, float lg_tau, float m0, int64_t ldp, float *__restrict__ part, float *__restrict__ mean,
     unsigned long long *__restrict__ key, unsigned char *__restrict__ thr, unsigned long long *__restrict__ wkey,
-    unsigned long long *__restrict__ bits, int wide, int blk) {
+    unsigned long long *__restrict__ bits, int wide, int blk, const float *__restrict__ colmax, int zero_empty,
+    unsigned long long *__restrict__ nemask) {
     extern __shared__ unsigned plan_dyn[];
     __shared__ float red[4 * kPlanWaves];
+    __shared__ unsigned long long nearm[kPlanD2 / 64];
+    __shared__ int nearp[kPlanD2 / 64 + 1];
+    __shared__ unsigned long long nem[(1 << kLevelShift) / kTilesPerRowBlockStep / 64];
     __shared__ unsigned long long bins[kPlanWaves][kBudgetBins];
     __shared__ unsigned long long wtot[kPlanMaxI];
     __shared__ unsigned long long budget_exp;
+    __shared__ int cumn[kPlanMaxI + 1];
+    __shared__ unsigned short todo[kPlanMaxI];
+    __shared__ int ntodo;
+    __shared__ unsigned ovm[kPlanMaxI / 32];
     const int64_t qb = blockIdx.x;
     const int lane = threadIdx.x & 63, wave = threadIdx.x >> 6;
     const int nkt = kTilesPerRowBlockStep * nI;
+    const int nem_words = (nI + 63) >> 6;
+    for (int i = threadIdx.x; i < nem_words; i += kPlanThreads) nem[i] = 0ull;
     unsigned *bc = plan_dyn + wave * kPlanBinCache;
     float *d2s = reinterpret_cast<float *>(plan_dyn + kPlanWaves * kPlanBinCache);
     float *kns = d2s + min(nkt, kPlanD2);
     PlanRule R{kbox, lgn, cexp, skip_d2, skip_d2_mean, plan_ref(lg_tau, nI), nI, {}, d2s, kns, levels, lvl_key};
+#ifdef SBO_DIAG
+    unsigned long long tprev_ = wall_clock64(), lap[7] = {0ull, 0ull, 0ull, 0ull, 0ull, 0ull, 0ull};
+#endif
     R.box = plan_setup(qx, qy, m, qb, kbox, lgn ? kcoord : nullptr, cexp, nkt, d2s, kns, red);
+    SBO_PLAN_LAP(lap[0])
+    const bool pre = lgn && colmax && nkt <= kPlanD2;
+    if (pre) {
+        unsigned short *nearl = reinterpret_cast<unsigned short *>(kns + nkt);
+        const int nch = (nkt + 63) >> 6;
+        for (int c = wave; c < nch; c += kPlanWaves) {
+            const int t = c * 64 + lane;
+            const unsigned long long b = __ballot(t < nkt && !R.far_lg(colmax[t < nkt ? t : 0], d2s[t < nkt ? t : 0]));
+            if (lane == 0) nearm[c] = b;
+        }
+        __syncthreads();
+        if (wave == 0) {
+            const int cnt = lane < nch ? __popcll(nearm[lane]) : 0;
+            int incl = cnt;
+#pragma unroll
+            for (int o = 1; o < 64; o <<= 1) {
+                const int u = __shfl_up(incl, o);
+                if (lane >= o) incl += u;
+            }
+            if (lane < nch) nearp[lane + 1] = incl;
+            if (lane == 0) nearp[0] = 0;
+        }
+        __syncthreads();
+        for (int c = wave; c < nch; c += kPlanWaves) {
+            const unsigned long long b = nearm[c];
+            if ((b >> lane) & 1ull)
+                nearl[nearp[c] + __popcll(b & ((1ull << lane) - 1ull))] = (unsigned short)(c * 64 + lane);
+        }
+        __syncthreads();
+        R.nearm = nearm;
+        R.nearp = nearp;
+        R.nearl = nearl;
+#ifdef SBO_DIAG
+        if (threadIdx.x == 0) {
+            atomicAdd(&g_plan_near[0], (unsigned long long)nearp[nch]);
+            atomicAdd(&g_plan_near[1], (unsigned long long)nkt);
+        }
+#endif
+    }
+    SBO_PLAN_LAP(lap[1])
     const bool fill = lgn && nI <= kPlanMaxI;
-    if (fill) {
+    if (fill && pre) {
+        for (int I = threadIdx.x; I < nI; I += kPlanThreads) {
+            const int T = kTilesPerRowBlockStep * (I + 1), n = R.near_count(T);
+            cumn[I + 1] = n;
+            wtot[I] = 6ull * (unsigned long long)(T - n);
+        }
+        if (threadIdx.x < kPlanMaxI / 32) ovm[threadIdx.x] = 0u;
+        if (threadIdx.x == 0) cumn[0] = 0;
+        __syncthreads();
+        if (wave == 0) {
+            const int per = (nI + 63) >> 6, base = 1 + lane * per;
+            int sum = 0;
+            for (int j = 0; j < per; ++j) sum += base + j <= nI ? cumn[base + j] : 0;
+            int incl = sum;
+#pragma unroll
+            for (int o = 1; o < 64; o <<= 1) {
+                const int u = __shfl_up(incl, o);
+                if (lane >= o) incl += u;
+            }
+            int run = incl - sum;
+            for (int j = 0; j < per; ++j)
+                if (base + j <= nI) {
+                    run += cumn[base + j];
+                    cumn[base + j] = run;
+                }
+        }
+        __syncthreads();
+        const int ptot = cumn[nI];
+        for (int p = threadIdx.x; p < ptot; p += kPlanThreads) {
+            int lo = 0, hi = nI - 1;
+            while (lo < hi) {
+                const int mid = (lo + hi + 1) >> 1;
+                if (cumn[mid] <= p) lo = mid;
+                else hi = mid - 1;
+            }
+            const int I = lo, t = (int)R.nearl[p - cumn[I]];
+            if (R.far_tile(I, t, R.d2(t))) {
+                atomicAdd(&wtot[I], 6ull);
+            } else {
+                int bi[3];
+                unsigned long long w[3], ws = 0ull;
+                R.incs(I, t, bi, w);
+                bool ov = false;
+#pragma unroll
+                for (int j = 0; j < 3; ++j) {
+                    if (bi[j] < kBudgetBins - 1) ws += w[j];
+                    else ov = true;
+                }
+                atomicAdd(&wtot[I], ws);
+                if (ov) atomicOr(&ovm[I >> 5], 1u << (I & 31));
+            }
+        }
+        __syncthreads();
+        for (int I = threadIdx.x; I < nI; I += kPlanThreads)
+            if ((ovm[I >> 5] >> (I & 31)) & 1u) wtot[I] = ~0ull;
+        __syncthreads();
+    } else if (fill) {
         for (int I = wave; I < nI; I += kPlanWaves) {
             bool over;
             const unsigned long long w = R.total_weight(I, lane, over);
             if (lane == 0) wtot[I] = over ? ~0ull : w;
         }
         __syncthreads();
+    }
+    if (fill) {
+        SBO_PLAN_LAP(lap[2])
         if (threadIdx.x == 0) {
             const double one = 4294967296.0;
             double share = 1.0 / sqrt((double)nI);
@@ -1749,12 +1903,39 @@
             budget_exp = (unsigned long long)floor(share * one);
         }
         __syncthreads();
-    }
-    for (int I = wave; I < nI; I += kPlanWaves) {
+        SBO_PLAN_LAP(lap[3])
+    }
+    const bool flat = pre && fill && !zero_empty;
+    if (flat) {
+        if (wave == 0) {
+            int base = 0;
+            for (int I0 = 0; I0 < nI; I0 += 64) {
+                const int I = I0 + lane;
+                const bool work = I < nI && (I == nI - 1 || wtot[I] > budget_exp);
+                const unsigned long long b = __ballot(work);
+                if (work) todo[base + __popcll(b & ((1ull << lane) - 1ull))] = (unsigned short)I;
+                base += __popcll(b);
+            }
+            if (lane == 0) ntodo = base;
+        }
+        for (int I = threadIdx.x; I < nI - 1; I += kPlanThreads)
+            if (wtot[I] <= budget_exp) {
+                const int64_t item = plan_item(I, nI, nQ, qb, blk);
+                key[item] = 0ull;
+                thr[item] = (unsigned char)(kDropAll + 1);
+                wkey[item] = 0ull;
+            }
+        __syncthreads();
+    }
+    const int nwork = flat ? ntodo : nI;
+    for (int idx = wave; idx < nwork; idx += kPlanWaves) {
+        const int I = flat ? (int)todo[idx] : idx;
         const int T = kTilesPerRowBlockStep * (I + 1);
         const unsigned long long bud = !fill ? (unsigned long long)floor(4294967296.0 / sqrt((double)nI))
                                        : (wtot[I] <= budget_exp ? ~0ull : budget_exp);
-        const int drop_max = R.threshold(I, bins[wave], lane, bud, bc);
+        const bool cheap = pre && bud == ~0ull;
+        const int drop_max = cheap ? kDropAll : R.threshold(I, bins[wave], lane, bud, bc);
+        SBO_PLAN_LAP(lap[4])
         const int64_t item = plan_item(I, nI, nQ, qb, blk);
         unsigned long long *ib = bits + item * (int64_t)plan_chunks(nI) * 3;
         int cnt = 0;
@@ -1762,7 +1943,23 @@
 #pragma unroll 1
         for (int t0 = 0; t0 < T; t0 += 64) {
             const int t = t0 + lane;
-            const int code = t < T ? R.level(I, t, drop_max, bc) : -1;
+            int code;
+            if (cheap) {
+                if (I != nI - 1) {
+                    if (lane < 3) ib[(t0 >> 6) * 3 + lane] = 0ull;
+                    continue;
+                }
+                code = t < T ? R.mean_keep(I, R.d2(t), -1) : -1;
+            } else if (pre) {
+                const unsigned long long nm = nearm[t0 >> 6];
+                if (nm == 0ull && drop_max >= 0 && I != nI - 1) {
+                    if (lane < 3) ib[(t0 >> 6) * 3 + lane] = 0ull;
+                    continue;
+                }
+                code = t < T ? (((nm >> lane) & 1ull) ? R.level(I, t, drop_max, bc) : R.level_far(I, t, drop_max)) : -1;
+            } else {
+                code = t < T ? R.level(I, t, drop_max, bc) : -1;
+            }
             const unsigned long long b0 = __ballot(code == 0), b1 = __ballot(code == 1), b2 = __ballot(code == 2);
             if (lane < 3) ib[(t0 >> 6) * 3 + lane] = lane == 0 ? (b0 | b1 | b2) : (lane == 1 ? b1 : b2);
             const int n0 = __popcll(b0), n1 = __popcll(b1), n2 = __popcll(b2);
@@ -1770,6 +1967,7 @@
             wsum += I == nI - 1 ? g_mean_w[0] * n0 + g_mean_w[1] * n1 + g_mean_w[2] * n2
                                 : kLevelWeight0 * n0 + kLevelWeight1 * n1 + kLevelWeight2 * n2;
         }
+        SBO_PLAN_LAP(lap[5])
         if (g_rb_slope)
             wsum = (unsigned)((unsigned long long)wsum * (100u * (unsigned)nI + g_rb_slope * (unsigned)I) /
                               (100u * (unsigned)nI));
@@ -1777,21 +1975,29 @@
             key[item] = (unsigned long long)cnt | ((cnt > 0 ? 1ull : 0ull) << kPlanKeyShift);
             thr[item] = (unsigned char)(drop_max + 1);
             wkey[item] = wsum;
+            if (cnt > 0) atomicOr(&nem[I >> 6], 1ull << (I & 63));
         }
         if (cnt == 0)
             for (int j = lane; j < kBN; j += 64) {
                 const int64_t q = qb * kBN + j;
                 if (q < m) {
                     if (wide) {
-                        reinterpret_cast<double *>(part)[(int64_t)I * ldp + q] = 0.0;
+                        if (zero_empty) reinterpret_cast<double *>(part)[(int64_t)I * ldp + q] = 0.0;
                         if (I == nI - 1) reinterpret_cast<double *>(mean)[q] = (double)m0;
                     } else {
-                        part[(int64_t)I * ldp + q] = 0.0f;
+                        if (zero_empty) part[(int64_t)I * ldp + q] = 0.0f;
                         if (I == nI - 1) mean[q] = m0;
                     }
                 }
             }
-    }
+        SBO_PLAN_LAP(lap[6])
+    }
+#ifdef SBO_DIAG
+    if (threadIdx.x == 0)
+        for (int i = 0; i < 7; ++i) atomicAdd(&g_plan_near[2 + i], lap[i]);
+#endif
+    __syncthreads();
+    for (int i = threadIdx.x; i < nem_words; i += kPlanThreads) nemask[qb * nem_words + i] = nem[i];
 }
 
 __global__ __launch_bounds__(256) void plan_write_kernel(
@@ -1908,7 +2114,10 @@
                                  int *__restrict__ pos_of, unsigned long long *__restrict__ cnt2) {
     const int64_t nne = (int64_t)(scan[n_items - 1] >> kPlanKeyShift);
     const int64_t k = (int64_t)blockIdx.x * blockDim.x + threadIdx.x;
-    if (k >= nne) return;
+    if (k >= nne) {
+        if (k < n_items) cnt2[k] = 0ull;
+        return;
+    }
     const int64_t p = xcd_position(k, xseg, G);
     pos_of[k] = (int)p;
     cnt2[p] = (unsigned long long)(desc[k].w & 0xffff);
@@ -2211,21 +2420,24 @@
     double sf2, double beta, double f_min, int score_kind, int64_t index_offset,
     const int32_t *__restrict__ perm, float *__restrict__ mu_out, float *__restrict__ sd_out,
     double *__restrict__ lo_out, double *__restrict__ hi_out, uint8_t *__restrict__ safe_out,
-    sbo_key *__restrict__ keys) {
+    sbo_key *__restrict__ keys, const unsigned long long *__restrict__ nemask) {
     const int64_t i = (int64_t)blockIdx.x * kAcqThreads + threadIdx.x;
     double bs = 0.0;
     int64_t bi = -1;
     if (i < m && (!perm || perm[i] >= 0)) {
+        const unsigned long long *ne = nemask ? nemask + (i / kBN) * (int64_t)((nI + 63) >> 6) : nullptr;
         double s = 0.0;
         int I = 0;
         for (; I + 8 <= nI; I += 8) {
+            const unsigned b = ne ? (unsigned)(ne[I >> 6] >> (I & 63)) & 0xffu : 0xffu;
             PT v[8];
 #pragma unroll
-            for (int u = 0; u < 8; ++u) v[u] = part[(int64_t)(I + u) * ldp + i];
+            for (int u = 0; u < 8; ++u) v[u] = ((b >> u) & 1u) ? part[(int64_t)(I + u) * ldp + i] : (PT)0;
 #pragma unroll
             for (int u = 0; u < 8; ++u) s += (double)v[u];
         }
-        for (; I < nI; ++I) s += (double)part[(int64_t)I * ldp + i];
+        for (; I < nI; ++I)
+            if (!ne || ((ne[I >> 6] >> (I & 63)) & 1ull)) s += (double)part[(int64_t)I * ldp + i];
         double vd = sf2 - s;
         float var = vd > 0.0 ? (float)vd : 0.0f;
         const float sd = __fsqrt_rn(var);
@@ -2495,7 +2707,7 @@
 
 namespace {
 struct PlanLayout {
-    size_t key, scan, thr, desc, tl, seg, temp, temp_bytes, wkey, wscan, lvcnt, rec, bits;
+    size_t key, scan, thr, desc, tl, seg, temp, temp_bytes, wkey, wscan, lvcnt, rec, bits, nemask;
     bool xcd;
     size_t xseg, pos_of, cnt2, off2, desc2, tl2, seg2, temp2, temp2_bytes;
     size_t total;
@@ -2518,6 +2730,7 @@
     L.thr = take((size_t)items);
     L.wkey = take(8 * (size_t)items);
     L.wscan = take(8 * (size_t)items);
+    L.nemask = take(8 * (size_t)nQ * (size_t)((nI + 63) / 64));
     L.lvcnt = take(8 * 3 * 4 * (size_t)kPlanWriteBlocks);
     L.bits = take(8 * 3 * (size_t)items * (size_t)plan_chunks((int)nI));
     L.desc = take(16 * (size_t)(items + 2 * kDescWindow));
@@ -2598,14 +2811,25 @@
     const int levels = lgn ? skip.levels : 0;
     auto *bits = reinterpret_cast<unsigned long long *>(w + L.bits);
     const int nc = std::min(kTilesPerRowBlockStep * nI, kPlanD2);
-    const size_t plan_lds = 4 * (size_t)kPlanWaves * kPlanBinCache + 8 * (size_t)nc;
+    const size_t plan_lds = 4 * (size_t)kPlanWaves * kPlanBinCache + 8 * (size_t)nc + 2 * (size_t)nc;
     hipLaunchKernelGGL(plan_count_kernel, dim3((unsigned)nQ), dim3(kPlanThreads), plan_lds, s, kbox, skip.kcoord, lgn,
                        levels, make_float2(skip.lvl_key[0], skip.lvl_key[1]), nI,
                        nQ, qx, qy,
                        m, cexp, skip_d2, skip_d2_mean, skip.lg_tau_v, m0, ldp, part, mean, key, thr, wkey, bits,
-                       skip.wide ? 1 : 0, skip.order_blk);
+                       skip.wide ? 1 : 0, skip.order_blk, lgn ? skip.colmax : nullptr, skip.zero_empty ? 1 : 0,
+                       reinterpret_cast<unsigned long long *>(w + L.nemask));
     hipError_t e = hipGetLastError();
     if (e != hipSuccess) return e;
+#ifdef SBO_DIAG
+    if (getenv("SBO_PLAN_STATS")) {
+        unsigned long long h[9] = {}, z[9] = {};
+        (void)hipStreamSynchronize(s);
+        (void)hipMemcpyFromSymbol(h, HIP_SYMBOL(g_plan_near), sizeof(h));
+        (void)hipMemcpyToSymbol(HIP_SYMBOL(g_plan_near), z, sizeof(z));
+        fprintf(stderr, "plan stats: near (qb, t) pairs %llu of %llu; clock setup %llu near %llu totals %llu fill %llu "
+                        "thresholds %llu levels %llu rest %llu\n", h[0], h[1], h[2], h[3], h[4], h[5], h[6], h[7], h[8]);
+    }
+#endif
     size_t tb = L.temp_bytes;
     e = rocprim::inclusive_scan(w + L.temp, tb, key, scan, (size_t)items, rocprim::plus<unsigned long long>(), s);
     if (e != hipSuccess) return e;
@@ -2636,8 +2860,10 @@
     auto *tl2 = reinterpret_cast<unsigned short *>(w + L.tl2);
     auto *seg2 = reinterpret_cast<int *>(w + L.seg2);
     const int G = P / 8;
-    e = hipMemsetAsync(cnt2, 0, 8 * (size_t)items, s);
-    if (e != hipSuccess) return e;
+    if (skip.ref_chain) {
+        e = hipMemsetAsync(cnt2, 0, 8 * (size_t)items, s);
+        if (e != hipSuccess) return e;
+    }
     hipLaunchKernelGGL(plan_seg_kernel, dim3(1), dim3(256), 0, s, scan, items, desc, 8, xseg, tiles_done, wkey, wscan,
                        nI, nQ, skip.order_blk);
     hipLaunchKernelGGL(plan_perm_kernel, dim3((unsigned)((items + 255) / 256)), dim3(256), 0, s, scan, items, desc,
@@ -2662,6 +2888,37 @@
     *tl = reinterpret_cast<const unsigned short *>(w + (L.xcd ? L.tl2 : L.tl));
     *seg = reinterpret_cast<const int *>(w + (L.xcd ? L.seg2 : L.seg));
     if (rec) *rec = reinterpret_cast<const int4 *>(w + L.rec);
+}
+
+void plan_item_views(int64_t npad, int64_t m, int P, const void *work, const unsigned long long **key,
+                     const unsigned long long **scan, const unsigned char **thr, const unsigned long long **nonempty) {
+    const PlanLayout L = plan_layout(npad / kBM, (m + kBN - 1) / kBN, P);
+    const char *w = static_cast<const char *>(work);
+    *key = reinterpret_cast<const unsigned long long *>(w + L.key);
+    *scan = reinterpret_cast<const unsigned long long *>(w + L.scan);
+    *thr = reinterpret_cast<const unsigned char *>(w + L.thr);
+    if (nonempty) *nonempty = reinterpret_cast<const unsigned long long *>(w + L.nemask);
+}
+
+namespace {
+__global__ void tile_colmax_kernel(const float4 *__restrict__ lgn, int nI, float *__restrict__ colmax) {
+    const int t = blockIdx.x * blockDim.x + threadIdx.x;
+    if (t >= kTilesPerRowBlockStep * nI) return;
+    float mx = -INFINITY;
+    for (int I = t / kTilesPerRowBlockStep; I < nI; ++I) {
+        const float v = lgn[2 * (tile_start(I) + t)].x;
+        mx = v != v ? INFINITY : fmaxf(mx, v);
+    }
+    colmax[t] = mx;
+}
+}
+
+hipError_t launch_tile_colmax(hipStream_t s, const float4 *lgn, int64_t npad, float *colmax) {
+    const int nI = (int)(npad / kBM);
+    if (nI <= 0) return hipSuccess;
+    hipLaunchKernelGGL(tile_colmax_kernel, dim3((unsigned)((kTilesPerRowBlockStep * nI + 255) / 256)), dim3(256), 0, s,
+                       lgn, nI, colmax);
+    return hipGetLastError();
 }
 
 float exp2_coef_f(float ell) { return (float)exp2_coef(ell); }
@@ -2702,20 +2959,20 @@
 hipError_t launch_acquire(hipStream_t s, const float *part, const float *mean, int nI, int64_t ldp,
                           int64_t m, float sf2, double beta, double f_min, int score_kind,
                           int64_t index_offset, const int32_t *perm, float *mu, float *sd, double *lo,
-                          double *hi, uint8_t *safe, sbo_key *block_keys) {
+                          double *hi, uint8_t *safe, sbo_key *block_keys, const unsigned long long *nonempty) {
     hipLaunchKernelGGL(acquire_kernel<float>, dim3((unsigned)acq_blocks(m)), dim3(kAcqThreads), 0, s, part, mean,
                        nI, ldp, m, (double)sf2, beta, f_min, score_kind, index_offset, perm, mu, sd, lo, hi, safe,
-                       block_keys);
+                       block_keys, nonempty);
     return hipGetLastError();
 }
 
 hipError_t launch_acquire(hipStream_t s, const double *part, const double *mean, int nI, int64_t ldp,
                           int64_t m, double sf2, double beta, double f_min, int score_kind,
                           int64_t index_offset, const int32_t *perm, float *mu, float *sd, double *lo,
-                          double *hi, uint8_t *safe, sbo_key *block_keys) {
+                          double *hi, uint8_t *safe, sbo_key *block_keys, const unsigned long long *nonempty) {
     hipLaunchKernelGGL(acquire_kernel<double>, dim3((unsigned)acq_blocks(m)), dim3(kAcqThreads), 0, s, part, mean,
                        nI, ldp, m, sf2, beta, f_min, score_kind, index_offset, perm, mu, sd, lo, hi, safe,
-                       block_keys);
+                       block_keys, nonempty);
     return hipGetLastError();
 }
 
diff --git a/safe_bayesian_optimization_amd/csrc/sbo_api.cpp b/safe_bayesian_optimization_amd/csrc/sbo_api.cpp
--- a/safe_bayesian_optimization_amd/csrc/sbo_api.cpp
+++ b/safe_bayesian_optimization_amd/csrc/sbo_api.cpp
@@ -953,6 +953,12 @@
     return SBO_OK;
 }
 
+sbo_status refresh_colmax(sbo_ctx *ctx, int64_t npad) {
+    SBO_HIP(ctx->tile_colmax.reserve(sizeof(float) * (size_t)(npad / sbo::kBK)));
+    SBO_HIP(sbo::launch_tile_colmax(ctx->stream, ctx->tile_lgn.as<float4>(), npad, ctx->tile_colmax.as<float>()));
+    return SBO_OK;
+}
+
 sbo_status refresh_join(sbo_ctx *ctx, const RefreshPlan &p) {
     const int64_t npad = p.npad;
     const bool packs_aux = p.eager_x3 || p.eager_f64;
@@ -965,6 +971,7 @@
                           2 * sizeof(float4) * p.old_tiles));
         SBO_HIP(sbo::launch_tile_norms(ctx->stream, ctx->aug.as<float>(), npad, p.I0, ctx->tile_lgn.as<float4>()));
     }
+    if (sbo_status st = refresh_colmax(ctx, npad)) return st;
     if (p.f64) {
         if (p.aux) SBO_HIP(hipStreamWaitEvent(ctx->stream, ctx->ev_trail, 0));
         SBO_HIP(sbo::launch_pack_kcoord(ctx->stream, ctx->x.as<float>(), ctx->y.as<float>(), ctx->alpha.as<float>(),
@@ -1450,11 +1457,13 @@
         skip_budget_for(ctx, ctx->probe_ref_tol, plan.L, plan.lg_tau_v);
         plan.L_mean = ctx->auto_skip_mean_log2;
         plan.lgn = ctx->tile_lgn.as<float4>();
+        plan.colmax = ctx->tile_colmax.as<float>();
         plan.kcoord = ctx->kcoord.as<float>();
     } else if (ctx->skip_log2 < 0) {
         plan.L = precise ? ctx->p_skip_log2 : ctx->auto_skip_log2;
         plan.L_mean = precise ? std::min(160, ctx->auto_skip_mean_log2 + 8) : ctx->auto_skip_mean_log2;
         plan.lgn = ctx->tile_lgn.as<float4>();
+        plan.colmax = ctx->tile_colmax.as<float>();
         plan.levels = !precise && sbo::x3_levels(ctx->kernel_variant) ? 1 : 0;
         plan.kcoord = ctx->kcoord.as<float>();
         plan.lg_tau_v = precise ? ctx->p_lg_tau_v : ctx->lg_tau_v;
@@ -1517,12 +1526,22 @@
     SBO_HIP(ctx->plan_work.reserve(sbo::predict_work_bytes(ctx->npad, ms, P)));
     const bool chunked = precise && ctx->precise_kernel >= 3 && ctx->precise_kernel != 9 && !cost;
     const bool pairs = ctx->precise_kernel == 4 || ctx->precise_kernel == 10;
+    plan.zero_empty = chunked;
+#ifdef SBO_DIAG
+    if (const char *e = getenv("SBO_PLAN_REF"); e && atoi(e)) {
+        plan.colmax = nullptr;
+        plan.zero_empty = true;
+        plan.ref_chain = true;
+    }
+#endif
     if (!chunked)
         SBO_HIP(sbo::launch_plan(ctx->stream, ctx->kbox.as<float4>(), ctx->npad, qx, qy, ms, ldp,
                                  (float)ctx->hyper.length_scale, (float)ctx->hyper.prior_mean, plan,
                                  ctx->part.as<float>(), ctx->mean.as<float>(),
                                  ctx->prof && !cost ? ctx->counters.as<unsigned long long>() : nullptr, P,
                                  ctx->plan_work.as<void>(), ctx->plan_work.capacity()));
+    ctx->plan_ms = chunked ? 0 : ms;
+    ctx->plan_P = P;
     if (cost) {
         SBO_HIP(ctx->qcost.reserve(sizeof(float) * (size_t)((ms + sbo::kBN - 1) / sbo::kBN)));
         SBO_HIP(sbo::launch_plan_cost(ctx->stream, ctx->npad, ms, P, ctx->plan_work.as<void>(), perm,
@@ -1613,14 +1632,19 @@
                                     ctx->part.as<float>(), ctx->mean.as<float>(), ctx->kernel_variant, P,
                                     ctx->plan_work.as<void>()));
     }
+    const unsigned long long *pkey = nullptr, *pscan = nullptr, *nonempty = nullptr;
+    const unsigned char *pthr = nullptr;
+    if (!plan.zero_empty)
+        sbo::plan_item_views(ctx->npad, ms, P, ctx->plan_work.as<void>(), &pkey, &pscan, &pthr, &nonempty);
     if (precise) {
         SBO_HIP(sbo::launch_acquire(ctx->stream, ctx->part.as<double>(), ctx->mean.as<double>(), (int)nI, ldp, ms,
                                     ctx->hyper.sigma_f * ctx->hyper.sigma_f, beta, f_min, score_kind, index_offset,
-                                    perm, mu, sd, lo, hi, safe, bkeys));
+                                    perm, mu, sd, lo, hi, safe, bkeys, nonempty));
     } else {
         const float sf2 = (float)(ctx->hyper.sigma_f * ctx->hyper.sigma_f);
         SBO_HIP(sbo::launch_acquire(ctx->stream, ctx->part.as<float>(), ctx->mean.as<float>(), (int)nI, ldp, ms, sf2,
-                                    beta, f_min, score_kind, index_offset, perm, mu, sd, lo, hi, safe, bkeys));
+                                    beta, f_min, score_kind, index_offset, perm, mu, sd, lo, hi, safe, bkeys,
+                                    nonempty));
     }
     SBO_HIP(sbo::launch_reduce_keys(ctx->stream, bkeys, nb, key_dev ? key_dev : bkeys + nb));
     return SBO_OK;
@@ -2174,6 +2198,78 @@
     if (cap < need) return SBO_E_INVAL;
     SBO_HIP(hipMemcpyAsync(host_buf, ctx->ax3.as<char>(), (size_t)need, hipMemcpyDeviceToHost, ctx->stream));
     SBO_HIP(hipStreamSynchronize(ctx->stream));
+    return SBO_OK;
+}
+
+SBO_API sbo_status sbo_debug_plan(sbo_ctx *ctx, const float *qx, const float *qy, int64_t m, int32_t *host_buf,
+                                  int64_t cap, int64_t *n_out) {
+    if (!ctx || !n_out || cap < 0) return SBO_E_INVAL;
+    SBO_CHECK(ctx->fitted, SBO_E_STATE, "sbo_debug_plan: call sbo_fit first");
+    SBO_CHECK(qx && qy, SBO_E_INVAL, "sbo_debug_plan: null pointer");
+    SBO_CHECK(m > 0, SBO_E_EMPTY, "sbo_debug_plan: m must be > 0");
+    SBO_HIP(hipSetDevice(ctx->device));
+    SBO_HIP(ctx->hq.reserve(Carve::need(m, 4) * 3));
+    Carve c(ctx->hq.as<void>());
+    float *dqx = c.take<float>(m), *dqy = c.take<float>(m), *dc = c.take<float>(m);
+    SBO_HIP(hipMemcpyAsync(dqx, qx, sizeof(float) * m, hipMemcpyHostToDevice, ctx->stream));
+    SBO_HIP(hipMemcpyAsync(dqy, qy, sizeof(float) * m, hipMemcpyHostToDevice, ctx->stream));
+    if (sbo_status st = run_tick(ctx, dqx, dqy, m, 0.0, 0.0, SBO_SCORE_WIDTH, 0, nullptr, nullptr, nullptr, nullptr,
+                                 nullptr, nullptr, dc))
+        return st;
+    const int64_t nI = ctx->npad / sbo::kBM, ms = ctx->plan_ms, nQ = (ms + sbo::kBN - 1) / sbo::kBN;
+    const int64_t items = nI * nQ;
+    const unsigned long long *key = nullptr, *scan = nullptr;
+    const unsigned char *thr = nullptr;
+    const int4 *desc = nullptr;
+    const unsigned short *tl = nullptr;
+    const int *seg = nullptr;
+    sbo::plan_item_views(ctx->npad, ms, ctx->plan_P, ctx->plan_work.as<void>(), &key, &scan, &thr);
+    sbo::plan_views(ctx->npad, ms, ctx->plan_P, ctx->plan_work.as<void>(), &desc, &tl, &seg);
+    std::vector<unsigned long long> hkey((size_t)items);
+    std::vector<unsigned char> hthr((size_t)items);
+    unsigned long long last = 0;
+    SBO_HIP(hipMemcpyAsync(hkey.data(), key, 8 * (size_t)items, hipMemcpyDeviceToHost, ctx->stream));
+    SBO_HIP(hipMemcpyAsync(hthr.data(), thr, (size_t)items, hipMemcpyDeviceToHost, ctx->stream));
+    SBO_HIP(hipMemcpyAsync(&last, scan + items - 1, 8, hipMemcpyDeviceToHost, ctx->stream));
+    SBO_HIP(hipStreamSynchronize(ctx->stream));
+    const unsigned long long cmask = (1ull << 40) - 1ull;
+    const int64_t total = (int64_t)(last & cmask), nne = (int64_t)(last >> 40);
+    const int64_t need = 4 + 2 * items + 4 * total;
+    *n_out = need;
+    if (!host_buf) return SBO_OK;
+    if (cap < need) return SBO_E_INVAL;
+    std::vector<int4> hdesc((size_t)nne);
+    std::vector<unsigned short> htl((size_t)total);
+    if (nne) SBO_HIP(hipMemcpyAsync(hdesc.data(), desc, 16 * (size_t)nne, hipMemcpyDeviceToHost, ctx->stream));
+    if (total) SBO_HIP(hipMemcpyAsync(htl.data(), tl, 2 * (size_t)total, hipMemcpyDeviceToHost, ctx->stream));
+    SBO_HIP(hipStreamSynchronize(ctx->stream));
+    host_buf[0] = (int32_t)nI;
+    host_buf[1] = (int32_t)nQ;
+    host_buf[2] = (int32_t)total;
+    host_buf[3] = (int32_t)nne;
+    int32_t *it = host_buf + 4, *rec = it + 2 * items;
+    for (int64_t I = 0; I < nI; ++I)
+        for (int64_t qb = 0; qb < nQ; ++qb) {
+            const int64_t item = (nI - 1 - I) * nQ + qb;
+            it[2 * (I * nQ + qb)] = (int32_t)hthr[(size_t)item];
+            it[2 * (I * nQ + qb) + 1] = (int32_t)(hkey[(size_t)item] & cmask);
+        }
+    int64_t r = 0;
+    for (int64_t k = 0; k < nne; ++k) {
+        const int4 d = hdesc[(size_t)k];
+        const int cnt = d.w & 0xffff;
+        const uint64_t off = (uint64_t)(uint32_t)d.z | ((uint64_t)((uint32_t)d.w >> 16) << 32);
+        SBO_CHECK(off + (uint64_t)cnt <= (uint64_t)total && r + cnt <= total, SBO_E_DEVICE,
+                  "sbo_debug_plan: a descriptor points outside the tile list");
+        for (int i = 0; i < cnt; ++i, ++r) {
+            const unsigned short te = htl[(size_t)off + i];
+            rec[4 * r] = d.x;
+            rec[4 * r + 1] = d.y;
+            rec[4 * r + 2] = te & ((1 << sbo::kLevelShift) - 1);
+            rec[4 * r + 3] = te >> sbo::kLevelShift;
+        }
+    }
+    SBO_CHECK(r == total, SBO_E_DEVICE, "sbo_debug_plan: the descriptors' counts do not sum to the plan's total");
     return SBO_OK;
 }
 
@@ -2870,6 +2966,7 @@
                            ctx->stream));
     SBO_HIP(hipMemcpyAsync(ctx->tile_lgn.as<void>(), b + h.off_lgn, 32 * (size_t)sbo::total_tiles(h.npad / sbo::kBM),
                            hipMemcpyDeviceToDevice, ctx->stream));
+    if (sbo_status st = refresh_colmax(ctx, h.npad)) return st;
     SBO_HIP(hipStreamSynchronize(ctx->stream));
     {
         std::vector<uint8_t> seen((size_t)h.n, 0);
diff --git a/safe_bayesian_optimization_amd/csrc/sbo_internal.hpp b/safe_bayesian_optimization_amd/csrc/sbo_internal.hpp
--- a/safe_bayesian_optimization_amd/csrc/sbo_internal.hpp
+++ b/safe_bayesian_optimization_amd/csrc/sbo_internal.hpp
@@ -129,6 +129,7 @@
     int auto_skip_mean_log2 = 160;
     float lg_tau_v = -1000.0f;
     sbo::DevBuf tile_lgn;
+    sbo::DevBuf tile_colmax;
     int skip_budget = 20;
     double max_row_l1 = 0.0;
     double alpha_l1 = 0.0;
@@ -143,6 +144,8 @@
     int sweep_groups = 0;
     int num_cu = 0;
     sbo::DevBuf plan_work;
+    int64_t plan_ms = 0;
+    int plan_P = 0;
     sbo::DevBuf fwork, fowner, fimg, fpix, fout;
     sbo::DevBuf qwork;
     sbo::DevBuf kbox;
@@ -234,6 +237,9 @@
     bool records = false;
     bool wide = false;
     int order_blk = 0;
+    const float *colmax = nullptr;
+    bool zero_empty = false;
+    bool ref_chain = false;
     float lvl_key[2] = {0.80f, 1.72f};
 };
 size_t predict_work_bytes(int64_t npad, int64_t m, int P);
@@ -248,6 +254,10 @@
                             float *bcost, float *cost);
 void plan_views(int64_t npad, int64_t m, int P, const void *work, const int4 **desc, const unsigned short **tl,
                 const int **seg, const int4 **rec = nullptr);
+void plan_item_views(int64_t npad, int64_t m, int P, const void *work, const unsigned long long **key,
+                     const unsigned long long **scan, const unsigned char **thr,
+                     const unsigned long long **nonempty = nullptr);
+hipError_t launch_tile_colmax(hipStream_t s, const float4 *lgn, int64_t npad, float *colmax);
 size_t x3_operand_bytes(int64_t npad);
 size_t x3_coord_bytes(int64_t npad);
 hipError_t launch_pack_x3(hipStream_t s, const float *aug, const float *kcoord, int64_t npad, int64_t I0, int layout,
@@ -295,11 +305,13 @@
 hipError_t launch_acquire(hipStream_t s, const float *part, const float *mean, int nI, int64_t ldp,
                           int64_t m, float sf2, double beta, double f_min, int score_kind,
                           int64_t index_offset, const int32_t *perm, float *mu, float *sd, double *lo,
-                          double *hi, uint8_t *safe, sbo_key *block_keys);
+                          double *hi, uint8_t *safe, sbo_key *block_keys,
+                          const unsigned long long *nonempty = nullptr);
 hipError_t launch_acquire(hipStream_t s, const double *part, const double *mean, int nI, int64_t ldp,
                           int64_t m, double sf2, double beta, double f_min, int score_kind,
                           int64_t index_offset, const int32_t *perm, float *mu, float *sd, double *lo,
-                          double *hi, uint8_t *safe, sbo_key *block_keys);
+                          double *hi, uint8_t *safe, sbo_key *block_keys,
+                          const unsigned long long *nonempty = nullptr);
 size_t f64_operand_bytes(int64_t npad);
 size_t f64_coord_bytes(int64_t npad);
 hipError_t launch_pack_f64(hipStream_t s, const double *Linv, int64_t ld, int64_t n, int64_t npad, int64_t I0,
```

New measurement: 45.84 million, median of 6. +2.0%, better.
